# semihkacmaz/CoNFiLD

Hardware: AMD Instinct MI355X
Metric: generated fields/sec (256-step sample + CNF decode), Case4 latent, 1/2/4/8 GPU (higher is better)
Workload: dtype f32

## Files before the change

confild_amd/_lib.py:

```python
from __future__ import annotations

import ctypes as C
import os
import threading

_HERE = os.path.dirname(os.path.abspath(__file__))
LIB_PATH = os.path.join(_HERE, "lib", "libconfild_hip.so")
if os.environ.get("CFD_LIB"):
    LIB_PATH = os.path.join(_HERE, "lib", os.path.basename(os.environ["CFD_LIB"]))

_lock = threading.Lock()
_lib = None

c_f32p = C.POINTER(C.c_float)
c_i64p = C.POINTER(C.c_int64)


class CfdError(RuntimeError):
    pass


class UNetCfg(C.Structure):
    _fields_ = [("image_size", C.c_int), ("in_channels", C.c_int), ("model_channels", C.c_int),
                ("out_channels", C.c_int), ("num_res_blocks", C.c_int), ("n_mult", C.c_int),
                ("channel_mult", C.c_int * 8), ("n_attn", C.c_int), ("attention_ds", C.c_int * 8),
                ("num_heads", C.c_int), ("num_head_channels", C.c_int)]


class SirenCfg(C.Structure):
    _fields_ = [("in_coord_features", C.c_int), ("in_latent_features", C.c_int), ("out_features", C.c_int),
                ("num_hidden_layers", C.c_int), ("hidden_features", C.c_int), ("w0", C.c_float)]


_SIGS = {
    "cfd_last_error": (C.c_char_p, []),
    "cfd_version": (C.c_char_p, []),
    "cfd_unet_create": (C.c_int, [C.POINTER(UNetCfg), C.c_int, C.POINTER(C.c_void_p)]),
    "cfd_unet_destroy": (None, [C.c_void_p]),
    "cfd_unet_num_params": (C.c_int, [C.c_void_p, C.POINTER(C.c_int)]),
    "cfd_unet_param_info": (C.c_int, [C.c_void_p, C.c_int, C.POINTER(C.c_char_p), C.POINTER(C.c_int),
                                      C.c_int64 * 4]),
    "cfd_unet_set_param": (C.c_int, [C.c_void_p, C.c_char_p, C.c_void_p, C.c_size_t]),
    "cfd_unet_set_time_freqs": (C.c_int, [C.c_void_p, C.c_void_p, C.c_int]),
    "cfd_unet_ready": (C.c_int, [C.c_void_p]),
    "cfd_unet_load_flat": (C.c_int, [C.c_void_p, C.c_void_p, C.c_size_t, C.c_void_p]),
    "cfd_unet_set_compute": (C.c_int, [C.c_void_p, C.c_int]),
    "cfd_unet_set_plan_batch": (C.c_int, [C.c_void_p, C.c_int]),
    "cfd_device_cu_count": (C.c_int, [C.c_int, C.POINTER(C.c_int)]),
    "cfd_stream_create_cu_range": (C.c_int, [C.c_int, C.c_int, C.c_int, C.POINTER(C.c_void_p)]),
    "cfd_stream_destroy": (C.c_int, [C.c_void_p]),
    "cfd_unet_check_finite": (C.c_int, [C.c_void_p, C.POINTER(C.c_int), C.c_void_p]),
    "cfd_unet_workspace_bytes": (C.c_int, [C.c_void_p, C.c_int, C.POINTER(C.c_size_t)]),
    "cfd_unet_forward": (C.c_int, [C.c_void_p, C.c_void_p, C.c_void_p, C.c_void_p, C.c_int, C.c_void_p,
                                   C.c_size_t, C.c_void_p]),
    "cfd_unet_tape_bytes": (C.c_int, [C.c_void_p, C.c_int, C.POINTER(C.c_size_t)]),
    "cfd_unet_vjp_workspace_bytes": (C.c_int, [C.c_void_p, C.c_int, C.POINTER(C.c_size_t)]),
    "cfd_unet_forward_tape": (C.c_int, [C.c_void_p, C.c_void_p, C.c_void_p, C.c_void_p, C.c_int, C.c_void_p,
                                        C.c_size_t, C.c_void_p, C.c_size_t, C.c_void_p]),
    "cfd_unet_input_vjp": (C.c_int, [C.c_void_p, C.c_void_p, C.c_void_p, C.c_int, C.c_void_p, C.c_size_t,
                                     C.c_void_p, C.c_size_t, C.c_void_p]),
    "cfd_unet_set_tape_mode": (C.c_int, [C.c_void_p, C.c_int]),
    "cfd_sched_create": (C.c_int, [C.c_void_p, C.c_int, C.c_int, C.POINTER(C.c_void_p)]),
    "cfd_sched_destroy": (None, [C.c_void_p]),
    "cfd_sched_step": (C.c_int, [C.c_void_p, C.c_int, C.c_int, C.c_void_p, C.c_void_p, C.c_void_p, C.c_void_p,
                                 C.c_uint64, C.c_uint64, C.c_uint64, C.c_void_p, C.c_void_p, C.c_int64, C.c_int,
                                 C.c_void_p]),
    "cfd_sched_step_known": (C.c_int, [C.c_void_p, C.c_int, C.c_int, C.c_void_p, C.c_void_p, C.c_void_p, C.c_void_p,
                                       C.c_uint64, C.c_uint64, C.c_uint64, C.c_void_p, C.c_void_p, C.c_int64,
                                       C.c_int, C.c_void_p, C.c_int64, C.c_void_p, C.c_int64, C.c_void_p,
                                       C.c_void_p, C.c_uint64, C.c_void_p]),
    "cfd_sched_step_jump": (C.c_int, [C.c_void_p, C.c_int, C.c_int, C.c_void_p, C.c_void_p, C.c_void_p, C.c_void_p,
                                      C.c_uint64, C.c_uint64, C.c_uint64, C.c_void_p, C.c_void_p, C.c_int64,
                                      C.c_int, C.c_void_p, C.c_int64, C.c_void_p, C.c_int64, C.c_void_p,
                                      C.c_void_p, C.c_uint64, C.c_float, C.c_float, C.c_void_p, C.c_uint64,
                                      C.c_void_p]),
    "cfd_sampler_set_jumps": (C.c_int, [C.c_void_p, C.c_void_p]),
    "cfd_sampler_set_known": (C.c_int, [C.c_void_p, C.c_void_p, C.c_int64, C.c_void_p, C.c_int64, C.c_void_p,
                                        C.c_void_p]),
    "cfd_sampler_captures": (C.c_int, [C.c_void_p, C.POINTER(C.c_uint64)]),
    "cfd_dps_latent_residual_workspace_bytes": (C.c_int, [C.c_int64, C.c_int, C.POINTER(C.c_size_t)]),
    "cfd_dps_latent_residual": (C.c_int, [C.c_void_p, C.c_int, C.c_void_p, C.c_void_p, C.c_void_p, C.c_void_p,
                                          C.c_int64, C.c_void_p, C.c_int64, C.c_void_p, C.c_void_p, C.c_void_p,
                                          C.c_int64, C.c_int, C.c_void_p, C.c_size_t, C.c_void_p]),
    "cfd_sampler_create": (C.c_int, [C.c_void_p, C.c_void_p, C.c_int, C.c_int, C.c_int, C.c_int64, C.c_int,
                                     C.c_void_p, C.c_void_p, C.c_int, C.c_int, C.POINTER(C.c_void_p)]),
    "cfd_sampler_destroy": (None, [C.c_void_p]),
    "cfd_sampler_run": (C.c_int, [C.c_void_p, C.c_void_p, C.c_void_p, C.c_int, C.c_int, C.c_uint64, C.c_uint64,
                                  C.c_void_p]),
    "cfd_randn": (C.c_int, [C.c_void_p, C.c_int64, C.c_uint64, C.c_uint64, C.c_uint64, C.c_void_p]),
    "cfd_sine_probe": (C.c_int, [C.c_void_p, C.c_void_p, C.c_int64, C.c_int, C.c_void_p]),
    "cfd_latent_denorm": (C.c_int, [C.c_void_p, C.c_void_p, C.c_int64, C.c_void_p, C.c_void_p, C.c_int64,
                                    C.c_void_p]),
    "cfd_dps_residual": (C.c_int, [C.c_void_p, C.c_int64, C.c_void_p, C.c_void_p, C.c_void_p, C.c_int64, C.c_int,
                                   C.c_void_p]),
    "cfd_dps_latent_grad": (C.c_int, [C.c_void_p, C.c_int, C.c_void_p, C.c_void_p, C.c_void_p, C.c_void_p,
                                      C.c_void_p, C.c_void_p, C.c_int64, C.c_void_p, C.c_void_p, C.c_int64, C.c_int,
                                      C.c_void_p]),
    "cfd_dps_update": (C.c_int, [C.c_void_p, C.c_void_p, C.c_void_p, C.c_float, C.c_void_p, C.c_int64,
                                 C.c_void_p]),
    "cfd_dps_update_known": (C.c_int, [C.c_void_p, C.c_void_p, C.c_void_p, C.c_float, C.c_void_p, C.c_void_p,
                                       C.c_int64, C.c_int, C.c_void_p, C.c_int64, C.c_void_p, C.c_int64, C.c_void_p,
                                       C.c_void_p, C.c_uint64, C.c_uint64, C.c_uint64, C.c_void_p]),
    "cfd_siren_create": (C.c_int, [C.POINTER(SirenCfg), C.c_int, C.POINTER(C.c_void_p)]),
    "cfd_siren_destroy": (None, [C.c_void_p]),
    "cfd_siren_num_params": (C.c_int, [C.c_void_p, C.POINTER(C.c_int)]),
    "cfd_siren_param_info": (C.c_int, [C.c_void_p, C.c_int, C.POINTER(C.c_char_p), C.POINTER(C.c_int),
                                       C.c_int64 * 4]),
    "cfd_siren_set_param": (C.c_int, [C.c_void_p, C.c_char_p, C.c_void_p, C.c_size_t]),
    "cfd_siren_ready": (C.c_int, [C.c_void_p]),
    "cfd_siren_workspace_bytes": (C.c_int, [C.c_void_p, C.c_int, C.POINTER(C.c_size_t)]),
    "cfd_siren_set_compute": (C.c_int, [C.c_void_p, C.c_int]),
    "cfd_siren_get_compute": (C.c_int, [C.c_void_p, C.POINTER(C.c_int)]),
    "cfd_siren_forward": (C.c_int, [C.c_void_p, C.c_void_p, C.c_int64, C.c_void_p, C.c_int, C.c_void_p,
                                    C.c_void_p, C.c_void_p, C.c_void_p, C.c_int64, C.c_void_p, C.c_void_p,
                                    C.c_size_t, C.c_void_p]),
    "cfd_siren_jacobian_workspace_bytes": (C.c_int, [C.c_void_p, C.c_int, C.POINTER(C.c_size_t)]),
    "cfd_siren_forward_jacobian": (C.c_int, [C.c_void_p, C.c_void_p, C.c_int64, C.c_void_p, C.c_int, C.c_void_p,
                                             C.c_void_p, C.c_void_p, C.c_void_p, C.c_int64, C.c_void_p, C.c_void_p,
                                             C.c_void_p, C.c_size_t, C.c_void_p]),
    "cfd_siren_forward_jacobian_split": (C.c_int, [C.c_void_p, C.c_void_p, C.c_int64, C.c_void_p, C.c_int,
                                                   C.c_void_p, C.c_void_p, C.c_void_p, C.c_void_p, C.c_int64,
                                                   C.c_void_p, C.c_void_p, C.c_void_p, C.c_size_t, C.c_void_p]),
    "cfd_siren_hessian_workspace_bytes": (C.c_int, [C.c_void_p, C.c_int, C.POINTER(C.c_size_t)]),
    "cfd_siren_forward_hessian": (C.c_int, [C.c_void_p, C.c_void_p, C.c_int64, C.c_void_p, C.c_int, C.c_void_p,
                                            C.c_void_p, C.c_void_p, C.c_void_p, C.c_int64, C.c_void_p, C.c_void_p,
                                            C.c_void_p, C.c_int, C.c_void_p, C.c_size_t, C.c_void_p]),
    "cfd_siren_forward_hessian_split": (C.c_int, [C.c_void_p, C.c_void_p, C.c_int64, C.c_void_p, C.c_int,
                                                  C.c_void_p, C.c_void_p, C.c_void_p, C.c_void_p, C.c_int64,
                                                  C.c_void_p, C.c_void_p, C.c_void_p, C.c_int, C.c_void_p,
                                                  C.c_size_t, C.c_void_p]),
    "cfd_siren_vjp_workspace_bytes": (C.c_int, [C.c_void_p, C.c_int64, C.c_int, C.POINTER(C.c_size_t)]),
    "cfd_siren_tape_forward": (C.c_int, [C.c_void_p, C.c_void_p, C.c_int64, C.c_void_p, C.c_int, C.c_void_p,
                                         C.c_void_p, C.c_void_p, C.c_void_p, C.c_int64, C.c_void_p, C.c_void_p,
                                         C.c_size_t, C.c_void_p]),
    "cfd_siren_tape_vjp": (C.c_int, [C.c_void_p, C.c_void_p, C.c_int64, C.c_int, C.c_void_p, C.c_void_p,
                                     C.c_int64, C.c_void_p, C.c_void_p, C.c_size_t, C.c_void_p]),
    "cfd_siren_jtape_workspace_bytes": (C.c_int, [C.c_void_p, C.c_int64, C.c_int, C.POINTER(C.c_size_t)]),
    "cfd_siren_jtape_forward": (C.c_int, [C.c_void_p, C.c_void_p, C.c_int64, C.c_void_p, C.c_int, C.c_void_p,
                                          C.c_void_p, C.c_void_p, C.c_void_p, C.c_int64, C.c_void_p, C.c_void_p,
                                          C.c_void_p, C.c_size_t, C.c_void_p]),
    "cfd_siren_jtape_vjp": (C.c_int, [C.c_void_p, C.c_void_p, C.c_void_p, C.c_int64, C.c_int, C.c_void_p,
                                      C.c_void_p, C.c_int64, C.c_void_p, C.c_void_p, C.c_size_t, C.c_void_p]),
    "cfd_dps_residual_linear": (C.c_int, [C.c_void_p, C.c_int, C.c_void_p, C.c_void_p, C.c_void_p, C.c_int,
                                          C.c_void_p, C.c_int, C.c_void_p, C.c_void_p, C.c_void_p, C.c_void_p,
                                          C.c_int64, C.c_int, C.c_int, C.c_int, C.c_int, C.c_int, C.c_void_p]),
    "cfd_siren_dense_plan": (C.c_int, [C.POINTER(SirenCfg), C.c_int64, C.c_int, C.c_size_t, C.c_int, C.c_int,
                                       C.POINTER(C.c_size_t), C.POINTER(C.c_int64), C.POINTER(C.c_int)]),
    "cfd_siren_dense_workspace_bytes": (C.c_int, [C.c_void_p, C.c_int64, C.c_int, C.c_size_t,
                                                  C.POINTER(C.c_size_t)]),
    "cfd_siren_dense_grad": (C.c_int, [C.c_void_p, C.c_void_p, C.c_int64, C.c_void_p, C.c_int, C.c_int, C.c_void_p,
                                       C.c_void_p, C.c_void_p, C.c_void_p, C.c_int64, C.c_void_p, C.c_int,
                                       C.c_void_p, C.c_int, C.c_void_p, C.c_void_p, C.c_void_p, C.c_size_t,
                                       C.c_size_t, C.c_void_p]),
    "cfd_siren_dense_set_form": (C.c_int, [C.c_void_p, C.c_int, C.c_int]),
    "cfd_siren_train_workspace_bytes": (C.c_int, [C.c_void_p, C.c_int64, C.c_int, C.POINTER(C.c_size_t)]),
    "cfd_siren_train_grad": (C.c_int, [C.c_void_p, C.c_void_p, C.c_int64, C.c_void_p, C.c_void_p, C.c_int,
                                       C.c_void_p, C.c_float, C.c_void_p, C.c_void_p, C.c_void_p, C.c_void_p,
                                       C.c_size_t, C.c_void_p]),
    "cfd_unet_param_grad_workspace_bytes": (C.c_int, [C.c_void_p, C.c_int, C.POINTER(C.c_size_t)]),
    "cfd_unet_param_grad": (C.c_int, [C.c_void_p, C.c_void_p, C.c_void_p, C.c_int, C.c_void_p, C.c_size_t,
                                      C.c_void_p, C.c_void_p, C.c_size_t, C.c_void_p]),
    "cfd_eps_mse": (C.c_int, [C.c_void_p, C.c_void_p, C.c_void_p, C.c_void_p, C.c_int64, C.c_int, C.c_float,
                              C.c_void_p, C.c_void_p]),
    "cfd_ema_update": (C.c_int, [C.c_void_p, C.c_void_p, C.c_int64, C.c_double, C.c_void_p]),
    "cfd_q_sample": (C.c_int, [C.c_void_p, C.c_void_p, C.c_void_p, C.c_void_p, C.c_void_p, C.c_int64, C.c_int,
                               C.c_void_p]),
    "cfd_adam_step": (C.c_int, [C.c_void_p, C.c_void_p, C.c_void_p, C.c_void_p, C.c_int64, C.c_double, C.c_double,
                                C.c_double, C.c_double, C.c_double, C.c_int64, C.c_void_p]),
}

EXPORTS = tuple(_SIGS)


def load(path: str = LIB_PATH):
    global _lib
    with _lock:
        if _lib is not None:
            return _lib
        if not os.path.exists(path):
            raise CfdError(f"{path} is missing: build it with `python -c 'import __graft_entry__ as g; g.build()'` "
                           "(or `make -C confild_amd/csrc`)")
        lib = C.CDLL(path)
        for name, (res, args) in _SIGS.items():
            if os.environ.get("CFD_LIB") and not hasattr(lib, name):
                continue
            fn = getattr(lib, name)
            fn.restype = res
            fn.argtypes = args
        _lib = lib
        return lib


def lib():
    import torch
    if not torch.cuda.is_available():
        raise CfdError("confild_amd needs an AMD GPU (MI355X); no HIP device is visible and there is no CPU path")
    return load()


def check(rc: int, what: str = ""):
    if rc != 0:
        msg = load().cfd_last_error().decode()
        kind = {1: "bad argument", 2: "HIP error", 3: "unknown key", 4: "shape error", 5: "state error"}.get(rc, rc)
        raise CfdError(f"{what}: {kind}: {msg}")
# ... 12 lines not shown
```

confild_amd/csrc/conv_x.hip:

```cpp
#include <algorithm>
#include <type_traits>

#include "unet_kernels.hpp"

namespace cfd {

typedef float f16v __attribute__((ext_vector_type(16)));
typedef float f2 __attribute__((ext_vector_type(2)));
typedef _Float16 h2 __attribute__((ext_vector_type(2)));
typedef unsigned u4 __attribute__((ext_vector_type(4)));

__device__ __forceinline__ int xswz(int row, int chunk) { return row * 64 + ((chunk ^ ((row >> 2) & 3)) << 4); }

__device__ __forceinline__ void split4_mix_x(const f4& x, uint2& hi, uint2& lo) {
    hi.x = __builtin_bit_cast(unsigned, __builtin_convertvector((f2){x[0], x[1]}, h2));
    hi.y = __builtin_bit_cast(unsigned, __builtin_convertvector((f2){x[2], x[3]}, h2));
    asm("v_fma_mixlo_f16 %0, %1, 1.0, -%2 op_sel_hi:[0,0,1]" : "=&v"(lo.x) : "v"(x[0]), "v"(hi.x));
    asm("v_fma_mixhi_f16 %0, %1, 1.0, -%2 op_sel:[0,0,1] op_sel_hi:[0,0,1]" : "+v"(lo.x) : "v"(x[1]), "v"(hi.x));
    asm("v_fma_mixlo_f16 %0, %1, 1.0, -%2 op_sel_hi:[0,0,1]" : "=&v"(lo.y) : "v"(x[2]), "v"(hi.y));
    asm("v_fma_mixhi_f16 %0, %1, 1.0, -%2 op_sel:[0,0,1] op_sel_hi:[0,0,1]" : "+v"(lo.y) : "v"(x[3]), "v"(hi.y));
}

template <int BM, int BN, int WGM, int WGN, int PF = 1>
__global__ __launch_bounds__(64 * WGM * WGN, 1) void conv_x_kernel(ConvArgs a) {
    constexpr int NW = WGM * WGN, NT = 64 * NW;
    constexpr int WTM = BM / WGM, WTN = BN / WGN;
    constexpr int TM = WTM / 32, TN = WTN / 32;
    constexpr int RPP = NT / 8;
    constexpr int AIT = BM / RPP, BIT = BN / RPP;
    static_assert(TM >= 1 && TN >= 1 && AIT >= 1 && BIT >= 1, "tile");
    static_assert(BM % RPP == 0 && BN % RPP == 0, "staging");
    constexpr int ABYTES = BM * 64, BBYTES = BN * 64;
    constexpr int STAGE = 2 * ABYTES + 2 * BBYTES;
    __shared__ __attribute__((aligned(16))) char lds[2 * STAGE];

    CFD_STAMP(a.stamps, 2, a.seq, 0);
    const int tid = threadIdx.x, lane = tid & 63;
    const int wave = __builtin_amdgcn_readfirstlane(tid >> 6);
    const int wm = wave / WGN, wn = wave % WGN;

    int bx, by, bz;
    xcd_tile(a.xcd, bx, by, bz);
    const int m0 = bx * BM, n0 = by * BN;
    const int HWo = a.Hout * a.Wout;
    const int kq = tid & 7, rsub = tid >> 3;
    __shared__ int pixtab[9 * BM];

    const int srows = __builtin_amdgcn_readfirstlane(a.Hin * a.Win * (a.M / HWo));
    const __amdgpu_buffer_rsrc_t rs1 = __builtin_amdgcn_make_buffer_rsrc((void*)a.src1, 0, srows * a.C1 * 4, 0x00020000);
    const __amdgpu_buffer_rsrc_t rs2 = __builtin_amdgcn_make_buffer_rsrc(
        (void*)(a.src2 ? (const void*)a.src2 : (const void*)a.src1), 0, a.src2 ? srows * a.C2 * 4 : 0, 0x00020000);
    const int ntap = a.ks * a.ks, KM = ntap * a.Ctot;
    const __amdgpu_buffer_rsrc_t rwh = __builtin_amdgcn_make_buffer_rsrc((void*)a.wbf, 0, a.Cout * KM * 2, 0x00020000);
    const __amdgpu_buffer_rsrc_t rwl = __builtin_amdgcn_make_buffer_rsrc((void*)a.wlo, 0, a.Cout * KM * 2, 0x00020000);
    {
        const float rhw = 1.0f / (float)HWo, rw = 1.0f / (float)a.Wout;
        for (int e = tid; e < ntap * BM; e += NT) {
            const int tap = e / BM, r = e - tap * BM;
            const int ty = tap_row(tap, a.ks), tx = tap - ty * a.ks;
            const int m = m0 + r;
            int pix = -1;
            if (m < a.M) {
                const int b = fdiv24(m, HWo, rhw), rem = m - b * HWo;
                const int oy = fdiv24(rem, a.Wout, rw), ox = rem - oy * a.Wout;
                int iy, ix;
                bool ok;
                if (a.up) {
                    iy = oy - a.pad + ty;
                    ix = ox - a.pad + tx;
                    ok = iy >= 0 && iy < 2 * a.Hin && ix >= 0 && ix < 2 * a.Win;
                    iy >>= 1;
                    ix >>= 1;
                } else {
                    iy = oy * a.stride - a.pad + ty;
                    ix = ox * a.stride - a.pad + tx;
                    ok = iy >= 0 && iy < a.Hin && ix >= 0 && ix < a.Win;
                }
                if (ok) pix = (b * a.Hin + iy) * a.Win + ix;
            }
            CFD_DASSERT(pix < srows);
            pixtab[e] = pix;
        }
    }

    int a_row[AIT];
#pragma unroll
    for (int it = 0; it < AIT; ++it) a_row[it] = rsub + it * RPP;
    int b_row[BIT];
    unsigned b_voff[BIT];
#pragma unroll
    for (int it = 0; it < BIT; ++it) {
        b_row[it] = rsub + it * RPP;
        const int n = n0 + b_row[it];
        b_voff[it] = n < a.Cout ? (unsigned)((n * KM + 4 * kq) * 2) : 0x80000000u;
    }

    const int nkt = a.K / 32;
    const int per = (nkt + gridDim.z - 1) / gridDim.z;
    const int kt0 = bz * per;
    const int kt1 = min(nkt, kt0 + per);
    int cbg, tpg;
    {
        const int kb = kt0 * 32;
        const int tp = kb / a.Ctot;
        tpg = __builtin_amdgcn_readfirstlane(tp);
        cbg = __builtin_amdgcn_readfirstlane(kb - tp * a.Ctot);
    }
    __syncthreads();

    f4 ra[PF][AIT];
    uint2 rbh[PF][BIT], rbl[PF][BIT];
    auto load_tile = [&](int kt, int set) __attribute__((always_inline)) {
#pragma unroll
        for (int it = 0; it < AIT; ++it) {
            const bool second = cbg >= a.C1;
            const unsigned csrc4 = 4u * (second ? a.C2 : a.C1);
            const unsigned cofs4 = 4u * ((second ? cbg - a.C1 : cbg) + 4 * kq);
            const int pix = kt < kt1 ? pixtab[tpg * BM + a_row[it]] : -1;
            const unsigned off = pix >= 0 ? __umul24((unsigned)pix, csrc4) + cofs4 : 0x80000000u;
            ra[set][it] = __builtin_bit_cast(f4, __builtin_amdgcn_raw_buffer_load_b128(second ? rs2 : rs1, off, 0, 0));
        }
#pragma unroll
        for (int it = 0; it < BIT; ++it) {
            const unsigned voff = kt < kt1 ? b_voff[it] : 0x80000000u;
            const int soff = (tpg * a.Ctot + cbg) * 2;
            rbh[set][it] = __builtin_bit_cast(uint2, __builtin_amdgcn_raw_buffer_load_b64(rwh, voff, soff, 0));
            rbl[set][it] = __builtin_bit_cast(uint2, __builtin_amdgcn_raw_buffer_load_b64(rwl, voff, soff, 0));
        }
        cbg += 32;
        while (cbg >= a.Ctot && tpg < ntap) {
            cbg -= a.Ctot;
            ++tpg;
        }
    };
    auto store_tile = [&](int buf, int set) __attribute__((always_inline)) {
        char* base = lds + buf * STAGE;
#pragma unroll
        for (int it = 0; it < AIT; ++it) {
            const int off = xswz(a_row[it], kq >> 1) + (kq & 1) * 8;
            uint2 hv, lv;
            split4_mix_x(ra[set][it], hv, lv);
            *(uint2*)(base + off) = hv;
            *(uint2*)(base + ABYTES + off) = lv;
        }
#pragma unroll
        for (int it = 0; it < BIT; ++it) {
            const int off = xswz(b_row[it], kq >> 1) + (kq & 1) * 8;
            *(uint2*)(base + 2 * ABYTES + off) = rbh[set][it];
            *(uint2*)(base + 2 * ABYTES + BBYTES + off) = rbl[set][it];
        }
    };

    f16v acc[TM][TN];
#pragma unroll
    for (int i = 0; i < TM; ++i)
#pragma unroll
        for (int j = 0; j < TN; ++j)
#pragma unroll
            for (int e = 0; e < 16; ++e) acc[i][j][e] = 0.f;

    const int l32 = lane & 31, hsel = lane >> 5;
    const int arow0 = wm * WTM + l32, brow0 = wn * WTN + l32;
    auto kstep = [&](int kt, int cur, int lset, int sset) __attribute__((always_inline)) {
            const bool more = kt + 1 < kt1;
            if (kt + PF < kt1) load_tile(kt + PF, lset);
            const char* base = lds + cur * STAGE;
#pragma unroll
            for (int s = 0; s < 2; ++s) {
                const int ch = 2 * s + hsel;
                h8v fah[TM], fal[TM], fbh[TN], fbl[TN];
#pragma unroll
                for (int i = 0; i < TM; ++i) {
                    const int off = xswz(arow0 + 32 * i, ch);
                    fah[i] = *(const h8v*)(base + off);
                    fal[i] = *(const h8v*)(base + ABYTES + off);
                }
#pragma unroll
                for (int j = 0; j < TN; ++j) {
                    const int off = xswz(brow0 + 32 * j, ch);
                    fbh[j] = *(const h8v*)(base + 2 * ABYTES + off);
                    fbl[j] = *(const h8v*)(base + 2 * ABYTES + BBYTES + off);
                }
#pragma unroll
                for (int i = 0; i < TM; ++i)
#pragma unroll
                    for (int j = 0; j < TN; ++j) {
                        acc[i][j] = __builtin_amdgcn_mfma_f32_32x32x16_f16(fal[i], fbh[j], acc[i][j], 0, 0, 0);
                        acc[i][j] = __builtin_amdgcn_mfma_f32_32x32x16_f16(fah[i], fbl[j], acc[i][j], 0, 0, 0);
                        acc[i][j] = __builtin_amdgcn_mfma_f32_32x32x16_f16(fah[i], fbh[j], acc[i][j], 0, 0, 0);
                    }
            }
            if (more) store_tile(cur ^ 1, sset);
            __syncthreads();
    };
    if (kt0 < kt1) {
        load_tile(kt0, 0);
        if constexpr (PF == 2) {
            if (kt0 + 1 < kt1) load_tile(kt0 + 1, 1);
        }
        store_tile(0, 0);
        __syncthreads();
        CFD_STAMP(a.stamps, 2, a.seq, 2);
        if constexpr (PF == 1) {
            int cur = 0;
            for (int kt = kt0; kt < kt1; ++kt) {
                kstep(kt, cur, 0, 0);
                cur ^= 1;
            }
        } else {
            for (int kt = kt0; kt < kt1; kt += 2) {
                kstep(kt, 0, 0, 1);
                if (kt + 1 < kt1) kstep(kt + 1, 1, 1, 0);
            }
        }
    }

    CFD_STAMP(a.stamps, 2, a.seq, 3);
#pragma unroll
    for (int i = 0; i < TM; ++i)
#pragma unroll
        for (int j = 0; j < TN; ++j) acc[i][j] *= a.acc_scale;
    const int n_base = n0 + wn * WTN + l32;
    const int m_base = m0 + wm * WTM + 4 * hsel;
    if (gridDim.z > 1) {
        float* part = a.part + (int64_t)bz * a.M * a.Cout;
#pragma unroll
        for (int i = 0; i < TM; ++i)
#pragma unroll
            for (int e = 0; e < 16; ++e) {
                const int m = m_base + 32 * i + 8 * (e >> 2) + (e & 3);
                if (m >= a.M) continue;
#pragma unroll
                for (int j = 0; j < TN; ++j) {
                    const int n = n_base + 32 * j;
                    if (n < a.Cout) part[(int64_t)m * a.Cout + n] = acc[i][j][e];
                }
            }
#ifdef CFD_STAMPS
        __builtin_amdgcn_s_waitcnt(0);
#endif
        CFD_STAMP(a.stamps, 2, a.seq, 4);
        return;
    }
#pragma unroll
    for (int i = 0; i < TM; ++i)
#pragma unroll
        for (int e = 0; e < 16; ++e) {
            const int m = m_base + 32 * i + 8 * (e >> 2) + (e & 3);
            if (m >= a.M) continue;
            const int bb = m / HWo;
#pragma unroll
            for (int j = 0; j < TN; ++j) {
                const int n = n_base + 32 * j;
                if (n >= a.Cout) continue;
                float v = a.bias ? acc[i][j][e] + a.bias[n] : acc[i][j][e];
                if (a.emb) v = v + a.emb[(int64_t)bb * a.emb_stride + n];
                if (a.res) v = a.res[(int64_t)m * a.Cout + n] + v;
                a.out[(int64_t)m * a.Cout + n] = v;
            }
        }
}

template <int BM, int TW, bool BF = false, bool SB = false, int BN = 128>
__global__ __launch_bounds__(BM * (BN / 64), 1) void conv_h_kernel(ConvArgs a) {
    static_assert(!SB || BF, "a bf16 source needs the bf16 kernel");
    constexpr unsigned SES = SB ? 2u : 4u;
    constexpr int WGN = BN / 64, WGM = BM / 64, NTG = 64 * WGM * WGN;
    static_assert(BN == 64 || BN == 128, "K1h: 64 or 128 output channels per workgroup");
    constexpr int PL = BF ? 1 : 2;
    constexpr int HW2 = TW < 32 ? (TW + 2 + 3) / 4 * 4 : TW + 2;
    constexpr int TR = BM / TW, NPX = (TR + 2) * HW2;
    auto hswz = [](int px, int hr, int chunk) __attribute__((always_inline)) {
        if constexpr (TW == 16) return px * 64 + ((chunk ^ (((px >> 2) + 3 * hr) & 3)) << 4);
        else return xswz(px, chunk);
    };
    constexpr int HPLANE = NPX * 64;
    constexpr int HIT = (NPX * 8 + NTG - 1) / NTG;
    constexpr int TG = BF ? 3 : 1, SPR = 9 / TG;
    constexpr int BPLANE = BN * 64, BSTAGE = PL * BPLANE * TG;
    constexpr int BIT = BN * 4 / NTG;
    constexpr int GBYTES = PL * HPLANE + 2 * BSTAGE;
    static_assert(BM % TW == 0 && BIT >= 1, "tile");
    __shared__ __attribute__((aligned(16))) char lds[GBYTES];

    CFD_STAMP(a.stamps, 3, a.seq, 0);
    const int tid = threadIdx.x, lane = tid & 63;
    const int wave = __builtin_amdgcn_readfirstlane(tid >> 6);
    const int wm = wave / WGN, wn = wave % WGN;
    const int gt = tid;
    char* const halo = lds;
    char* const ring = halo + PL * HPLANE;
    int bx, by, bz;
    xcd_tile(a.xcd, bx, by, bz);
    const int n0 = by * BN;
    const int W = a.Wout, HWo = a.Hout * W;
    const int tps = HWo / BM, tpr = W / TW;
    const int bimg = bx / tps, tl = bx - bimg * tps;
    const int y0 = (tl / tpr) * TR, x0 = (tl - (tl / tpr) * tpr) * TW;
    const int64_t mrow0 = (int64_t)bimg * HWo + (int64_t)y0 * W + x0;
    CFD_DASSERT(mrow0 + (int64_t)(TR - 1) * W + TW <= a.M && HWo % BM == 0 && W % TW == 0);

    const int srows = __builtin_amdgcn_readfirstlane(a.Hin * a.Win * (a.M / HWo));
    const __amdgpu_buffer_rsrc_t rs1 = __builtin_amdgcn_make_buffer_rsrc((void*)a.src1, 0, srows * a.C1 * SES, 0x00020000);
    const __amdgpu_buffer_rsrc_t rs2 = __builtin_amdgcn_make_buffer_rsrc(
        (void*)(a.src2 ? (const void*)a.src2 : (const void*)a.src1), 0, a.src2 ? srows * a.C2 * SES : 0, 0x00020000);
    const __amdgpu_buffer_rsrc_t rwh = __builtin_amdgcn_make_buffer_rsrc((void*)a.wbf, 0, a.Cout * 9 * a.Ctot * 2, 0x00020000);
    const __amdgpu_buffer_rsrc_t rwl = __builtin_amdgcn_make_buffer_rsrc((void*)a.wlo, 0, a.Cout * 9 * a.Ctot * 2, 0x00020000);

    const int kq = gt & 7;
    int hpix[HIT];
#pragma unroll
    for (int it = 0; it < HIT; ++it) {
        const int hp = (gt + it * NTG) >> 3;
        int pix = -1;
        if (hp < NPX) {
            const int hr = hp / HW2, hc = hp - hr * HW2;
            const int iy = y0 - 1 + hr, ix = x0 - 1 + hc;
            if (hc < TW + 2 && iy >= 0 && iy < a.Hout && ix >= 0 && ix < W)
                pix = a.up ? (bimg * a.Hin + (iy >> 1)) * a.Win + (ix >> 1) : (bimg * a.Hin + iy) * a.Win + ix;
        }
        CFD_DASSERT(pix < srows);
        hpix[it] = pix;
    }
    const int bq = gt & 3;
    unsigned bvoff[BIT];
#pragma unroll
    for (int it = 0; it < BIT; ++it) {
        const int n = n0 + (gt >> 2) + it * (NTG / 4);
        bvoff[it] = n < a.Cout ? (unsigned)((n * 9 * a.Ctot + 8 * bq) * 2) : 0x80000000u;
    }

    const int nch = a.Ctot / 32;
    const int per = (nch + gridDim.z - 1) / gridDim.z;
    const int c0 = bz * per, cend = min(nch, c0 + per);
    const int nrounds = max(cend - c0, 0);
    auto chunk_of = [&](int r) __attribute__((always_inline)) { return c0 + r; };

    typedef typename std::conditional<SB, uint2, f4>::type HT;
    HT rh[HIT];
    constexpr int BW = BIT * TG;
    u4 wx_h[BW], wx_l[BW], wy_h[BW], wy_l[BW];
    auto load_halo = [&](int c) __attribute__((always_inline)) {
        const int cb = 32 * c;
        const bool second = cb >= a.C1;
        const unsigned csrc = SES * (unsigned)(second ? a.C2 + 0 : a.C1 + 0);
        const unsigned cofs = SES * ((second ? cb - a.C1 : cb) + 4 * kq);
        if (second) {
#pragma unroll
            for (int it = 0; it < HIT; ++it) {
                const unsigned off = hpix[it] >= 0 ? __umul24((unsigned)hpix[it], csrc) + cofs : 0x80000000u;
                if constexpr (SB)
                    rh[it] = __builtin_bit_cast(uint2, __builtin_amdgcn_raw_buffer_load_b64(rs2, off, 0, 0));
                else
                    rh[it] = __builtin_bit_cast(f4, __builtin_amdgcn_raw_buffer_load_b128(rs2, off, 0, 0));
            }
        } else {
#pragma unroll
            for (int it = 0; it < HIT; ++it) {
                const unsigned off = hpix[it] >= 0 ? __umul24((unsigned)hpix[it], csrc) + cofs : 0x80000000u;
                if constexpr (SB)
                    rh[it] = __builtin_bit_cast(uint2, __builtin_amdgcn_raw_buffer_load_b64(rs1, off, 0, 0));
                else
                    rh[it] = __builtin_bit_cast(f4, __builtin_amdgcn_raw_buffer_load_b128(rs1, off, 0, 0));
            }
        }
    };
    auto store_halo = [&]() __attribute__((always_inline)) {
#pragma unroll
        for (int it = 0; it < HIT; ++it) {
            const int e = gt + it * NTG;
            if (e < NPX * 8) {
                const int off = hswz(e >> 3, (e >> 3) / HW2, kq >> 1) + (kq & 1) * 8;
                if constexpr (SB) {
                    *(uint2*)(halo + off) = rh[it];
                } else if constexpr (BF) {
                    *(bf16x4*)(halo + off) = __builtin_convertvector(rh[it], bf16x4);
                } else {
                    uint2 hv, lv;
                    split4_mix_x(rh[it], hv, lv);
                    *(uint2*)(halo + off) = hv;
                    *(uint2*)(halo + HPLANE + off) = lv;
                }
            }
        }
    };
    auto load_w = [&](int s, u4 (&rbh)[BW], u4 (&rbl)[BW]) __attribute__((always_inline)) {
        const int r = s / SPR, c = chunk_of(r);
        if (c >= cend) return;
#pragma unroll
        for (int u = 0; u < TG; ++u) {
            const int soff = (((s - SPR * r) * TG + u) * a.Ctot + 32 * c) * 2;
#pragma unroll
            for (int it = 0; it < BIT; ++it) {
                rbh[u * BIT + it] = __builtin_bit_cast(u4, __builtin_amdgcn_raw_buffer_load_b128(rwh, bvoff[it], soff, 0));
                if constexpr (!BF)
                    rbl[u * BIT + it] = __builtin_bit_cast(u4, __builtin_amdgcn_raw_buffer_load_b128(rwl, bvoff[it], soff, 0));
            }
        }
    };
    auto store_w = [&](int stage, const u4 (&rbh)[BW], const u4 (&rbl)[BW]) __attribute__((always_inline)) {
#pragma unroll
        for (int u = 0; u < TG; ++u) {
            char* base = ring + stage * BSTAGE + u * PL * BPLANE;
#pragma unroll
            for (int it = 0; it < BIT; ++it) {
                const int off = xswz((gt >> 2) + it * (NTG / 4), bq);
                *(u4*)(base + off) = rbh[u * BIT + it];
                if constexpr (!BF) *(u4*)(base + BPLANE + off) = rbl[u * BIT + it];
            }
        }
    };

    f16v acc[2][2];
#pragma unroll
    for (int i = 0; i < 2; ++i)
#pragma unroll
        for (int j = 0; j < 2; ++j)
#pragma unroll
            for (int e = 0; e < 16; ++e) acc[i][j][e] = 0.f;

    const int l32 = lane & 31, hsel = lane >> 5;
    int hb[2], hrb[2];
#pragma unroll
    for (int i = 0; i < 2; ++i) {
        const int p = wm * 64 + 32 * i + l32;
        hb[i] = (p / TW) * HW2 + (p % TW);
        hrb[i] = p / TW;
    }
    const int brow0 = wn * 64 + l32;
    const int nsteps = nrounds * SPR;

    auto step = [&](int s, u4 (&ldh)[BW], u4 (&ldl)[BW], const u4 (&sth)[BW], const u4 (&stl)[BW])
        __attribute__((always_inline)) {
        const int r = s / SPR, t = s - SPR * r;
        const int c = chunk_of(r);
        if (s + 2 < nsteps) load_w(s + 2, ldh, ldl);
        if (t == 0 && chunk_of(r + 1) < cend) load_halo(chunk_of(r + 1));
        if (c < cend) {
            const char* wb = ring + (s & 1) * BSTAGE;
            if constexpr (BF) {
                const int ty = t;
#pragma unroll
                for (int u = 0; u < TG; ++u) {
                    const int tofs = ty * HW2 + u;
                    const char* wbu = wb + u * BPLANE;
#pragma unroll
                    for (int s2 = 0; s2 < 2; ++s2) {
                        const int ch = 2 * s2 + hsel;
                        bf16x8 fa[2], fb[2];
#pragma unroll
                        for (int i = 0; i < 2; ++i) fa[i] = *(const bf16x8*)(halo + hswz(hb[i] + tofs, hrb[i] + ty, ch));
#pragma unroll
                        for (int jj = 0; jj < 2; ++jj) fb[jj] = *(const bf16x8*)(wbu + xswz(brow0 + 32 * jj, ch));
#pragma unroll
                        for (int i = 0; i < 2; ++i)
#pragma unroll
                            for (int jj = 0; jj < 2; ++jj)
                                acc[i][jj] = __builtin_amdgcn_mfma_f32_32x32x16_bf16(fa[i], fb[jj], acc[i][jj], 0, 0, 0);
                    }
                }
            } else {
            const int ty = t / 3;
            const int tofs = ty * HW2 + (t - 3 * ty);
#pragma unroll
            for (int s2 = 0; s2 < 2; ++s2) {
                const int ch = 2 * s2 + hsel;
                h8v fah[2], fal[2], fbh[2], fbl[2];
#pragma unroll
                for (int i = 0; i < 2; ++i) {
                    CFD_DASSERT(hb[i] + tofs < NPX);
                    const int off = hswz(hb[i] + tofs, hrb[i] + ty, ch);
                    fah[i] = *(const h8v*)(halo + off);
                    fal[i] = *(const h8v*)(halo + HPLANE + off);
                }
#pragma unroll
                for (int jj = 0; jj < 2; ++jj) {
                    const int off = xswz(brow0 + 32 * jj, ch);
                    fbh[jj] = *(const h8v*)(wb + off);
                    fbl[jj] = *(const h8v*)(wb + BPLANE + off);
                }
#pragma unroll
                for (int i = 0; i < 2; ++i)
#pragma unroll
                    for (int jj = 0; jj < 2; ++jj) {
                        acc[i][jj] = __builtin_amdgcn_mfma_f32_32x32x16_f16(fal[i], fbh[jj], acc[i][jj], 0, 0, 0);
                        acc[i][jj] = __builtin_amdgcn_mfma_f32_32x32x16_f16(fah[i], fbl[jj], acc[i][jj], 0, 0, 0);
                        acc[i][jj] = __builtin_amdgcn_mfma_f32_32x32x16_f16(fah[i], fbh[jj], acc[i][jj], 0, 0, 0);
                    }
            }
            }
        }
        if (s + 1 < nsteps && chunk_of((s + 1) / SPR) < cend) store_w((s + 1) & 1, sth, stl);
        __syncthreads();
        if (t == SPR - 1 && s + 1 < nsteps) {
            if (chunk_of(r + 1) < cend) store_halo();
            __syncthreads();
        }
    };

    if (nsteps > 0) {
        load_w(0, wx_h, wx_l);
        if (nsteps > 1) load_w(1, wy_h, wy_l);
        load_halo(chunk_of(0));
        store_w(0, wx_h, wx_l);
        store_halo();
        __syncthreads();
        CFD_STAMP(a.stamps, 3, a.seq, 2);
        for (int s = 0; s < nsteps; s += 2) {
            step(s, wx_h, wx_l, wy_h, wy_l);
            if (s + 1 < nsteps) step(s + 1, wy_h, wy_l, wx_h, wx_l);
        }
    }

    CFD_STAMP(a.stamps, 3, a.seq, 3);
    if constexpr (!BF) {
#pragma unroll
        for (int i = 0; i < 2; ++i)
#pragma unroll
            for (int j = 0; j < 2; ++j) acc[i][j] *= a.acc_scale;
    }
    const int n_base = n0 + wn * 64 + l32;
    const int p_base = wm * 64 + 4 * hsel;
    auto pix_of = [&](int p) __attribute__((always_inline)) { return mrow0 + (int64_t)(p / TW) * W + (p % TW); };
    {
        if (a.ldsepi) {
            static_assert(64 * BN * 4 <= (int)sizeof(lds), "epilogue stage fits the LDS");
            float* stg = (float*)lds;
            const bool split = gridDim.z > 1;
            float* dstb = split ? a.part + (int64_t)bz * a.M * a.Cout : a.out;
            constexpr int Q = BN / 4;
            __syncthreads();
            for (int r = 0; r < WGM; ++r) {
                if (wm == r) {
#pragma unroll
                    for (int i = 0; i < 2; ++i)
#pragma unroll
                        for (int e = 0; e < 16; ++e)
#pragma unroll
                            for (int j = 0; j < 2; ++j)
                                stg[(32 * i + 8 * (e >> 2) + (e & 3) + 4 * hsel) * BN + wn * 64 + 32 * j + l32] =
                                    acc[i][j][e];
                }
                __syncthreads();
                for (int q = tid; q < 64 * Q; q += NTG) {
                    const int p = q / Q, c = (q - p * Q) * 4;
                    const int n = n0 + c;
                    if (n < a.Cout) {
                        const int64_t m = pix_of(r * 64 + p);
                        f4 v = *(const f4*)(stg + p * BN + c);
                        if (!split) {
                            if (a.bias) v = v + *(const f4*)(a.bias + n);
                            if (a.emb) v = v + *(const f4*)(a.emb + (int64_t)bimg * a.emb_stride + n);
                            if (a.res) v = *(const f4*)(a.res + m * a.Cout + n) + v;
                        }
                        *(f4*)(dstb + m * a.Cout + n) = v;
                    }
                }
                __syncthreads();
            }
#ifdef CFD_STAMPS
            __builtin_amdgcn_s_waitcnt(0);
#endif
            CFD_STAMP(a.stamps, 3, a.seq, 4);
            return;
        }
    }
    if (gridDim.z > 1) {
        float* part = a.part + (int64_t)bz * a.M * a.Cout;
#pragma unroll
        for (int i = 0; i < 2; ++i)
#pragma unroll
            for (int e = 0; e < 16; ++e) {
                const int64_t m = pix_of(p_base + 32 * i + 8 * (e >> 2) + (e & 3));
#pragma unroll
                for (int j = 0; j < 2; ++j) {
                    const int n = n_base + 32 * j;
                    if (n < a.Cout) part[(int64_t)m * a.Cout + n] = acc[i][j][e];
                }
            }
#ifdef CFD_STAMPS
        __builtin_amdgcn_s_waitcnt(0);
#endif
        CFD_STAMP(a.stamps, 3, a.seq, 4);
        return;
    }
#pragma unroll
    for (int i = 0; i < 2; ++i)
#pragma unroll
        for (int e = 0; e < 16; ++e) {
            const int64_t m = pix_of(p_base + 32 * i + 8 * (e >> 2) + (e & 3));
#pragma unroll
            for (int j = 0; j < 2; ++j) {
                const int n = n_base + 32 * j;
                if (n >= a.Cout) continue;
                float v = a.bias ? acc[i][j][e] + a.bias[n] : acc[i][j][e];
                if (a.emb) v = v + a.emb[(int64_t)bimg * a.emb_stride + n];
                if (a.res) v = a.res[(int64_t)m * a.Cout + n] + v;
                a.out[(int64_t)m * a.Cout + n] = v;
            }
        }
#ifdef CFD_STAMPS
    __builtin_amdgcn_s_waitcnt(0);
#endif
    CFD_STAMP(a.stamps, 3, a.seq, 4);
}

int conv_h_tw(const ConvArgs& a) {
    const bool geo = !a.tmode && a.ks == 3 && a.stride == 1 && a.pad == 1 && a.C1 % 32 == 0 && a.C2 % 32 == 0 &&
                     (a.up ? a.Hout == 2 * a.Hin && a.Wout == 2 * a.Win : a.Hout == a.Hin && a.Wout == a.Win) &&
                     a.M % (a.Hout * a.Wout) == 0;
    if (!geo) return 0;
    for (int tw = 64; tw >= 16; tw >>= 1)
        if (a.Wout % tw == 0 && a.Hout % (256 / tw) == 0) return tw;
    return 0;
}

int launch_conv_x(const ConvArgs& a, int variant, int splits, hipStream_t st) {
    CFD_REQUIRE(a.wbf && !a.tmode, CFD_ESTATE, "conv_x: split-f16 or bf16 forward only");
    CFD_REQUIRE(a.Ctot % 32 == 0 && a.C1 % 4 == 0 && a.C2 % 4 == 0, CFD_ESHAPE, "conv_x needs channels % 32 == 0");
    CFD_REQUIRE(splits == 1 || a.part, CFD_ESTATE, "split-K needs a partial buffer");
    {
        const int64_t srows = (int64_t)a.Hin * a.Win * (a.M / (a.Hout * a.Wout));
        CFD_REQUIRE(srows < (1 << 24) && srows * std::max(a.C1, a.C2) * 4 < (1ll << 31) &&
                        (int64_t)a.Cout * a.K * 2 < (1ll << 31) && a.ks * a.ks <= 9,
                    CFD_ESHAPE, "conv_x: operands beyond 2 GiB");
    }
    auto grid = [&](int bm, int bn) __attribute__((always_inline)) {
        return dim3((unsigned)ceil_div(a.M, bm), (unsigned)ceil_div(a.Cout, bn), splits);
    };
    if (variant == 22) {
        const int tw = conv_h_tw(a);
        CFD_REQUIRE(tw > 0 && !a.wlo, CFD_ESHAPE, "conv_h bf16: 3x3 stride-1 with a 16/32/64-divisible width");
        const dim3 g = grid(256, 128);
        if (a.src_bf16) {
            if (tw == 64) hipLaunchKernelGGL((conv_h_kernel<256, 64, true, true>), g, dim3(512), 0, st, a);
            else if (tw == 32) hipLaunchKernelGGL((conv_h_kernel<256, 32, true, true>), g, dim3(512), 0, st, a);
            else hipLaunchKernelGGL((conv_h_kernel<256, 16, true, true>), g, dim3(512), 0, st, a);
        } else {
            if (tw == 64) hipLaunchKernelGGL((conv_h_kernel<256, 64, true>), g, dim3(512), 0, st, a);
            else if (tw == 32) hipLaunchKernelGGL((conv_h_kernel<256, 32, true>), g, dim3(512), 0, st, a);
            else hipLaunchKernelGGL((conv_h_kernel<256, 16, true>), g, dim3(512), 0, st, a);
        }
        check_launch("conv_h_kernel");
        return splits;
    }
    CFD_REQUIRE(!a.src_bf16, CFD_ESTATE, "internal: a bf16 convolution source needs the K1hb kernel");
    if (variant == 20) {
        const int tw = conv_h_tw(a);
        CFD_REQUIRE(tw > 0, CFD_ESHAPE, "conv_h: 3x3 stride-1 with a 16/32/64-divisible width");
        static const int smalln = smalln_below();
        const dim3 g = grid(256, 128);
        if ((int64_t)g.x * g.y * g.z < smalln && a.Cout % 64 == 0) {
            const dim3 g64 = grid(256, 64);
            if (tw == 64) hipLaunchKernelGGL((conv_h_kernel<256, 64, false, false, 64>), g64, dim3(256), 0, st, a);
            else if (tw == 32) hipLaunchKernelGGL((conv_h_kernel<256, 32, false, false, 64>), g64, dim3(256), 0, st, a);
            else hipLaunchKernelGGL((conv_h_kernel<256, 16, false, false, 64>), g64, dim3(256), 0, st, a);
            check_launch("conv_h_kernel");
            return splits;
        }
        if (tw == 64) hipLaunchKernelGGL((conv_h_kernel<256, 64>), g, dim3(512), 0, st, a);
        else if (tw == 32) hipLaunchKernelGGL((conv_h_kernel<256, 32>), g, dim3(512), 0, st, a);
        else hipLaunchKernelGGL((conv_h_kernel<256, 16>), g, dim3(512), 0, st, a);
        check_launch("conv_h_kernel");
        return splits;
    }
    CFD_REQUIRE(a.wlo, CFD_ESTATE, "internal: K1x runs split-f16 operands only");
    switch (variant) {
        case 1: hipLaunchKernelGGL((conv_x_kernel<128, 128, 2, 2>), grid(128, 128), dim3(256), 0, st, a); break;
        case 2: hipLaunchKernelGGL((conv_x_kernel<256, 128, 4, 2>), grid(256, 128), dim3(512), 0, st, a); break;
        default: CFD_REQUIRE(false, CFD_EARG, "conv_x variant");
    }
    check_launch("conv_x_kernel");
    return splits;
}

}
```

confild_amd/csrc/siren_split.hip:

```cpp
#include <cstdint>
#include <cstdlib>
#include <algorithm>

#include "siren.hpp"

typedef _Float16 h8 __attribute__((ext_vector_type(8)));
typedef _Float16 h2 __attribute__((ext_vector_type(2)));
typedef float f2 __attribute__((ext_vector_type(2)));
typedef unsigned u2 __attribute__((ext_vector_type(2)));
typedef unsigned u4 __attribute__((ext_vector_type(4)));

namespace cfd {

struct Frag {
    u4 v;
    __device__ __forceinline__ h8 h() const { return __builtin_bit_cast(h8, v); }
};

__device__ __forceinline__ unsigned pk_f16(float a, float b) {
    return __builtin_bit_cast(unsigned, __builtin_convertvector((f2){a, b}, h2));
}

__device__ __forceinline__ void split8(const float (&x0)[4], const float (&x1)[4], Frag& hi, Frag& lo) {
    unsigned hw[4], lw[4];
// ... 42 lines not shown
    u = fmaf(u, s, -0.166666597127914428710938f);
    const float y = fmaf(s, u * r, r);
    return __uint_as_float(__float_as_uint(y) + (__float_as_uint(t) << 31));
}

__device__ __forceinline__ float sin_hw(float x) {
    const float t = fmaf(x, 0.159154943091895335768f, 12582912.0f);
    const float q = t - 12582912.0f;
    float r = fmaf(q, -6.28125f, x);
    r = fmaf(q, -0.001934051513671875f, r);
    r = fmaf(q, -1.2554228305816650391e-06f, r);
    r = fmaf(q, -2.4308402513106841524e-10f, r);
    return __builtin_amdgcn_sinf(r * 0.159154943091895335768f);
}

__device__ __forceinline__ float sin_hw_rev(float x) {
    const float t = fmaf(x, 0.159154943091895335768f, 12582912.0f);
    const float q = t - 12582912.0f;
    float r = fmaf(x, 0.15915493667125701904f, -q);
    r = fmaf(x, 6.4206382432985265041e-09f, r);
    return __builtin_amdgcn_sinf(r);
}

template <int HWSIN>
__device__ __forceinline__ float hidden_sine(float x) {
    if constexpr (HWSIN == 4) return __builtin_amdgcn_sinf(x);
    else if constexpr (HWSIN == 3) return __builtin_amdgcn_sinf(__builtin_amdgcn_fractf(x));
    else if constexpr (HWSIN == 2) return sin_hw_rev(x);
    else if constexpr (HWSIN == 1) return sin_hw(x);
    else return sin1_cw(x);
}

template <bool PK>
__device__ __forceinline__ f2 sin2_sel(f2 x) {
    if constexpr (PK) return sin2_cw(x);
    else return (f2){sin1_cw(x.x), sin1_cw(x.y)};
}

constexpr int vmcnt_imm(int n) { return (n & 15) | (7 << 4) | (15 << 8) | (((n >> 4) & 3) << 14); }
constexpr int vm_lgkm0_imm(int n) { return vmcnt_imm(n) & ~(15 << 8); }

template <int NB, int WAVES, int RING, int CG, int RB = 1, bool NOSYNC = false, bool PKSIN = true>
__global__ __launch_bounds__(64 * WAVES, CG == 1 ? 2 : 1) void siren_fused_split(SirenArgs p) {
    static_assert(NB % 2 == 0, "split-f16 chain needs H % 32 == 0");
    constexpr int NQ = NB / 2;
    constexpr int TILE = 16 * CG * WAVES;
    constexpr int H = NB * 16;
    constexpr int BLK = NB * 256;
    constexpr int SLOT = RB * BLK;
    static_assert(NB % RB == 0, "ring slots hold whole groups of RB blocks");
    extern __shared__ __attribute__((aligned(16))) float smem[];
    const int nh = p.nh;
    float* wbuf = smem;
    float* film = smem + RING * SLOT;
    float* w0s = film + (nh + 1) * H;
    float* wos = w0s + 4 * H;

    const int lane = threadIdx.x & 63;
    const int wave = threadIdx.x >> 6;
    const int g = lane >> 4;
    const int j16 = lane & 15;
    const int64_t b = p.b0 + blockIdx.y;
    const int64_t n0 = (int64_t)blockIdx.x * TILE + wave * 16 * CG + j16;

    {
        const float* fsrc = p.film + b * (int64_t)(nh + 1) * H;
        const int nf = (nh + 1) * H;
        for (int i = threadIdx.x * 4; i < nf; i += 64 * WAVES * 4) {
            const int layer = i / H;
            const float sc = layer == 0 ? 1.0f : p.wscale[layer - 1];
            *(f4*)(film + i) = *(const f4*)(fsrc + i) * sc;
        }
    }
    for (int f = threadIdx.x; f < H; f += 64 * WAVES) {
        f4 w = {0.f, 0.f, 0.f, 0.f};
        for (int k = 0; k < p.d; ++k) w[k] = p.w0[f * p.d + k];
        *(f4*)(w0s + 4 * f) = w;
    }
    for (int i = threadIdx.x; i < 4 * H; i += 64 * WAVES) wos[i] = i < p.c * H ? p.wout[i] : 0.f;
    float cn[CG][4];
#pragma unroll
    for (int c = 0; c < CG; ++c) {
        const int64_t n = n0 + 16 * c;
        const int64_t nc = n < p.N ? n : p.N - 1;
#pragma unroll
        for (int k = 0; k < 4; ++k) {
            float v = 0.f;
            if (k < p.d) {
                v = p.coords[nc * p.d + k];
                if (p.xmax) v = (v - p.xmin[k]) / (p.xmax[k] - p.xmin[k]) * 2.0f - 1.0f;
            }
            cn[c][k] = v;
        }
    }

    __syncthreads();
    const int nslots = nh * NB / RB;
    for (int k = 0; k < RING - 1; ++k)
        if (k < nslots) siren_issue_block<RB * NB, WAVES>(p.wimg, k, wbuf + k * SLOT, wave, lane);
    constexpr int PC_LO = RB * NB / WAVES, PC_HI = (RB * NB + WAVES - 1) / WAVES;
    const bool pc_hi = wave < (RB * NB) % WAVES;

    Frag BH[CG][NQ], BL[CG][NQ], NH[CG][NQ], NL[CG][NQ];
    float o[CG][4];
#pragma unroll
    for (int c = 0; c < CG; ++c)
#pragma unroll
        for (int oc = 0; oc < 4; ++oc) o[c][oc] = 0.f;
    auto out_acc = [&](int c, int j, const float (&x)[4]) __attribute__((always_inline)) {
#pragma unroll
        for (int oc = 0; oc < 4; ++oc) {
            if (oc < p.c) {
                const f4 w = *(const f4*)(wos + oc * H + 16 * j + 4 * g);
                o[c][oc] = fmaf(w.x, x[0], o[c][oc]);
                o[c][oc] = fmaf(w.y, x[1], o[c][oc]);
                o[c][oc] = fmaf(w.z, x[2], o[c][oc]);
                o[c][oc] = fmaf(w.w, x[3], o[c][oc]);
            }
        }
    };

    static_for<NQ>([&](auto qc) {
        constexpr int q = decltype(qc)::value;
#pragma unroll
        for (int c = 0; c < CG; ++c) {
            float x[2][4];
#pragma unroll
            for (int hb = 0; hb < 2; ++hb) {
                const int blk = 2 * q + hb;
                const f4 fv = *(const f4*)(film + 16 * blk + 4 * g);
                float u[4];
#pragma unroll
                for (int r = 0; r < 4; ++r) {
                    const f4 w = *(const f4*)(w0s + 4 * (16 * blk + 4 * g + r));
                    float a = cn[c][0] * w[0];
#pragma unroll
                    for (int k = 1; k < 4; ++k)
                        if (k < p.d) a = fmaf(cn[c][k], w[k], a);
                    u[r] = p.w0f * (a + fv[r]);
                }
#pragma unroll
                for (int r = 0; r < 4; r += 2) {
                    const f2 v = sin2_cw((f2){u[r], u[r + 1]});
                    x[hb][r] = v.x;
                    x[hb][r + 1] = v.y;
                }
            }
            split8(x[0], x[1], BH[c][q], BL[c][q]);
        }
    });

    int J = 0, slot = 0;
    constexpr int QE = NQ > 1 ? 1 : 0;
    for (int layer = 1; layer <= nh; ++layer) {
        const bool last = layer == nh;
        const float m = p.w0f / p.wscale[layer - 1];
        float x[CG][4], xs[CG][4];
        auto sines = [&](const f4 (&a)[CG]) __attribute__((always_inline)) {
#pragma unroll
            for (int c = 0; c < CG; ++c) {
                const f2 v0 = sin2_sel<PKSIN>((f2){a[c][0] * m, a[c][1] * m});
                const f2 v1 = sin2_sel<PKSIN>((f2){a[c][2] * m, a[c][3] * m});
                x[c][0] = v0.x;
                x[c][1] = v0.y;
                x[c][2] = v1.x;
                x[c][3] = v1.y;
                asm volatile("" : "+v"(x[c][0]), "+v"(x[c][1]), "+v"(x[c][2]), "+v"(x[c][3]));
            }
        };
        auto epilogue = [&](auto jc) __attribute__((always_inline)) {
            constexpr int j = decltype(jc)::value;
#pragma unroll
            for (int c = 0; c < CG; ++c) {
                if (last) {
                    out_acc(c, j, x[c]);
                } else if constexpr (j & 1) {
                    split8(xs[c], x[c], NH[c][j / 2], NL[c][j / 2]);
                } else {
#pragma unroll
                    for (int r = 0; r < 4; ++r) xs[c][r] = x[c][r];
                }
            }
        };
        f4 prev[CG];
        static_for<NB>([&](auto jc) {
            constexpr int j = decltype(jc)::value;
            const bool steady = J + RING - 1 < nslots;
            {
                const int fill = slot == 0 ? RING - 1 : slot - 1;
                if (steady && !NOSYNC)
                    siren_issue_block<NB, WAVES>(p.wimg, (J + RING - 1) * RB + j % RB,
                                                 wbuf + fill * SLOT + (j % RB) * BLK, wave, lane);
            }
            const float* wb = wbuf + slot * SLOT + (j % RB) * BLK;
            f4 a[CG];
            {
                const f4 f = *(const f4*)(film + layer * H + 16 * j + 4 * g);
#pragma unroll
                for (int c = 0; c < CG; ++c) a[c] = f;
            }
            h8 FH[NQ], FL[NQ];
            FH[0] = *(const h8*)(wb + lane * 4);
            FL[0] = *(const h8*)(wb + 256 + lane * 4);
            static_for<NQ>([&](auto qc) {
                constexpr int q = decltype(qc)::value;
                if constexpr (q + 1 < NQ) {
                    FH[q + 1] = *(const h8*)(wb + (q + 1) * 512 + lane * 4);
                    FL[q + 1] = *(const h8*)(wb + (q + 1) * 512 + 256 + lane * 4);
                }
#pragma unroll
                for (int c = 0; c < CG; ++c)
                    a[c] = __builtin_amdgcn_mfma_f32_16x16x32_f16(FL[q], BH[c][q].h(), a[c], 0, 0, 0);
#pragma unroll
                for (int c = 0; c < CG; ++c)
                    a[c] = __builtin_amdgcn_mfma_f32_16x16x32_f16(FH[q], BL[c][q].h(), a[c], 0, 0, 0);
#pragma unroll
                for (int c = 0; c < CG; ++c)
                    a[c] = __builtin_amdgcn_mfma_f32_16x16x32_f16(FH[q], BH[c][q].h(), a[c], 0, 0, 0);
                if constexpr (j > 0) {
                    if constexpr (q == 0) sines(prev);
                    if constexpr (q == QE) epilogue(std::integral_constant<int, j - 1>{});
                }
                __builtin_amdgcn_sched_barrier(0);
            });
#pragma unroll
            for (int c = 0; c < CG; ++c) prev[c] = a[c];
            if constexpr (j % RB == RB - 1) {
                if (NOSYNC) {
                } else if (steady) {
                    if (PC_HI == PC_LO || !pc_hi)
                        __builtin_amdgcn_s_waitcnt(vmcnt_imm((RING - 2) * PC_LO));
                    else
                        __builtin_amdgcn_s_waitcnt(vmcnt_imm((RING - 2) * PC_HI));
                } else {
                    __builtin_amdgcn_s_waitcnt(vmcnt_imm(0));
                }
                if (!NOSYNC) asm volatile("s_barrier" ::: "memory");
                ++J;
                slot = slot == RING - 1 ? 0 : slot + 1;
            }
        });
        sines(prev);
        epilogue(std::integral_constant<int, NB - 1>{});
        static_for<NQ>([&](auto qc) {
            constexpr int q = decltype(qc)::value;
#pragma unroll
            for (int c = 0; c < CG; ++c) {
                BH[c][q] = NH[c][q];
                BL[c][q] = NL[c][q];
            }
        });
    }

#pragma unroll
    for (int c = 0; c < CG; ++c) {
        float ov[4];
#pragma unroll
        for (int oc = 0; oc < 4; ++oc) {
            float sum = o[c][oc];
            sum += __shfl_xor(sum, 16);
            sum += __shfl_xor(sum, 32);
            ov[oc] = oc < p.c ? sum + p.bout[oc] : 0.f;
        }
        const int64_t n = n0 + 16 * c;
        if (n < p.N && g < p.c) {
            float v = g == 0 ? ov[0] : g == 1 ? ov[1] : g == 2 ? ov[2] : ov[3];
            if (p.ymax) {
                const int64_t yi = n * p.ystride + g;
                const float hi = p.ymax[yi], lo = p.ymin[yi];
                v = (v + 1.0f) / 2.0f * (hi - lo) + lo;
            }
            p.out[(b * p.N + n) * p.c + g] = v;
        }
    }
}

typedef float f16v __attribute__((ext_vector_type(16)));

__device__ __forceinline__ void split2_mix(float a, float b, unsigned& hi, unsigned& lo) {
    hi = pk_f16(a, b);
    asm("v_fma_mixlo_f16 %0, %1, 1.0, -%2 op_sel_hi:[0,0,1]" : "=&v"(lo) : "v"(a), "v"(hi));
    asm("v_fma_mixhi_f16 %0, %1, 1.0, -%2 op_sel:[0,0,1] op_sel_hi:[0,0,1]" : "+v"(lo) : "v"(b), "v"(hi));
}

__device__ __forceinline__ void split_chunk(const float (&x)[16], int e, Frag& hi, Frag& lo) {
    unsigned hw[4], lw[4];
#pragma unroll
    for (int w = 0; w < 4; ++w) split2_mix(x[8 * e + 2 * w], x[8 * e + 2 * w + 1], hw[w], lw[w]);
    hi.v = (u4){hw[0], hw[1], hw[2], hw[3]};
    lo.v = (u4){lw[0], lw[1], lw[2], lw[3]};
    asm volatile("" : "+v"(hi.v), "+v"(lo.v));
}

__device__ __forceinline__ float fma_scalar(float a, float b, float c) {
    float d;
    asm("v_fma_f32 %0, %1, %2, %3" : "=v"(d) : "v"(a), "v"(b), "v"(c));
    return d;
}

template <int NB2, int EXP, int HWSIN>
__device__ __forceinline__ void split32_body(const SirenArgs& p) {
    constexpr int NK = 2 * NB2;
    constexpr int H = 32 * NB2;
    constexpr int BLK = NK * 512;
    constexpr int WAVES = 4, TILE = 128;
    constexpr int NPC = 2 * NK;
// ... 1039 lines not shown
```

confild_amd/csrc/unet.hip:

```cpp
#include <algorithm>
#include <cstring>
#include <cmath>
#include <functional>
#include <map>
#include <string>
#include <vector>

#include "sampler.hpp"
#include "unet_kernels.hpp"
#include "unet_train.hpp"

namespace cfd {

enum class Pack { Raw, Conv3, Conv1, EmbW, EmbB };

struct UParam {
    std::string key;
    std::vector<int64_t> shape;
    Pack pack = Pack::Raw;
    size_t offset = 0;
    size_t count = 0;
    int emb_row = 0;
    bool set = false;
    int tpack = 0;
    size_t toffset = 0;
    float split_inv = 1.f;
    float tsplit_inv = 1.f;
};

struct ResSpec {
    std::string pre;
    int cin, cout, emb_off;
};
struct AttnSpec {
    std::string pre;
    int C, heads, ch;
};

struct Step {
    enum Kind { In, Res, Attn, Down, Up, Push, Cat, Out } kind;
    int idx = 0;
    std::string conv;
    int cin = 0, cout = 0;
};

}

struct cfd_unet {
    cfd_unet_cfg cfg{};
    int device = 0;
    int tdim = 0;
    std::vector<cfd::UParam> params;
    std::map<std::string, int> index;
    std::vector<cfd::ResSpec> res;
    std::vector<cfd::AttnSpec> attn;
    std::vector<cfd::Step> steps;
    int emb_total = 0;
    float* arena = nullptr;
    size_t arena_floats = 0;
    float* emb_w = nullptr;
    float* emb_b = nullptr;
    float* freqs = nullptr;
    float* arena_t = nullptr;
    size_t arena_t_floats = 0;
    uint16_t* arena_bf = nullptr;
    uint16_t* arena_hi = nullptr;
    uint16_t* arena_lo = nullptr;
    uint16_t* arena_thi = nullptr;
    uint16_t* arena_tlo = nullptr;
    int compute = CFD_COMPUTE_SPLIT_F16;
    int plan_b = 0;
    int tape_mode = CFD_TAPE_INPUT_VJP;
    struct TapeRec { int mode, B, plan; uint64_t seq; };
    std::map<const void*, TapeRec> tapes;
    uint64_t tape_seq = 0;
    int* nonfinite = nullptr;
    mutable std::map<int, size_t> ws_cache;
    uint64_t version = 0;
    void* rp_desc = nullptr;
    int64_t* rp_first = nullptr;
    float* rp_part = nullptr;
    float* rp_amax = nullptr;
    int64_t rp_blocks = 0;
    int64_t* rp_tfirst = nullptr;
    int64_t rp_tiles = 0;
};

namespace {

using cfd::Pack;

void add_param(cfd_unet* h, const std::string& key, std::vector<int64_t> shape, Pack pack, int emb_row = 0) {
    cfd::UParam p;
    p.key = key;
    p.shape = shape;
    p.pack = pack;
    p.emb_row = emb_row;
    p.count = 1;
    for (auto s : shape) p.count *= (size_t)s;
    h->index[key] = (int)h->params.size();
    h->params.push_back(p);
}

void add_conv(cfd_unet* h, const std::string& pre, int cin, int cout, int k, bool conv1d = false, bool up = false,
              bool mirror = false) {
    if (conv1d)
        add_param(h, pre + ".weight", {cout, cin, 1}, Pack::Conv1);
    else
        add_param(h, pre + ".weight", {cout, cin, k, k}, k == 3 ? Pack::Conv3 : Pack::Conv1);
    h->params.back().tpack = up ? 2 : mirror ? 3 : 1;
    add_param(h, pre + ".bias", {cout}, Pack::Raw);
}

void add_norm(cfd_unet* h, const std::string& pre, int c) {
    add_param(h, pre + ".weight", {c}, Pack::Raw);
    add_param(h, pre + ".bias", {c}, Pack::Raw);
}

int add_res(cfd_unet* h, const std::string& pre, int cin, int cout) {
    add_norm(h, pre + ".in_layers.0", cin);
    add_conv(h, pre + ".in_layers.2", cin, cout, 3, false, false, true);
    add_param(h, pre + ".emb_layers.1.weight", {cout, h->tdim}, Pack::EmbW, h->emb_total);
    add_param(h, pre + ".emb_layers.1.bias", {cout}, Pack::EmbB, h->emb_total);
    add_norm(h, pre + ".out_layers.0", cout);
    add_conv(h, pre + ".out_layers.3", cout, cout, 3, false, false, true);
    if (cin != cout) add_conv(h, pre + ".skip_connection", cin, cout, 1);
    h->res.push_back({pre, cin, cout, h->emb_total});
    h->emb_total += cout;
    return (int)h->res.size() - 1;
}

int add_attn(cfd_unet* h, const std::string& pre, int C) {
    const int heads = h->cfg.num_head_channels == -1 ? h->cfg.num_heads : C / h->cfg.num_head_channels;
    CFD_REQUIRE(heads > 0 && C % heads == 0, CFD_EARG, "channels not divisible into heads at " + pre);
    add_norm(h, pre + ".norm", C);
    add_conv(h, pre + ".qkv", C, 3 * C, 1, true);
    add_conv(h, pre + ".proj_out", C, C, 1, true);
    h->attn.push_back({pre, C, heads, C / heads});
    return (int)h->attn.size() - 1;
}

bool has_attn(const cfd_unet* h, int ds) {
    for (int i = 0; i < h->cfg.n_attn; ++i)
        if (h->cfg.attention_ds[i] == ds) return true;
    return false;
}

void build(cfd_unet* h) {
    const auto& c = h->cfg;
    const int mc = c.model_channels;
    h->tdim = 4 * mc;
    add_param(h, "time_embed.0.weight", {h->tdim, mc}, Pack::Raw);
    add_param(h, "time_embed.0.bias", {h->tdim}, Pack::Raw);
    add_param(h, "time_embed.2.weight", {h->tdim, h->tdim}, Pack::Raw);
    add_param(h, "time_embed.2.bias", {h->tdim}, Pack::Raw);
    int ch = c.channel_mult[0] * mc;
    add_conv(h, "input_blocks.0.0", c.in_channels, ch, 3);
    h->steps.push_back({cfd::Step::In, 0, "input_blocks.0.0", c.in_channels, ch});
    h->steps.push_back({cfd::Step::Push});
    std::vector<int> chans{ch};
    int ds = 1, idx = 1;
    for (int level = 0; level < c.n_mult; ++level) {
        for (int r = 0; r < c.num_res_blocks; ++r) {
            const int cout = c.channel_mult[level] * mc;
            const std::string pre = "input_blocks." + std::to_string(idx);
            int ri = add_res(h, pre + ".0", ch, cout);
            h->steps.push_back({cfd::Step::Res, ri});
            ch = cout;
            if (has_attn(h, ds)) h->steps.push_back({cfd::Step::Attn, add_attn(h, pre + ".1", ch)});
            h->steps.push_back({cfd::Step::Push});
            chans.push_back(ch);
            ++idx;
        }
        if (level != c.n_mult - 1) {
            const std::string pre = "input_blocks." + std::to_string(idx) + ".0.op";
            add_conv(h, pre, ch, ch, 3);
            h->steps.push_back({cfd::Step::Down, 0, pre, ch, ch});
            h->steps.push_back({cfd::Step::Push});
            chans.push_back(ch);
            ds *= 2;
            ++idx;
        }
    }
    h->steps.push_back({cfd::Step::Res, add_res(h, "middle_block.0", ch, ch)});
    h->steps.push_back({cfd::Step::Attn, add_attn(h, "middle_block.1", ch)});
    h->steps.push_back({cfd::Step::Res, add_res(h, "middle_block.2", ch, ch)});
    idx = 0;
    for (int level = c.n_mult - 1; level >= 0; --level) {
        for (int i = 0; i < c.num_res_blocks + 1; ++i) {
            const int ich = chans.back();
            chans.pop_back();
            const int cout = mc * c.channel_mult[level];
            const std::string pre = "output_blocks." + std::to_string(idx);
            h->steps.push_back({cfd::Step::Cat});
            h->steps.push_back({cfd::Step::Res, add_res(h, pre + ".0", ch + ich, cout)});
            ch = cout;
            int j = 1;
            if (has_attn(h, ds)) {
                h->steps.push_back({cfd::Step::Attn, add_attn(h, pre + ".1", ch)});
                j = 2;
            }
            if (level && i == c.num_res_blocks) {
                const std::string up = pre + "." + std::to_string(j) + ".conv";
                add_conv(h, up, ch, ch, 3, false, true);
                h->steps.push_back({cfd::Step::Up, 0, up, ch, ch});
                ds /= 2;
            }
            ++idx;
        }
    }
    add_norm(h, "out.0", ch);
    add_conv(h, "out.2", c.channel_mult[0] * mc, c.out_channels, 3);
    h->steps.push_back({cfd::Step::Out, 0, "out", ch, c.out_channels});
    size_t off = 0;
    for (auto& p : h->params) {
        if (p.pack == Pack::EmbW || p.pack == Pack::EmbB) continue;
        p.offset = off;
        off += (p.count + 3) & ~size_t(3);
    }
    h->arena_floats = off;
    size_t toff = 0;
    for (auto& p : h->params) {
        if (!p.tpack) continue;
        p.toffset = toff;
        toff += ((p.tpack == 2 ? p.count / 9 * 16 : p.count) + 3) & ~size_t(3);
    }
    h->arena_t_floats = toff;
}

const void* PB(const cfd_unet* h, const std::string& key) {
    if (h->compute == CFD_COMPUTE_F32) return nullptr;
    auto it = h->index.find(key);
    CFD_REQUIRE(it != h->index.end(), CFD_EKEY, "internal: missing param " + key);
    return (h->compute == CFD_COMPUTE_BF16 ? h->arena_bf : h->arena_hi) + h->params[it->second].offset;
}

const void* PL(const cfd_unet* h, const std::string& key, float* inv) {
    *inv = 1.f;
    if (h->compute != CFD_COMPUTE_SPLIT_F16) return nullptr;
    auto it = h->index.find(key);
    CFD_REQUIRE(it != h->index.end(), CFD_EKEY, "internal: missing param " + key);
    *inv = h->params[it->second].split_inv;
    return h->arena_lo + h->params[it->second].offset;
}

uint16_t to_bf16(float f) {
    uint32_t u;
    std::memcpy(&u, &f, 4);
    if ((u & 0x7fffffffu) > 0x7f800000u) return (uint16_t)((u >> 16) | 0x40u);
    return (uint16_t)((u + 0x7fffu + ((u >> 16) & 1u)) >> 16);
}

void PTS(const cfd_unet* h, const std::string& key, cfd::ConvArgs* a) {
    if (h->compute != CFD_COMPUTE_SPLIT_F16) return;
    auto it = h->index.find(key);
    CFD_REQUIRE(it != h->index.end() && h->params[it->second].tpack, CFD_EKEY, "internal: missing conv " + key);
    const auto& p = h->params[it->second];
    a->wbf = h->arena_thi + p.toffset;
    a->wlo = h->arena_tlo + p.toffset;
    a->acc_scale = p.tsplit_inv;
}

const float* PT(const cfd_unet* h, const std::string& key) {
    auto it = h->index.find(key);
    CFD_REQUIRE(it != h->index.end() && h->params[it->second].tpack, CFD_EKEY, "internal: missing conv " + key);
    return h->arena_t + h->params[it->second].toffset;
}

const float* P(const cfd_unet* h, const std::string& key) {
    auto it = h->index.find(key);
    CFD_REQUIRE(it != h->index.end(), CFD_EKEY, "internal: missing param " + key);
    return h->arena + h->params[it->second].offset;
}

struct Act {
    const float* a = nullptr;
    int Ca = 0;
    const float* b = nullptr;
    int Cb = 0;
    int H = 0, W = 0;
    int C() const { return Ca + Cb; }
    bool bf16 = false;
};

struct Workspace {
    char* base;
    size_t off = 0;
    bool dry;
    float* take(size_t nfloats) {
        off = (off + 255) & ~size_t(255);
        float* p = dry ? nullptr : (float*)(base + off);
        off += nfloats * sizeof(float);
        return p;
    }
};

struct Rec {
    Act in;
    const float* h1 = nullptr;
    float *ss1 = nullptr, *st1 = nullptr;
    float *ss2 = nullptr, *st2 = nullptr;
    float *qkv = nullptr, *o = nullptr, *lse = nullptr;
    const float *act1 = nullptr, *act2 = nullptr;
    unsigned *amx1 = nullptr, *amx2 = nullptr;
    int skip_hs = -1;
    int push_hs = -1;
};

struct Tape {
    Workspace* tws;
    std::vector<Rec>* recs;
    bool keep_gnout = false;
    float* temb = nullptr;
    float* th1 = nullptr;
    float* emb = nullptr;
};

struct Sizes {
    size_t max_act = 0, max_qkv = 0, max_cat = 0, max_att = 0;
    size_t max_kvf = 0;
    size_t max_abw = 0;
    size_t max_apart = 0;
    std::vector<size_t> hs;
};

int plan_batch(const cfd_unet* h);

Sizes sizes(const cfd_unet* h) {
    const auto& c = h->cfg;
    const int mc = c.model_channels, S = c.image_size;
    Sizes z;
    int ch = c.channel_mult[0] * mc, hw = S, cmax = 0;
    z.max_act = (size_t)hw * hw * ch;
    z.hs.push_back((size_t)hw * hw * ch);
    for (int l = 0; l < c.n_mult; ++l) cmax = std::max(cmax, c.channel_mult[l] * mc);
    for (int l = 0; l < c.n_mult; ++l) {
        const int co = c.channel_mult[l] * mc;
        z.max_act = std::max(z.max_act, (size_t)hw * hw * std::max(co, ch));
        z.max_qkv = std::max(z.max_qkv, (size_t)hw * hw * 3 * co);
        z.max_cat = std::max(z.max_cat, (size_t)hw * hw * (co + cmax));
        z.max_att = std::max(z.max_att, (size_t)hw * hw * co);
        z.max_kvf = std::max(z.max_kvf, cfd::attention_split_floats(hw * hw, co));
        if (has_attn(h, 1 << l) || l == c.n_mult - 1) {
            z.max_abw = std::max(z.max_abw, cfd::attention_bwd_split_floats(hw * hw, co));
            const int heads = c.num_head_channels == -1 ? c.num_heads : co / c.num_head_channels;
            z.max_apart = std::max(z.max_apart, cfd::attention_part_floats(hw * hw, co, co / heads, plan_batch(h)));
        }
        for (int r = 0; r < c.num_res_blocks; ++r) z.hs.push_back((size_t)hw * hw * co);
        ch = co;
        if (l != c.n_mult - 1) {
            hw /= 2;
            z.hs.push_back((size_t)hw * hw * ch);
        }
    }
    z.max_cat = std::max(z.max_cat, z.max_act);
    return z;
}

constexpr size_t kSplitPer8 = size_t(16) << 20;
int plan_batch(const cfd_unet* h) { return h->plan_b > 0 ? h->plan_b : 8; }
size_t split_cap(const cfd_unet* h, int B) {
    const int pb = plan_batch(h);
    return kSplitPer8 * (size_t)std::max(1, (B + pb - 1) / pb);
}

cfd::ConvPlan plan_checked(const cfd_unet* h, const cfd::ConvArgs& a0, size_t slab_floats) {
    cfd::ConvArgs a = a0;
    a.plan_b = plan_batch(h);
    const cfd::ConvPlan p = cfd::plan_conv(a, kSplitPer8);
    CFD_REQUIRE(p.splits == 1 || (size_t)p.splits * a.M * a.Cout <= slab_floats, CFD_ESTATE,
                "internal: split-K slab too small");
    return p;
}

void run(const cfd_unet* h, const float* x, const int64_t* t, float* eps, int B, Workspace& ws, hipStream_t st,
         Tape* tape = nullptr, bool launch_req = true) {
    const auto& c = h->cfg;
    const int mc = c.model_channels, S = c.image_size;
    const Sizes z = sizes(h);
    const bool launch = launch_req && !ws.dry && !(tape && tape->tws->dry);
    const size_t kSplitCap = split_cap(h, B);
    float* temb = tape ? tape->tws->take((size_t)B * mc) : ws.take((size_t)B * mc);
    float* h1 = tape ? tape->tws->take((size_t)B * h->tdim) : ws.take((size_t)B * h->tdim);
    float* emb = tape ? tape->tws->take((size_t)B * h->tdim) : ws.take((size_t)B * h->tdim);
    if (tape) {
        tape->temb = temb;
        tape->th1 = h1;
        tape->emb = emb;
    }
    float* embo = ws.take((size_t)B * h->emb_total);
    double* gnpart = (double*)ws.take((size_t)B * cfd::kGnMaxChunks * 32 * 2 * 2);
    float* gnss = ws.take((size_t)B * 1024 * 2);
    float* nbuf = ws.take((size_t)B * z.max_cat);
    float* splitk = ws.take(kSplitCap);
    float* kvws = ws.take((size_t)B * z.max_kvf);
    float* apart = z.max_apart ? ws.take((size_t)B * z.max_apart) : nullptr;
    float* pool[3];
    for (auto& p : pool) p = ws.take((size_t)B * z.max_act);
    float* tmp = ws.take((size_t)B * z.max_act);
    float* skipb = ws.take((size_t)B * z.max_act);
    float* qkv = tape ? nullptr : ws.take((size_t)B * z.max_qkv);
    float* abuf = tape ? nullptr : ws.take((size_t)B * z.max_act);
    std::vector<float*> hsbuf;
    for (size_t n : z.hs) hsbuf.push_back(tape ? tape->tws->take((size_t)B * n) : ws.take((size_t)B * n));
    constexpr int kGnSlots = 256;
    unsigned* gslots = tape ? (unsigned*)tape->tws->take(kGnSlots) : nullptr;
    int ngs = 0;
    if (ws.dry && !tape) return;
    auto keep = [&](size_t nfloats) -> float* { return tape->tws->take(nfloats); };
    if (tape && tape->keep_gnout && launch) CFD_HIP(hipMemsetAsync(gslots, 0, sizeof(unsigned) * kGnSlots, st));
    std::vector<Rec>* recs = tape ? tape->recs : nullptr;
    if (recs) recs->assign(h->steps.size(), Rec{});

    auto pick = [&](const float* busy1, const float* busy2) -> float* {
        if (!launch && (ws.dry || !busy1)) return pool[0];
        for (auto p : pool)
            if (p != busy1 && p != busy2) return p;
        throw cfd::Error{CFD_ESTATE, "internal: buffer pool exhausted"};
    };

    if (launch) {
        cfd::launch_temb(t, h->freqs, temb, mc, B, st);
        cfd::launch_linear(temb, P(h, "time_embed.0.weight"), P(h, "time_embed.0.bias"), h1, B, mc, h->tdim, 0, st);
        cfd::launch_linear(h1, P(h, "time_embed.2.weight"), P(h, "time_embed.2.bias"), emb, B, h->tdim, h->tdim, 1,
                           st);
        cfd::launch_linear(emb, h->emb_w, h->emb_b, embo, B, h->tdim, h->emb_total, 1, st);
    }

    struct Pending {
        cfd::ConvArgs a{};
        int splits = 0;
    } pend;
    auto flush = [&]() {
        if (pend.splits > 1 && launch) cfd::launch_splitk_reduce(pend.a, pend.splits, st);
        pend.splits = 0;
    };

    auto gn = [&](const Act& in, const std::string& pre, int silu, float** ss, float** stats,
                  bool keep_raw = true, bool bf16_out = false, const float** actp = nullptr,
                  unsigned** amxp = nullptr) -> Act {
        cfd::GnArgs g{};
        g.src1 = in.a;
        g.src2 = in.b;
        g.gamma = P(h, pre + ".weight");
        g.beta = P(h, pre + ".bias");
        g.part = gnpart;
        g.ss = gnss;
        if (tape) {
            *ss = g.ss = keep((size_t)B * in.C() * 2);
            *stats = g.stats = keep((size_t)B * 64);
        }
        g.out = nbuf;
        if (tape && actp && tape->keep_gnout) {
            CFD_REQUIRE(!bf16_out && ngs < kGnSlots, CFD_ESTATE, "internal: kept GroupNorm output");
            g.out = keep((size_t)B * in.H * in.W * in.C());
            g.amax_out = gslots + ngs++;
            *actp = g.out;
            *amxp = g.amax_out;
        }
        g.C1 = in.Ca;
        g.C2 = in.Cb;
        g.Ctot = in.C();
        g.HW = in.H * in.W;
        g.eps = 1e-5f;
        g.plan_b = plan_batch(h);
        g.silu = silu;
        if (pend.splits > 1 && pend.a.out == in.a && pend.a.Cout == in.Ca && cfd::gn_takes_splitk(g, B)) {
            g.kpart = pend.a.part;
            g.ksplits = pend.splits;
            g.kbias = pend.a.bias;
            g.kemb = pend.a.emb;
            g.kemb_stride = pend.a.emb_stride;
            g.kres = pend.a.res;
            g.kx = keep_raw || cfd::gn2_applies(g) ? pend.a.out : nullptr;
            pend.splits = 0;
        } else {
            flush();
        }
        static const int gn_log = getenv("CFD_CONV_LOG") ? atoi(getenv("CFD_CONV_LOG")) : 0;
        if (gn_log && launch)
            fprintf(stderr, "GN %s %dx%d C=%d+%d ksplits=%d kres=%d kx=%d silu=%d\n", pre.c_str(), in.H, in.W, g.C1,
                    g.C2, g.kpart ? g.ksplits : 0, g.kres ? 1 : 0, g.kx ? 1 : 0, silu);
        g.out_bf16 = bf16_out ? 1 : 0;
        if (launch) cfd::launch_gn(g, B, st);
        Act r{g.out, in.C(), nullptr, 0, in.H, in.W};
        r.bf16 = bf16_out;
        return r;
    };
    auto conv_args = [&](const Act& in, const std::string& pre, int cout, int ks, int stride, int up,
                         const float* embp, const float* resp, float* out) {
        cfd::ConvArgs a{};
        a.src1 = in.a;
        a.src2 = in.b;
        a.C1 = in.Ca;
        a.C2 = in.Cb;
        a.Ctot = in.C();
        a.w = P(h, pre + ".weight");
        a.wbf = PB(h, pre + ".weight");
        a.wlo = PL(h, pre + ".weight", &a.acc_scale);
        a.bias = P(h, pre + ".bias");
        a.emb = embp;
        a.emb_stride = h->emb_total;
        a.res = resp;
        a.out = out;
        a.part = splitk;
        a.Hin = in.H;
        a.Win = in.W;
        a.Hout = up ? in.H * 2 : (stride == 2 ? (in.H + 1) / 2 : in.H);
        a.Wout = up ? in.W * 2 : (stride == 2 ? (in.W + 1) / 2 : in.W);
        a.stride = stride;
        a.ks = ks;
        a.pad = ks == 3 ? 1 : 0;
        a.up = up;
        a.Cout = cout;
        a.M = B * a.Hout * a.Wout;
        a.K = ks * ks * a.Ctot;
        a.src_bf16 = in.bf16 ? 1 : 0;
        return a;
    };
    static const int gn_bf16out = getenv("CFD_GN_BF16OUT") ? atoi(getenv("CFD_GN_BF16OUT")) : 1;
    auto feeds_k1hb = [&](const Act& in, const std::string& pre, int cout) -> bool {
        if (!gn_bf16out || h->compute != CFD_COMPUTE_BF16) return false;
        Act n{nbuf, in.C(), nullptr, 0, in.H, in.W};
        const cfd::ConvArgs a = conv_args(n, pre, cout, 3, 1, 0, nullptr, nullptr, nullptr);
        return a.wbf && !a.wlo && cfd::conv_runs_k1hb(a, plan_checked(h, a, kSplitCap));
    };
    using Tweak = std::function<void(cfd::ConvArgs&, const cfd::ConvPlan&)>;
    auto conv = [&](const Act& in, const std::string& pre, int cout, int ks, int stride, int up,
                    const float* embp, const float* resp, float* out, const Tweak& tweak = {}) {
        cfd::ConvArgs a = conv_args(in, pre, cout, ks, stride, up, embp, resp, out);
        flush();
        const cfd::ConvPlan plan = plan_checked(h, a, kSplitCap);
        if (tweak) tweak(a, plan);
        CFD_REQUIRE(!a.src_bf16 || cfd::conv_runs_k1hb(a, plan), CFD_ESTATE,
                    "internal: bf16 GroupNorm output feeds a convolution other than K1hb at " + pre);
        static const int conv_log = getenv("CFD_CONV_LOG") ? atoi(getenv("CFD_CONV_LOG")) : 0;
        if (conv_log && launch)
            fprintf(stderr, "CONV %s %dx%d C=%d+%d->%d ks=%d s=%d up=%d M=%d kx=%d bm=%d bn=%d nw=%d splits=%d\n",
                    pre.c_str(), a.Hin, a.Win, a.C1, a.C2, a.Cout, a.ks, a.stride, a.up, a.M, plan.kx, plan.bm,
                    plan.bn, plan.nw, plan.splits);
        if (launch) {
            const int sp = cfd::launch_conv(a, plan, st, true);
            if (sp > 1) {
                pend.a = a;
                pend.splits = sp;
            }
        }
    };

    std::vector<std::pair<Act, int>> stack;
    Act cur;
    size_t hs_i = 0;
    int pending_skip = -1;
    for (size_t si = 0; si < h->steps.size(); ++si) {
        const auto& s = h->steps[si];
        Rec rec;
        rec.in = cur;
        const bool to_skip = si + 1 < h->steps.size() && h->steps[si + 1].kind == cfd::Step::Push;
        auto dest = [&](const float* busy1, const float* busy2, size_t nfl) -> float* {
            if (to_skip) return hsbuf[hs_i];
            return tape ? keep(nfl) : pick(busy1, busy2);
        };
        switch (s.kind) {
            case cfd::Step::In: {
                cfd::ConvArgs a{};
                a.src1 = x;
                a.C1 = c.in_channels;
                a.Ctot = c.in_channels;
                a.w = P(h, s.conv + ".weight");
                a.bias = P(h, s.conv + ".bias");
                a.out = hsbuf[0];
                a.Hin = a.Hout = S;
                a.Win = a.Wout = S;
                a.Cout = s.cout;
                a.M = B * S * S;
                if (launch) cfd::launch_conv_in(a, st);
                cur = Act{hsbuf[0], s.cout, nullptr, 0, S, S};
                break;
            }
            case cfd::Step::Push: {
                float* dst = hsbuf[hs_i];
                if (cur.a != dst) {
                    flush();
                    if (launch)
                        CFD_HIP(hipMemcpyAsync(dst, cur.a, sizeof(float) * (size_t)B * cur.H * cur.W * cur.Ca,
                                               hipMemcpyDeviceToDevice, st));
                    cur.a = dst;
                }
                rec.push_hs = (int)hs_i;
                stack.push_back({cur, (int)hs_i});
                ++hs_i;
                break;
            }
            case cfd::Step::Cat: {
                const auto skip = stack.back();
                stack.pop_back();
                CFD_REQUIRE(cur.b == nullptr && skip.first.H == cur.H, CFD_ESTATE, "internal: concat shape");
                cur.b = skip.first.a;
                cur.Cb = skip.first.Ca;
                pending_skip = skip.second;
                break;
            }
            case cfd::Step::Res: {
                const auto& r = h->res[s.idx];
                CFD_REQUIRE(cur.C() == r.cin, CFD_ESTATE, "internal: ResBlock input channels at " + r.pre);
                rec.skip_hs = pending_skip;
                pending_skip = -1;
                const size_t nout = (size_t)B * cur.H * cur.W * r.cout;
                const Act xin = gn(cur, r.pre + ".in_layers.0", 1, &rec.ss1, &rec.st1, true,
                                   feeds_k1hb(cur, r.pre + ".in_layers.2", r.cout), &rec.act1, &rec.amx1);
                const float* resp = nullptr;
                if (r.cin != r.cout) {
                    resp = skipb;
                } else {
                    CFD_REQUIRE(cur.b == nullptr, CFD_ESTATE, "identity skip on a concatenated input");
                    resp = cur.a;
                }
                float* hb = tape ? keep(nout) : tmp;
                conv(xin, r.pre + ".in_layers.2", r.cout, 3, 1, 0, embo + r.emb_off, nullptr, hb);
                rec.h1 = hb;
                const Act th{hb, r.cout, nullptr, 0, cur.H, cur.W};
                const Act hn = gn(th, r.pre + ".out_layers.0", 1, &rec.ss2, &rec.st2, tape != nullptr,
                                  feeds_k1hb(th, r.pre + ".out_layers.3", r.cout), &rec.act2, &rec.amx2);
                float* out = dest(cur.a, cur.b, nout);
                if (r.cin != r.cout)
                    conv(cur, r.pre + ".skip_connection", r.cout, 1, 1, 0, nullptr, nullptr, skipb);
                conv(hn, r.pre + ".out_layers.3", r.cout, 3, 1, 0, nullptr, resp, out);
                cur = Act{out, r.cout, nullptr, 0, cur.H, cur.W};
                break;
            }
            case cfd::Step::Attn: {
                const auto& at = h->attn[s.idx];
                const int T = cur.H * cur.W;
                const Act xn = gn(cur, at.pre + ".norm", 0, &rec.ss1, &rec.st1, true, false, &rec.act1, &rec.amx1);
                float* qb = tape ? keep((size_t)B * T * 3 * at.C) : qkv;
                float* ob = tape ? keep((size_t)B * T * at.C) : abuf;
                const float attn_scale = (float)(1.0 / std::sqrt(std::sqrt((double)at.ch)));
                const bool split_attn = h->compute != CFD_COMPUTE_F32 && (at.ch == 32 || at.ch == 64 || at.ch == 128);
                bool kv_packed = false;
                conv(xn, at.pre + ".qkv", 3 * at.C, 1, 1, 0, nullptr, nullptr, qb,
                     [&](cfd::ConvArgs& a, const cfd::ConvPlan& plan) {
                         if (!split_attn || h->compute == CFD_COMPUTE_F32 || !cfd::conv_kv_pack_ok(a, plan, T))
                             return;
                         a.kvf = kvws;
                         a.kv_voff = cfd::attention_split_voff(T, at.ch, at.heads, B);
                         a.kv_ch = at.ch;
                         a.kv_heads = at.heads;
                         a.kv_T = T;
                         a.kv_scale = attn_scale;
                         kv_packed = true;
                     });
                cfd::AttnArgs aa{qb, ob, T, at.C, attn_scale, nullptr};
// ... 280 lines not shown
                float* out = gfree(dcur.a);
                if (pg) wgrad(dcur.a, dcur.Ca, in, nullptr, 0, dcur.H, dcur.W, 3, 2, 1, 0, s.conv, dmax);
                dconv(dcur.a, dcur.Ca, dcur.H, dcur.W, s.conv + ".weight", s.cin, in.H, in.W, 3, 2, 1, 1, out);
                dcur = Act{out, s.cin, nullptr, 0, in.H, in.W};
                dmax = nullptr;
                break;
            }
            case cfd::Step::Push:
                dmax = nullptr;
                cfd::launch_add(const_cast<float*>(dcur.a), dhs[r.push_hs], (int64_t)B * dcur.H * dcur.W * dcur.Ca,
                                st);
                break;
            case cfd::Step::Cat:
                break;
            case cfd::Step::Res: {
                const auto& rs = h->res[s.idx];
                const float* dout = dcur.a;
                float* G = gfree(dout);
                const Act h1{r.h1, rs.cout, nullptr, 0, in.H, in.W};
                unsigned* omax = dmax;
                if (pg)
                    omax = r.act2 ? wgrad(dout, rs.cout, Act{r.act2, rs.cout, nullptr, 0, in.H, in.W}, nullptr, 0, in.H,
                                          in.W, 3, 1, 1, 0, rs.pre + ".out_layers.3", omax, r.amx2)
                                  : wgrad(dout, rs.cout, h1, r.ss2, 1, in.H, in.W, 3, 1, 1, 0, rs.pre + ".out_layers.3",
                                          omax);
                dconv(dout, rs.cout, in.H, in.W, rs.pre + ".out_layers.3.weight", rs.cout, in.H, in.W, 3, 1, 1, 0, G);
                float* dh1 = gfree(dout, G);
                unsigned* h1max = slot();
                gnb(h1, r.ss2, r.st2, rs.pre + ".out_layers.0", 1, G, nullptr, dh1, nullptr, true, h1max);
                if (pg) {
                    if (r.act1)
                        wgrad(dh1, rs.cout, Act{r.act1, in.C(), nullptr, 0, in.H, in.W}, nullptr, 0, in.H, in.W, 3, 1, 1,
                              0, rs.pre + ".in_layers.2", h1max, r.amx1);
                    else
                        wgrad(dh1, rs.cout, in, r.ss1, 1, in.H, in.W, 3, 1, 1, 0, rs.pre + ".in_layers.2", h1max);
                    cfd::launch_colsum(dh1, (int64_t)in.H * in.W, rs.cout, B, cpart, crow, st);
                    const std::string ek = rs.pre + ".emb_layers.1";
                    cfd::launch_linear_wgrad(crow, pg->emb, B, h->tdim, rs.cout, 1, GP(ek + ".weight"),
                                             GP(ek + ".bias"), st);
                    const float* W_emb = h->emb_w + (size_t)h->params[h->index.at(ek + ".weight")].emb_row * h->tdim;
                    cfd::launch_linear_dgrad(crow, W_emb, pg->emb, B, h->tdim, rs.cout, 1, 1, demb, st);
                }
                dconv(dh1, rs.cout, in.H, in.W, rs.pre + ".in_layers.2.weight", in.C(), in.H, in.W, 3, 1, 1, 0, G);
                const float* addsrc = dout;
                if (rs.cin != rs.cout) {
                    if (pg) wgrad(dout, rs.cout, in, nullptr, 0, in.H, in.W, 1, 1, 0, 0, rs.pre + ".skip_connection", omax);
                    float* sk = gfree(dout, G, dh1);
                    dconv(dout, rs.cout, in.H, in.W, rs.pre + ".skip_connection.weight", in.C(), in.H, in.W, 1, 1, 0,
                          0, sk);
                    addsrc = sk;
                }
                float* dx = dh1;
                unsigned* xm = slot();
                gnb(in, r.ss1, r.st1, rs.pre + ".in_layers.0", 1, G, addsrc, dx,
                    in.b ? dhs[r.skip_hs] : nullptr, true, xm);
                dcur = Act{dx, in.Ca, nullptr, 0, in.H, in.W};
                dmax = xm;
                break;
            }
            case cfd::Step::Attn: {
                const auto& at = h->attn[s.idx];
                const int T = in.H * in.W;
                const float* dout = dcur.a;
                float* dA = gfree(dout);
                if (pg)
                    wgrad(dout, at.C, Act{r.o, at.C, nullptr, 0, in.H, in.W}, nullptr, 0, in.H, in.W, 1, 1, 0, 0,
                          at.pre + ".proj_out", dmax);
                dconv(dout, at.C, in.H, in.W, at.pre + ".proj_out.weight", at.C, in.H, in.W, 1, 1, 0, 0, dA);
                cfd::AttnBwdArgs ab{r.qkv, r.o, dA, r.lse, dd, dqkv, T, at.C,
                                    (float)(1.0 / std::sqrt(std::sqrt((double)at.ch)))};
                if (h->compute == CFD_COMPUTE_SPLIT_F16 && cfd::attention_bwd_split_ok(T, at.ch)) {
                    CFD_REQUIRE(cfd::attention_bwd_split_floats(T, at.C) <= z.max_abw, CFD_ESTATE,
                                "internal: attention backward workspace");
                    cfd::launch_attention_bwd_split(ab, at.ch, at.heads, B, abws, st);
                } else {
                    cfd::launch_attention_bwd(ab, at.ch, at.heads, B, st);
                }
                if (pg) {
                    if (r.act1)
                        wgrad(dqkv, 3 * at.C, Act{r.act1, at.C, nullptr, 0, in.H, in.W}, nullptr, 0, in.H, in.W, 1, 1, 0,
                              0, at.pre + ".qkv", nullptr, r.amx1);
                    else
                        wgrad(dqkv, 3 * at.C, in, r.ss1, 0, in.H, in.W, 1, 1, 0, 0, at.pre + ".qkv");
                }
                float* dxn = gfree(dout, dA);
                dconv(dqkv, 3 * at.C, in.H, in.W, at.pre + ".qkv.weight", at.C, in.H, in.W, 1, 1, 0, 0, dxn);
                unsigned* am = slot();
                gnb(in, r.ss1, r.st1, at.pre + ".norm", 0, dxn, dout, dA, nullptr, true, am);
                dcur = Act{dA, at.C, nullptr, 0, in.H, in.W};
                dmax = am;
                break;
            }
            case cfd::Step::In: {
                if (pg) {
                    wgrad(dcur.a, dcur.Ca, Act{pg->x, c.in_channels, nullptr, 0, S, S}, nullptr, 0, S, S, 3, 1, 1, 0,
                          s.conv, dmax);
                    cfd::launch_linear_wgrad(demb, pg->th1, B, h->tdim, h->tdim, 1, GP("time_embed.2.weight"),
                                             GP("time_embed.2.bias"), st);
                    cfd::launch_linear_dgrad(demb, P(h, "time_embed.2.weight"), pg->th1, B, h->tdim, h->tdim, 1, 0,
                                             dth1, st);
                    cfd::launch_linear_wgrad(dth1, pg->temb, B, c.model_channels, h->tdim, 0,
                                             GP("time_embed.0.weight"), GP("time_embed.0.bias"), st);
                }
                if (!d_x) break;
                cfd::ConvArgs a{};
                a.src1 = dcur.a;
                a.C1 = dcur.Ca;
                a.Ctot = dcur.Ca;
                a.w = PT(h, s.conv + ".weight");
                a.out = d_x;
                a.Hin = a.Hout = S;
                a.Win = a.Wout = S;
                a.Cout = c.in_channels;
                a.M = B * S * S;
                a.K = 9 * dcur.Ca;
                a.tmode = 1;
                cfd::launch_conv_out(a, st);
                break;
            }
        }
    }
}

}

extern "C" int cfd_unet_create(const cfd_unet_cfg* cfg, int device, cfd_unet** out) {
    return cfd::guard([&] {
        CFD_REQUIRE(cfg && out, CFD_EARG, "null argument");
        CFD_REQUIRE(cfg->n_mult >= 1 && cfg->n_mult <= 8 && cfg->n_attn >= 0 && cfg->n_attn <= 8, CFD_EARG,
                    "bad channel_mult / attention list");
        CFD_REQUIRE(cfg->model_channels > 0 && cfg->model_channels % 32 == 0, CFD_EARG,
                    "model_channels must be a positive multiple of 32");
        CFD_REQUIRE(cfg->in_channels >= 1 && cfg->in_channels <= 4 && cfg->out_channels >= 1 &&
                        cfg->out_channels <= 4,
                    CFD_EARG, "in/out channels must be 1..4");
        const int levels_down = cfg->n_mult - 1;
        CFD_REQUIRE(cfg->image_size > 0 && (cfg->image_size >> levels_down) << levels_down == cfg->image_size,
                    CFD_EARG, "image_size must be divisible by 2^(len(channel_mult)-1)");
        cfd::DeviceGuard dg(device);
        auto* h = new cfd_unet();
        h->cfg = *cfg;
        h->device = device;
        try {
            build(h);
            CFD_HIP(hipMalloc(&h->arena, sizeof(float) * h->arena_floats));
            CFD_HIP(hipMalloc(&h->emb_w, sizeof(float) * (size_t)h->emb_total * h->tdim));
            CFD_HIP(hipMalloc(&h->emb_b, sizeof(float) * (size_t)h->emb_total));
            CFD_HIP(hipMalloc(&h->arena_t, sizeof(float) * std::max<size_t>(h->arena_t_floats, 4)));
            CFD_HIP(hipMalloc(&h->arena_bf, sizeof(uint16_t) * std::max<size_t>(h->arena_floats, 4)));
            CFD_HIP(hipMalloc(&h->arena_hi, sizeof(uint16_t) * std::max<size_t>(h->arena_floats, 4)));
            CFD_HIP(hipMalloc(&h->arena_lo, sizeof(uint16_t) * std::max<size_t>(h->arena_floats, 4)));
            CFD_HIP(hipMalloc(&h->arena_thi, sizeof(uint16_t) * std::max<size_t>(h->arena_t_floats, 4)));
            CFD_HIP(hipMalloc(&h->arena_tlo, sizeof(uint16_t) * std::max<size_t>(h->arena_t_floats, 4)));
            const int half = cfg->model_channels / 2;
            std::vector<float> fr(half);
            const float nl = (float)(-std::log(10000.0));
            for (int i = 0; i < half; ++i) fr[i] = std::exp((nl * (float)i) / (float)half);
            CFD_HIP(hipMalloc(&h->freqs, sizeof(float) * std::max(half, 1)));
            CFD_HIP(hipMalloc(&h->nonfinite, sizeof(int)));
            CFD_HIP(hipMemset(h->nonfinite, 0, sizeof(int)));
            CFD_HIP(hipMemcpy(h->freqs, fr.data(), sizeof(float) * half, hipMemcpyHostToDevice));
        } catch (...) {
            cfd_unet_destroy(h);
            throw;
        }
        *out = h;
    });
}

extern "C" void cfd_unet_destroy(cfd_unet* h) {
    if (!h) return;
    (void)hipFree(h->arena);
    (void)hipFree(h->emb_w);
    (void)hipFree(h->emb_b);
    (void)hipFree(h->freqs);
    (void)hipFree(h->arena_t);
    (void)hipFree(h->arena_bf);
    (void)hipFree(h->arena_hi);
    (void)hipFree(h->arena_lo);
    (void)hipFree(h->arena_thi);
    (void)hipFree(h->arena_tlo);
    (void)hipFree(h->nonfinite);
    (void)hipFree(h->rp_desc);
    (void)hipFree(h->rp_first);
    (void)hipFree(h->rp_part);
    (void)hipFree(h->rp_amax);
    (void)hipFree(h->rp_tfirst);
    delete h;
}

extern "C" int cfd_unet_num_params(const cfd_unet* h, int* n) {
    return cfd::guard([&] {
        CFD_REQUIRE(h && n, CFD_EARG, "null argument");
        *n = (int)h->params.size();
    });
}

extern "C" int cfd_unet_param_info(const cfd_unet* h, int idx, const char** key, int* ndim, int64_t shape[4]) {
    return cfd::guard([&] {
        CFD_REQUIRE(h && idx >= 0 && idx < (int)h->params.size(), CFD_EARG, "bad index");
        const auto& p = h->params[idx];
        if (key) *key = p.key.c_str();
        if (ndim) *ndim = (int)p.shape.size();
        if (shape)
            for (size_t i = 0; i < p.shape.size(); ++i) shape[i] = p.shape[i];
    });
}

extern "C" int cfd_unet_set_param(cfd_unet* h, const char* key, const float* host, size_t n) {
    return cfd::guard([&] {
        CFD_REQUIRE(h && key && host, CFD_EARG, "null argument");
        auto it = h->index.find(key);
        CFD_REQUIRE(it != h->index.end(), CFD_EKEY, std::string("unknown U-Net parameter key: ") + key);
        auto& p = h->params[it->second];
        CFD_REQUIRE(n == p.count, CFD_ESHAPE, std::string("size mismatch for ") + key);
        cfd::DeviceGuard dg(h->device);
        switch (p.pack) {
            case Pack::Raw:
                CFD_HIP(hipMemcpy(h->arena + p.offset, host, n * 4, hipMemcpyHostToDevice));
                break;
            case Pack::Conv1:
            case Pack::Conv3: {
                std::vector<float> pk(host, host + n);
                if (p.pack == Pack::Conv3) {
                    const int64_t co = p.shape[0], ci = p.shape[1];
                    for (int64_t o = 0; o < co; ++o)
                        for (int64_t i = 0; i < ci; ++i)
                            for (int tap = 0; tap < 9; ++tap)
                                pk[(o * 9 + tap) * ci + i] = host[(o * ci + i) * 9 + tap];
                }
                CFD_HIP(hipMemcpy(h->arena + p.offset, pk.data(), n * 4, hipMemcpyHostToDevice));
                std::vector<uint16_t> bf(n);
                for (size_t e = 0; e < n; ++e) bf[e] = to_bf16(pk[e]);
                CFD_HIP(hipMemcpy(h->arena_bf + p.offset, bf.data(), n * 2, hipMemcpyHostToDevice));
                float amax = 0.f;
                for (size_t e = 0; e < n; ++e) amax = std::max(amax, std::fabs(pk[e]));
                int ex = 0;
                if (amax > 0.f) std::frexp(amax, &ex);
                const float s = std::ldexp(1.0f, -ex);
                p.split_inv = std::ldexp(1.0f, ex);
                std::vector<_Float16> hi(n), lo(n);
                for (size_t e = 0; e < n; ++e) {
                    const float v = pk[e] * s;
                    hi[e] = (_Float16)v;
                    lo[e] = (_Float16)(v - (float)hi[e]);
                }
                CFD_HIP(hipMemcpy(h->arena_hi + p.offset, hi.data(), n * 2, hipMemcpyHostToDevice));
                CFD_HIP(hipMemcpy(h->arena_lo + p.offset, lo.data(), n * 2, hipMemcpyHostToDevice));
                break;
            }
            case Pack::EmbW:
                CFD_HIP(hipMemcpy(h->emb_w + (size_t)p.emb_row * h->tdim, host, n * 4, hipMemcpyHostToDevice));
                break;
            case Pack::EmbB:
                CFD_HIP(hipMemcpy(h->emb_b + p.emb_row, host, n * 4, hipMemcpyHostToDevice));
                break;
        }
        if (p.tpack) {
            const int64_t co = p.shape[0], ci = p.shape[1];
            const int taps = (int)(p.count / (size_t)(co * ci));
            std::vector<float> pk(p.tpack == 2 ? (size_t)ci * 16 * co : n);
            if (p.tpack == 1 || p.tpack == 3) {
                for (int64_t o = 0; o < co; ++o)
                    for (int64_t i = 0; i < ci; ++i)
                        for (int tap = 0; tap < taps; ++tap)
                            pk[((size_t)i * taps + (p.tpack == 3 ? taps - 1 - tap : tap)) * co + o] =
                                host[((size_t)o * ci + i) * taps + tap];
            } else {
                static const int dlo[4] = {2, 1, 0, 0}, dhi[4] = {2, 2, 1, 0};
                for (int64_t o = 0; o < co; ++o)
                    for (int64_t i = 0; i < ci; ++i)
                        for (int ey = 0; ey < 4; ++ey)
                            for (int ex = 0; ex < 4; ++ex) {
                                float v = 0.f;
                                for (int dy = dlo[ey]; dy <= dhi[ey]; ++dy)
                                    for (int dx = dlo[ex]; dx <= dhi[ex]; ++dx)
                                        v += host[((size_t)o * ci + i) * 9 + dy * 3 + dx];
                                pk[((size_t)i * 16 + ey * 4 + ex) * co + o] = v;
                            }
            }
            CFD_HIP(hipMemcpy(h->arena_t + p.toffset, pk.data(), pk.size() * 4, hipMemcpyHostToDevice));
            float amax = 0.f;
            for (float v : pk) amax = std::max(amax, std::fabs(v));
            int ex = 0;
            if (amax > 0.f) std::frexp(amax, &ex);
            const float sc = std::ldexp(1.0f, -ex);
            p.tsplit_inv = std::ldexp(1.0f, ex);
            std::vector<_Float16> thi(pk.size()), tlo(pk.size());
            for (size_t e = 0; e < pk.size(); ++e) {
                const float v = pk[e] * sc;
                thi[e] = (_Float16)v;
                tlo[e] = (_Float16)(v - (float)thi[e]);
            }
            CFD_HIP(hipMemcpy(h->arena_thi + p.toffset, thi.data(), pk.size() * 2, hipMemcpyHostToDevice));
            CFD_HIP(hipMemcpy(h->arena_tlo + p.toffset, tlo.data(), pk.size() * 2, hipMemcpyHostToDevice));
        }
        p.set = true;
        ++h->version;
    });
}

namespace cfd {
constexpr int RP_CHUNK = 4096;

struct RepackDesc {
    int64_t src, count, off, toff, tcount;
    int pack, tpack, co, ci, taps, emb_row;
};

__device__ __forceinline__ int rp_param(const int64_t* __restrict__ first, int np, int64_t blk) {
    int lo = 0, hi = np;
    while (hi - lo > 1) {
        const int mid = (lo + hi) >> 1;
        if (first[mid] <= blk) lo = mid; else hi = mid;
    }
    return lo;
}

__device__ __forceinline__ float rp_up_value(const float* __restrict__ w, const RepackDesc& d, int64_t e) {
    const int64_t o = e % d.co, r = e / d.co;
    const int q = (int)(r % 16);
    const int64_t i = r / 16;
    const int ey = q >> 2, ex = q & 3;
    const int dlo_y = ey == 0 ? 2 : ey == 1 ? 1 : 0, dhi_y = ey == 0 ? 2 : ey == 1 ? 2 : ey == 2 ? 1 : 0;
    const int dlo_x = ex == 0 ? 2 : ex == 1 ? 1 : 0, dhi_x = ex == 0 ? 2 : ex == 1 ? 2 : ex == 2 ? 1 : 0;
    const float* base = w + (o * d.ci + i) * 9;
    float v = 0.f;
    for (int dy = dlo_y; dy <= dhi_y; ++dy)
        for (int dx = dlo_x; dx <= dhi_x; ++dx) v += base[dy * 3 + dx];
    return v;
}

__global__ __launch_bounds__(256) void rp_amax_kernel(const float* __restrict__ flat,
                                                      const RepackDesc* __restrict__ desc,
                                                      const int64_t* __restrict__ first, int np,
                                                      float* __restrict__ part) {
    const int64_t blk = blockIdx.x;
    const int p = rp_param(first, np, blk);
    const RepackDesc d = desc[p];
    const float* w = flat + d.src;
    const int64_t e0 = (blk - first[p]) * RP_CHUNK;
    float m0 = 0.f, m1 = 0.f;
    for (int64_t e = e0 + threadIdx.x; e < e0 + RP_CHUNK; e += 256) {
        if (e < d.count) m0 = fmaxf(m0, fabsf(w[e]));
        if (d.tpack == 2 && e < d.tcount) m1 = fmaxf(m1, fabsf(rp_up_value(w, d, e)));
    }
    __shared__ float r0[256], r1[256];
    r0[threadIdx.x] = m0;
    r1[threadIdx.x] = m1;
    __syncthreads();
    for (int s = 128; s > 0; s >>= 1) {
        if (threadIdx.x < s) {
            r0[threadIdx.x] = fmaxf(r0[threadIdx.x], r0[threadIdx.x + s]);
            r1[threadIdx.x] = fmaxf(r1[threadIdx.x], r1[threadIdx.x + s]);
        }
        __syncthreads();
    }
    if (threadIdx.x == 0) {
        part[blk * 2] = r0[0];
        part[blk * 2 + 1] = d.tpack == 2 ? r1[0] : r0[0];
    }
}

__global__ __launch_bounds__(256) void rp_reduce_kernel(const float* __restrict__ part,
                                                        const int64_t* __restrict__ first, float* __restrict__ amax) {
    const int p = blockIdx.x;
    float m0 = 0.f, m1 = 0.f;
    for (int64_t b = first[p] + threadIdx.x; b < first[p + 1]; b += 256) {
        m0 = fmaxf(m0, part[b * 2]);
        m1 = fmaxf(m1, part[b * 2 + 1]);
    }
    __shared__ float r0[256], r1[256];
    r0[threadIdx.x] = m0;
    r1[threadIdx.x] = m1;
    __syncthreads();
    for (int s = 128; s > 0; s >>= 1) {
        if (threadIdx.x < s) {
            r0[threadIdx.x] = fmaxf(r0[threadIdx.x], r0[threadIdx.x + s]);
            r1[threadIdx.x] = fmaxf(r1[threadIdx.x], r1[threadIdx.x + s]);
        }
        __syncthreads();
    }
    if (threadIdx.x == 0) {
        amax[p * 2] = r0[0];
        amax[p * 2 + 1] = r1[0];
    }
}

__device__ __forceinline__ uint16_t rp_bf16(float f) {
    const uint32_t u = __float_as_uint(f);
    if ((u & 0x7fffffffu) > 0x7f800000u) return (uint16_t)((u >> 16) | 0x40u);
    return (uint16_t)((u + 0x7fffu + ((u >> 16) & 1u)) >> 16);
}

__device__ __forceinline__ float rp_scale(float amax) {
    if (!(amax > 0.f)) return 1.f;
    int ex;
    frexpf(amax, &ex);
    return ldexpf(1.f, -ex);
}

__device__ __forceinline__ void rp_split(float v, float s, _Float16* hi, _Float16* lo, int64_t i) {
#pragma clang fp contract(off)
    const float x = v * s;
    const _Float16 h = (_Float16)x;
    hi[i] = h;
    lo[i] = (_Float16)(x - (float)h);
}

__global__ __launch_bounds__(256) void rp_pack_kernel(const float* __restrict__ flat,
                                                      const RepackDesc* __restrict__ desc,
                                                      const int64_t* __restrict__ first, int np,
                                                      const float* __restrict__ amax, float* __restrict__ arena,
                                                      uint16_t* __restrict__ arena_bf, _Float16* __restrict__ arena_hi,
                                                      _Float16* __restrict__ arena_lo, float* __restrict__ arena_t,
                                                      _Float16* __restrict__ arena_thi,
                                                      _Float16* __restrict__ arena_tlo, float* __restrict__ emb_w,
                                                      float* __restrict__ emb_b, int tdim) {
    const int64_t blk = blockIdx.x;
    const int p = rp_param(first, np, blk);
    const RepackDesc d = desc[p];
    const float* w = flat + d.src;
    const int64_t e0 = (blk - first[p]) * RP_CHUNK;
    const float s = rp_scale(amax[p * 2]), ts = rp_scale(amax[p * 2 + 1]);
    const bool conv = d.pack == (int)Pack::Conv1 || d.pack == (int)Pack::Conv3;
    for (int64_t e = e0 + threadIdx.x; e < e0 + RP_CHUNK; e += 256) {
        if (e < d.count) {
            if (d.pack == (int)Pack::Raw) {
                arena[d.off + e] = w[e];
            } else if (d.pack == (int)Pack::EmbW) {
                emb_w[(int64_t)d.emb_row * tdim + e] = w[e];
            } else if (d.pack == (int)Pack::EmbB) {
                emb_b[d.emb_row + e] = w[e];
            } else {
                int64_t src = e;
                if (d.pack == (int)Pack::Conv3) {
                    const int64_t i = e % d.ci, ot = e / d.ci, tap = ot % 9, o = ot / 9;
                    src = (o * d.ci + i) * 9 + tap;
                }
                const float v = w[src];
                arena[d.off + e] = v;
                arena_bf[d.off + e] = rp_bf16(v);
                rp_split(v, s, arena_hi, arena_lo, d.off + e);
            }
        }
        (void)conv;
        (void)ts;
    }
}

constexpr int RP_TI = 8;
__global__ __launch_bounds__(256) void rp_tpack_kernel(const float* __restrict__ flat,
                                                       const RepackDesc* __restrict__ desc,
                                                       const int64_t* __restrict__ tfirst, int np,
                                                       const float* __restrict__ amax, float* __restrict__ arena_t,
                                                       _Float16* __restrict__ arena_thi,
                                                       _Float16* __restrict__ arena_tlo) {
    const int64_t blk = blockIdx.x;
    const int p = rp_param(tfirst, np, blk);
    const RepackDesc d = desc[p];
    const float* w = flat + d.src;
    const int64_t tile = blk - tfirst[p];
    const int nti = (d.ci + RP_TI - 1) / RP_TI;
    const int o0 = (int)(tile / nti) * 64, i0 = (int)(tile % nti) * RP_TI;
    const int taps = d.taps, run = RP_TI * taps, ld = run + 1;
    __shared__ float tl[64 * (RP_TI * 9 + 1)];
    for (int e = threadIdx.x; e < 64 * run; e += 256) {
        const int ol = e / run, c = e - ol * run;
        const int o = o0 + ol, i = i0 + c / taps;
        tl[ol * ld + c] = o < d.co && i < d.ci ? w[((int64_t)o * d.ci + i0) * taps + c] : 0.f;
    }
    __syncthreads();
    const float ts = rp_scale(amax[p * 2 + 1]);
    const int ol = threadIdx.x & 63, o = o0 + ol;
    const int nq = d.tpack == 2 ? 16 : taps;
    if (o < d.co) {
        for (int r = threadIdx.x >> 6; r < RP_TI * nq; r += 4) {
            const int il = r / nq, q = r - il * nq, i = i0 + il;
            if (i >= d.ci) break;
            const float* src = tl + ol * ld + il * taps;
            float v;
            if (d.tpack == 2) {
                const int ey = q >> 2, ex = q & 3;
                const int dlo_y = ey == 0 ? 2 : ey == 1 ? 1 : 0, dhi_y = ey == 0 ? 2 : ey == 1 ? 2 : ey == 2 ? 1 : 0;
                const int dlo_x = ex == 0 ? 2 : ex == 1 ? 1 : 0, dhi_x = ex == 0 ? 2 : ex == 1 ? 2 : ex == 2 ? 1 : 0;
                v = 0.f;
                for (int dy = dlo_y; dy <= dhi_y; ++dy)
                    for (int dx = dlo_x; dx <= dhi_x; ++dx) v += src[dy * 3 + dx];
            } else {
                v = src[d.tpack == 3 ? taps - 1 - q : q];
            }
            const int64_t e = ((int64_t)i * nq + q) * d.co + o;
            arena_t[d.toff + e] = v;
            rp_split(v, ts, arena_thi, arena_tlo, d.toff + e);
        }
    }
}
}

extern "C" int cfd_unet_load_flat(cfd_unet* h, const float* flat, size_t n, void* stream) {
    return cfd::guard([&] {
        CFD_REQUIRE(h && flat, CFD_EARG, "null argument");
        const int np = (int)h->params.size();
        size_t total = 0;
        for (const auto& p : h->params) total += p.count;
        CFD_REQUIRE(n == total, CFD_ESHAPE, "flat buffer size differs from the parameter count");
        cfd::DeviceGuard dg(h->device);
        hipStream_t st = (hipStream_t)stream;
        if (!h->rp_desc) {
            std::vector<cfd::RepackDesc> desc(np);
            std::vector<int64_t> first(np + 1);
            int64_t src = 0, blocks = 0;
            for (int k = 0; k < np; ++k) {
                const auto& p = h->params[k];
                cfd::RepackDesc d{};
                d.src = src;
                d.count = (int64_t)p.count;
                d.off = (int64_t)p.offset;
                d.toff = (int64_t)p.toffset;
                d.pack = (int)p.pack;
                d.tpack = p.tpack;
                d.emb_row = p.emb_row;
                d.co = p.shape.size() > 1 ? (int)p.shape[0] : 1;
                d.ci = p.shape.size() > 1 ? (int)p.shape[1] : 1;
                d.taps = (int)(d.count / std::max<int64_t>(1, (int64_t)d.co * d.ci));
                d.tcount = p.tpack == 2 ? (int64_t)d.ci * 16 * d.co : d.count;
                if (p.tpack == 2) CFD_REQUIRE(d.taps == 9, CFD_ESTATE, "internal: upsample pack needs 3x3");
                desc[k] = d;
                first[k] = blocks;
                blocks += std::max<int64_t>(1, cfd::ceil_div(std::max(d.count, d.tcount), cfd::RP_CHUNK));
                src += d.count;
            }
            first[np] = blocks;
            std::vector<int64_t> tfirst(np + 1);
            int64_t tiles = 0;
            for (int k = 0; k < np; ++k) {
                const auto& d = desc[k];
                const bool conv = d.pack == (int)Pack::Conv1 || d.pack == (int)Pack::Conv3;
                tfirst[k] = tiles;
                if (conv && d.tpack) {
                    CFD_REQUIRE(d.taps <= 9 && (int64_t)d.co * d.ci * d.taps == d.count, CFD_ESTATE,
                                "internal: input-gradient pack shape");
                    tiles += cfd::ceil_div(d.co, 64) * cfd::ceil_div(d.ci, cfd::RP_TI);
                }
            }
            tfirst[np] = tiles;
            CFD_HIP(hipMalloc(&h->rp_tfirst, sizeof(int64_t) * (np + 1)));
            CFD_HIP(hipMemcpy(h->rp_tfirst, tfirst.data(), sizeof(int64_t) * (np + 1), hipMemcpyHostToDevice));
            h->rp_tiles = tiles;
            CFD_HIP(hipMalloc(&h->rp_desc, sizeof(cfd::RepackDesc) * np));
            CFD_HIP(hipMalloc(&h->rp_first, sizeof(int64_t) * (np + 1)));
            CFD_HIP(hipMalloc(&h->rp_part, sizeof(float) * 2 * blocks));
            CFD_HIP(hipMalloc(&h->rp_amax, sizeof(float) * 2 * np));
            CFD_HIP(hipMemcpy(h->rp_desc, desc.data(), sizeof(cfd::RepackDesc) * np, hipMemcpyHostToDevice));
            CFD_HIP(hipMemcpy(h->rp_first, first.data(), sizeof(int64_t) * (np + 1), hipMemcpyHostToDevice));
            h->rp_blocks = blocks;
        }
        const auto* desc = (const cfd::RepackDesc*)h->rp_desc;
        hipLaunchKernelGGL(cfd::rp_amax_kernel, dim3((unsigned)h->rp_blocks), dim3(256), 0, st, flat, desc,
                           h->rp_first, np, h->rp_part);
        cfd::check_launch("rp_amax_kernel");
        hipLaunchKernelGGL(cfd::rp_reduce_kernel, dim3(np), dim3(256), 0, st, h->rp_part, h->rp_first, h->rp_amax);
        cfd::check_launch("rp_reduce_kernel");
        hipLaunchKernelGGL(cfd::rp_pack_kernel, dim3((unsigned)h->rp_blocks), dim3(256), 0, st, flat, desc,
                           h->rp_first, np, h->rp_amax, h->arena, h->arena_bf, (_Float16*)h->arena_hi,
                           (_Float16*)h->arena_lo, h->arena_t, (_Float16*)h->arena_thi, (_Float16*)h->arena_tlo,
                           h->emb_w, h->emb_b, h->tdim);
        cfd::check_launch("rp_pack_kernel");
        if (h->rp_tiles) {
            hipLaunchKernelGGL(cfd::rp_tpack_kernel, dim3((unsigned)h->rp_tiles), dim3(256), 0, st, flat, desc,
                               h->rp_tfirst, np, h->rp_amax, h->arena_t, (_Float16*)h->arena_thi,
                               (_Float16*)h->arena_tlo);
            cfd::check_launch("rp_tpack_kernel");
        }
        std::vector<float> amax(2 * (size_t)np);
        CFD_HIP(hipMemcpyAsync(amax.data(), h->rp_amax, sizeof(float) * 2 * np, hipMemcpyDeviceToHost, st));
        CFD_HIP(hipStreamSynchronize(st));
        for (int k = 0; k < np; ++k) {
            auto& p = h->params[k];
            if (p.pack == Pack::Conv1 || p.pack == Pack::Conv3) {
                int ex = 0;
                if (amax[2 * k] > 0.f) std::frexp(amax[2 * k], &ex);
                p.split_inv = std::ldexp(1.0f, ex);
            }
            if (p.tpack) {
                int ex = 0;
                if (amax[2 * k + 1] > 0.f) std::frexp(amax[2 * k + 1], &ex);
                p.tsplit_inv = std::ldexp(1.0f, ex);
            }
            p.set = true;
        }
        ++h->version;
    });
}

extern "C" int cfd_unet_set_compute(cfd_unet* h, int compute) {
    return cfd::guard([&] {
        CFD_REQUIRE(h, CFD_EARG, "null handle");
        CFD_REQUIRE(compute == CFD_COMPUTE_F32 || compute == CFD_COMPUTE_BF16 || compute == CFD_COMPUTE_SPLIT_F16,
                    CFD_EARG, "unknown compute mode");
        if (h->compute != compute) ++h->version;
        h->compute = compute;
    });
}

extern "C" int cfd_unet_set_plan_batch(cfd_unet* h, int nominal_batch) {
    return cfd::guard([&] {
        CFD_REQUIRE(h, CFD_EARG, "null handle");
        CFD_REQUIRE(nominal_batch >= 0 && nominal_batch <= 64, CFD_EARG, "plan batch must be 0 (default) .. 64");
        if (h->plan_b != nominal_batch) {
            ++h->version;
            h->ws_cache.clear();
        }
        h->plan_b = nominal_batch;
    });
}

extern "C" int cfd_unet_set_time_freqs(cfd_unet* h, const float* host, int n) {
    return cfd::guard([&] {
        CFD_REQUIRE(h && host && n == h->cfg.model_channels / 2, CFD_EARG, "freqs must have model_channels/2 entries");
        cfd::DeviceGuard dg(h->device);
        CFD_HIP(hipMemcpy(h->freqs, host, sizeof(float) * n, hipMemcpyHostToDevice));
    });
}

extern "C" int cfd_unet_ready(const cfd_unet* h) {
    return cfd::guard([&] {
        CFD_REQUIRE(h, CFD_EARG, "null handle");
        for (const auto& p : h->params) CFD_REQUIRE(p.set, CFD_ESTATE, "U-Net parameter not set: " + p.key);
    });
}

namespace cfd {
size_t unet_ws_bytes(const cfd_unet* h, int B) {
    auto it = h->ws_cache.find(B);
    if (it != h->ws_cache.end()) return it->second;
    Workspace ws{nullptr, 0, true};
    run(h, nullptr, nullptr, nullptr, B, ws, nullptr);
    h->ws_cache[B] = ws.off + 256;
    return ws.off + 256;
}
void unet_check_ready(const cfd_unet* h) {
    for (const auto& p : h->params) CFD_REQUIRE(p.set, CFD_ESTATE, "U-Net parameter not set: " + p.key);
}
int unet_compute(const cfd_unet* h) { return h->compute; }
uint64_t unet_version(const cfd_unet* h) { return h->version; }
int unet_device(const cfd_unet* h) { return h->device; }
int* unet_nonfinite(const cfd_unet* h) { return h->nonfinite; }
void unet_forward_raw(const cfd_unet* h, const float* x, const int64_t* t, float* eps, int B, void* workspace,
                      hipStream_t st) {
    Workspace ws{(char*)(((uintptr_t)workspace + 255) & ~uintptr_t(255)), 0, false};
    run(h, x, t, eps, B, ws, st);
}
}

extern "C" int cfd_unet_workspace_bytes(const cfd_unet* h, int B, size_t* bytes) {
    return cfd::guard([&] {
        CFD_REQUIRE(h && bytes && B > 0, CFD_EARG, "bad argument");
        *bytes = cfd::unet_ws_bytes(h, B);
    });
}

extern "C" int cfd_unet_forward(cfd_unet* h, const float* x, const int64_t* t, float* eps, int B, void* workspace,
                                size_t ws_bytes, void* stream) {
    return cfd::guard([&] {
        CFD_REQUIRE(h && x && t && eps && workspace, CFD_EARG, "null argument");
        CFD_REQUIRE(B > 0, CFD_EARG, "B must be positive");
        cfd::unet_check_ready(h);
        CFD_REQUIRE(ws_bytes >= cfd::unet_ws_bytes(h, B), CFD_EARG, "workspace too small");
        cfd::unet_forward_raw(h, x, t, eps, B, workspace, (hipStream_t)stream);
    });
}

namespace {
size_t tape_bytes_mode(const cfd_unet* h, int B, int mode) {
    Workspace ws{nullptr, 0, true}, tws{nullptr, 0, true};
    Tape tape{&tws, nullptr};
    tape.keep_gnout = mode == CFD_TAPE_PARAM_GRAD;
    run(h, nullptr, nullptr, nullptr, B, ws, nullptr, &tape, false);
    return tws.off + 256;
}
}

extern "C" int cfd_unet_tape_bytes(const cfd_unet* h, int B, size_t* bytes) {
    return cfd::guard([&] {
        CFD_REQUIRE(h && bytes && B > 0, CFD_EARG, "bad argument");
        *bytes = tape_bytes_mode(h, B, h->tape_mode);
    });
}

namespace {
constexpr size_t kMaxTapes = 64;

const cfd_unet::TapeRec& tape_rec(const cfd_unet* h, const void* tape, int B, size_t tape_bytes) {
    auto it = h->tapes.find(tape);
    CFD_REQUIRE(it != h->tapes.end(), CFD_ESTATE,
                "tape was not recorded by cfd_unet_forward_tape on this handle (or was forgotten: at most 64 live "
                "tapes per handle)");
    CFD_REQUIRE(it->second.B == B, CFD_EARG, "B differs from the batch the tape was recorded at");
    CFD_REQUIRE(it->second.plan == plan_batch(h), CFD_ESTATE,
                "the planned batch changed since the tape was recorded (cfd_unet_set_plan_batch)");
    CFD_REQUIRE(tape_bytes >= tape_bytes_mode(h, B, it->second.mode), CFD_EARG, "tape too small");
    return it->second;
}
}

extern "C" int cfd_unet_set_tape_mode(cfd_unet* h, int mode) {
    return cfd::guard([&] {
        CFD_REQUIRE(h, CFD_EARG, "null handle");
        CFD_REQUIRE(mode == CFD_TAPE_INPUT_VJP || mode == CFD_TAPE_PARAM_GRAD, CFD_EARG, "unknown tape mode");
        h->tape_mode = mode;
    });
}

extern "C" int cfd_unet_vjp_workspace_bytes(const cfd_unet* h, int B, size_t* bytes) {
    return cfd::guard([&] {
        CFD_REQUIRE(h && bytes && B > 0, CFD_EARG, "bad argument");
        Workspace ws{nullptr, 0, true};
        std::vector<Rec> none;
        run_vjp(h, nullptr, nullptr, B, none, ws, nullptr);
        *bytes = ws.off + 256;
    });
}

namespace {
char* align256(void* p) { return (char*)(((uintptr_t)p + 255) & ~uintptr_t(255)); }

void check_ready(const cfd_unet* h) {
    for (const auto& p : h->params) CFD_REQUIRE(p.set, CFD_ESTATE, "U-Net parameter not set: " + p.key);
}
}

extern "C" int cfd_unet_forward_tape(cfd_unet* h, const float* x, const int64_t* t, float* eps, int B,
                                     void* workspace, size_t ws_bytes, void* tape, size_t tape_bytes, void* stream) {
    return cfd::guard([&] {
        CFD_REQUIRE(h && x && t && eps && workspace && tape, CFD_EARG, "null argument");
        CFD_REQUIRE(h->compute != CFD_COMPUTE_BF16, CFD_ESTATE,
                    "the input-gradient path is fp32-accurate: call cfd_unet_set_compute(h, CFD_COMPUTE_F32) "
                    "or CFD_COMPUTE_SPLIT_F16 first");
        CFD_REQUIRE(B > 0, CFD_EARG, "B must be positive");
        check_ready(h);
        size_t need = 0;
        cfd_unet_workspace_bytes(h, B, &need);
        CFD_REQUIRE(ws_bytes >= need, CFD_EARG, "workspace too small");
        CFD_REQUIRE(tape_bytes >= tape_bytes_mode(h, B, h->tape_mode), CFD_EARG, "tape too small");
// ... 84 lines not shown
```

confild_amd/csrc/unet_kernels.hip:

```cpp
#include <algorithm>
#include <cstdlib>

#include "unet_kernels.hpp"

namespace cfd {

__global__ __launch_bounds__(256) void gn_partial_kernel(GnArgs a) {
    const int chunk = blockIdx.x;
    const int64_t b = blockIdx.y;
    const int Ctot = a.Ctot, cq = Ctot / 4, cpg = Ctot / 32;
    const int HW = a.HW;
    const int p0 = (int)((int64_t)HW * chunk / a.nchunks), p1 = (int)((int64_t)HW * (chunk + 1) / a.nchunks);
    const int rows = 256 / cq;
    const int q = threadIdx.x % cq, r0 = threadIdx.x / cq;
    __shared__ double red[2][1024];
    if (r0 < rows) {
        double s[4] = {0, 0, 0, 0}, s2[4] = {0, 0, 0, 0};
        const int c0 = 4 * q;
        for (int p = p0 + r0; p < p1; p += rows) {
            const int64_t pix = b * HW + p;
            const f4 v = c0 < a.C1 ? *(const f4*)(a.src1 + pix * a.C1 + c0)
                                   : *(const f4*)(a.src2 + pix * a.C2 + (c0 - a.C1));
#pragma unroll
            for (int j = 0; j < 4; ++j) {
// ... 1502 lines not shown
                const int k = 4 * (lane + 64 * i);
                if (k < K) {
                    const f4 v = *(const f4*)(xs + bb * K + k);
                    s = fmaf(w[i][0], v[0], s);
                    s = fmaf(w[i][1], v[1], s);
                    s = fmaf(w[i][2], v[2], s);
                    s = fmaf(w[i][3], v[3], s);
                }
            }
            for (int o = 32; o > 0; o >>= 1) s += __shfl_xor(s, o);
            if (lane == 0) y[(int64_t)(b0 + bb) * N + n] = s + bn;
        }
    }
}

int gn_chunks(int HW) {
    const int64_t small = std::min<int64_t>(64, HW / 16);
    return (int)std::max<int64_t>(1, std::min<int64_t>(kGnMaxChunks, std::max<int64_t>(HW / 64, small)));
}

static unsigned long long* g_stamps = nullptr;
void stamps_set(unsigned long long* buf) { g_stamps = buf; }
unsigned long long* stamps_buf() { return g_stamps; }
static int g_seq = 0;

static int env_int(const char* name, int dflt) {
    const char* e = getenv(name);
    return e ? atoi(e) : dflt;
}

bool gn2_applies(const GnArgs& a) {
    const int pb = a.plan_b > 0 ? a.plan_b : 8;
    return (int64_t)a.HW * 8 >= (int64_t)4096 * pb && a.Ctot % 4 == 0 && a.C1 % 4 == 0 && a.C2 % 4 == 0 &&
           a.Ctot <= 1024;
}

static int gn_reg_ipt(const GnArgs& a) {
    return a.Ctot % 128 == 0 ? (int)ceil_div(a.HW, 512 / (a.Ctot / 128)) : 0;
}

bool gn_takes_splitk(const GnArgs& a, int B) {
    (void)B;
    if (gn2_applies(a)) return a.C1 % 4 == 0;
    if (a.Ctot % 128 != 0 || a.C1 % 4 != 0) return false;
    return gn_reg_ipt(a) <= 16;
}

void launch_gn(const GnArgs& a0, int B, hipStream_t st) {
    CFD_REQUIRE(a0.Ctot % 32 == 0 && a0.C1 % 4 == 0 && a0.C2 % 4 == 0 && a0.Ctot <= 1024, CFD_ESHAPE,
                "GroupNorm32 needs channels % 32 == 0 (<= 1024)");
    GnArgs a = a0;
    a.nchunks = gn_chunks(a.HW);
    a.B = B;
    a.stamps = g_stamps;
    a.seq = g_seq++;
    CFD_REQUIRE(!a.kpart || gn_takes_splitk(a, B), CFD_ESTATE, "internal: split-K source on a GroupNorm path without it");
    if (gn2_applies(a)) {
        CFD_REQUIRE(!a.kpart || a.kx, CFD_ESTATE, "internal: gn2 needs the split-K sum's destination");
        a.nchunks = gn2_chunks(a.HW, a.plan_b);
        if (gn2_threads(a.nchunks) == 1024) {
            hipLaunchKernelGGL(gn2_stats_kernel<1024>, dim3(a.nchunks, B), dim3(1024), 0, st, a);
            check_launch("gn2_stats_kernel");
            hipLaunchKernelGGL(gn2_apply_kernel<1024>, dim3(a.nchunks, B), dim3(1024), 0, st, a);
        } else {
            hipLaunchKernelGGL(gn2_stats_kernel<256>, dim3(a.nchunks, B), dim3(256), 0, st, a);
            check_launch("gn2_stats_kernel");
            hipLaunchKernelGGL(gn2_apply_kernel<256>, dim3(a.nchunks, B), dim3(256), 0, st, a);
        }
        check_launch("gn2_apply_kernel");
        return;
    }
    const int ipt = gn_reg_ipt(a);
    if (ipt > 0 && ipt <= 32) {
        const dim3 grid((unsigned)(32 * B));
        const int nq = a.Ctot / 128, r256 = 256 / nq, i256 = (a.HW + r256 - 1) / r256;
        if (i256 <= 4) {
            if (i256 <= 1)
                hipLaunchKernelGGL((gn_fused_reg_kernel<1, 256>), grid, dim3(256), 0, st, a);
            else if (i256 <= 2)
                hipLaunchKernelGGL((gn_fused_reg_kernel<2, 256>), grid, dim3(256), 0, st, a);
            else
                hipLaunchKernelGGL((gn_fused_reg_kernel<4, 256>), grid, dim3(256), 0, st, a);
            check_launch("gn_fused_reg_kernel");
            return;
        }
        if (ipt <= 4)
            hipLaunchKernelGGL((gn_fused_reg_kernel<2, 1024>), grid, dim3(1024), 0, st, a);
        else if (ipt <= 8)
            hipLaunchKernelGGL((gn_fused_reg_kernel<4, 1024>), grid, dim3(1024), 0, st, a);
        else if (ipt <= 16)
            hipLaunchKernelGGL((gn_fused_reg_kernel<8, 1024>), grid, dim3(1024), 0, st, a);
        else
            hipLaunchKernelGGL(gn_fused_reg_kernel<32>, grid, dim3(512), 0, st, a);
        check_launch("gn_fused_reg_kernel");
        return;
    }
    hipLaunchKernelGGL(gn_partial_kernel, dim3(a.nchunks, B), dim3(256), 0, st, a);
    check_launch("gn_partial_kernel");
    hipLaunchKernelGGL(gn_finalize_kernel, dim3(B), dim3(1024), 0, st, a);
    check_launch("gn_finalize_kernel");
    const int64_t nq = (int64_t)B * a.HW * a.Ctot / 4;
    hipLaunchKernelGGL(gn_apply_kernel, dim3((unsigned)std::min<int64_t>(4096, ceil_div(nq, 256))), dim3(256), 0, st, a);
    check_launch("gn_apply_kernel");
}


static int even_splits(int nch, int splits) {
    if (splits <= 1) return 1;
    const int per = (nch + splits - 1) / splits;
    return (nch + per - 1) / per;
}

constexpr int64_t kK1pMin128 = 144, kK1pMin64 = 192;

ConvPlan plan_conv(const ConvArgs& a, size_t part_cap_floats) {
    const int plan_b = a.plan_b > 0 ? a.plan_b : 8;
    ConvPlan p;
    const int64_t mn = (int64_t)plan_b * a.Hout * a.Wout;
    p.bn = a.Cout >= 128 ? 128 : 64;
    auto tiles = [&](int bm) { return ceil_div(mn, bm) * ceil_div(a.Cout, p.bn); };
    p.bm = 64;
    int wg_per_tile = 1;
    if (p.bn == 128) {
        p.bm = 128;
        p.nw = 8;
        wg_per_tile = 2;
    }
    const int nkt = a.K / 32;
    p.splits = 1;
    while (tiles(p.bm) * wg_per_tile * p.splits < 768 && nkt / (p.splits * 2) >= 4 && p.splits < 16)
        p.splits *= 2;
    if (a.ks == 1 && !a.tmode && tiles(p.bm) >= 128) p.splits = 1;
    while (p.splits > 1 && (size_t)p.splits * mn * a.Cout > part_cap_floats) p.splits /= 2;
    if (conv_p_applies(a) && !(ceil_div(mn, 32) * ceil_div(a.Cout, 64) < 32 && a.K >= 1024)) {
        ConvPlan q;
        const int64_t t128 = ceil_div(mn, 128) * ceil_div(a.Cout, 128), t64 = ceil_div(mn, 64) * ceil_div(a.Cout, 64);
        q.kx = t128 >= kK1pMin128 ? 40 : t64 >= kK1pMin64 ? 41 : 42;
        conv_p_tile(q.kx, q.bm, q.bn, q.nw);
        q.splits = 1;
        return q;
    }
    if (a.wlo && a.ks == 3 && a.stride == 1 && !a.tmode && a.Ctot <= 128 && (int64_t)a.Hout * a.Wout >= 36864)
        return p;
    const int64_t srows = mn / ((int64_t)a.Hout * a.Wout) * a.Hin * a.Win;
    const bool fits32 = srows < (1 << 23) && srows * std::max(a.C1, a.C2) * 4 < (1ll << 30) &&
                        (int64_t)a.Cout * a.K * 2 < (1ll << 31);
    auto halo_splits = [&](int64_t t) {
        const int nch = a.Ctot / 32;
        int sp = 1;
        while (t * sp < 256 && sp * 2 <= nch && sp < 16) sp *= 2;
        while (sp > 1 && (size_t)sp * mn * a.Cout > part_cap_floats) sp /= 2;
        return even_splits(nch, sp);
    };
    if (a.wbf && !a.wlo && !a.tmode && a.ks == 3 && a.stride == 1 && a.Cout >= 128 && fits32 && conv_h_tw(a) > 0) {
        ConvPlan q;
        q.kx = 22;
        q.bm = 256;
        q.bn = 128;
        q.nw = 8;
        q.splits = halo_splits(ceil_div(mn, 256) * ceil_div(a.Cout, 128));
        return q;
    }
    if (a.wbf && a.wlo && !a.tmode && a.ks == 3 && a.stride == 1 && a.Cout >= 128 && fits32) {
        ConvPlan q;
        if (conv_h_tw(a) > 0) {
            q.kx = 20;
            q.bm = 256;
            q.bn = 128;
            q.nw = 8;
            q.splits = halo_splits(ceil_div(mn, 256) * ceil_div(a.Cout, 128));
            return q;
        }
        q.kx = mn >= 2048 ? 2 : 1;
        q.bm = q.kx == 2 ? 256 : 128;
        q.bn = 128;
        q.nw = q.kx == 2 ? 8 : 4;
        const int64_t t = ceil_div(mn, q.bm) * ceil_div(a.Cout, q.bn);
        q.splits = 1;
        while (t * q.splits < 256 && nkt / (q.splits * 2) >= 4 && q.splits < 32) q.splits *= 2;
        while (q.splits > 1 && (size_t)q.splits * mn * a.Cout > part_cap_floats) q.splits /= 2;
        return q;
    }
    return p;
}

int smalln_below() {
    const int v = env_int("CFD_CONV_SMALLN", 1);
    return v == 1 ? 128 : std::max(v, 0);
}

template <bool TMODE, int MODE, bool BUFA>
static void launch_conv_tiles_(const ConvArgs& a, const ConvPlan& p, dim3 grid, hipStream_t st) {
    if constexpr (MODE != 0 && BUFA) {
        static const int smalln = smalln_below();
        if (!TMODE && p.nw == 8 && p.bm == 128 && p.bn == 128 && (int64_t)grid.x * grid.y * grid.z < smalln &&
            a.Cout % 64 == 0) {
            const dim3 g64(grid.x, (unsigned)ceil_div(a.Cout, 64), grid.z);
            hipLaunchKernelGGL((conv_gemm_kernel<128, 64, false, MODE, 8, true>), g64, dim3(512), 0, st, a);
            return;
        }
        if (p.nw == 8 && p.bm == 128 && p.bn == 128 && p.pf == 2) {
            hipLaunchKernelGGL((conv_gemm_kernel<128, 128, TMODE, MODE, 8, true, 2>), grid, dim3(512), 0, st, a);
            return;
        }
        if (p.nw == 8 && p.bm == 128 && p.bn == 128 && p.pf == 3) {
            hipLaunchKernelGGL((conv_gemm_kernel<128, 128, TMODE, MODE, 8, true, 3>), grid, dim3(512), 0, st, a);
            return;
        }
    }
    if (p.nw == 8 && p.bm == 128 && p.bn == 128)
        hipLaunchKernelGGL((conv_gemm_kernel<128, 128, TMODE, MODE, 8, BUFA>), grid, dim3(512), 0, st, a);
    else if (p.bm == 128 && p.bn == 128)
        hipLaunchKernelGGL((conv_gemm_kernel<128, 128, TMODE, MODE, 4, BUFA>), grid, dim3(256), 0, st, a);
    else if (p.bm == 64 && p.bn == 128)
        hipLaunchKernelGGL((conv_gemm_kernel<64, 128, TMODE, MODE, 4, BUFA>), grid, dim3(256), 0, st, a);
    else if (p.bm == 128 && p.bn == 64)
        hipLaunchKernelGGL((conv_gemm_kernel<128, 64, TMODE, MODE, 4, BUFA>), grid, dim3(256), 0, st, a);
    else
        hipLaunchKernelGGL((conv_gemm_kernel<64, 64, TMODE, MODE, 4, BUFA>), grid, dim3(256), 0, st, a);
}

template <bool TMODE, int MODE>
static void launch_conv_tiles(const ConvArgs& a, const ConvPlan& p, dim3 grid, hipStream_t st) {
    if (a.bufaddr) return launch_conv_tiles_<TMODE, MODE, true>(a, p, grid, st);
    launch_conv_tiles_<TMODE, MODE, false>(a, p, grid, st);
}

void launch_splitk_reduce(const ConvArgs& a, int splits, hipStream_t st) {
    const int64_t total4 = (int64_t)a.M * a.Cout / 4;
    hipLaunchKernelGGL(splitk_reduce_kernel, dim3((unsigned)ceil_div(total4, 256)), dim3(256), 0, st, a, splits);
    check_launch("splitk_reduce_kernel");
}

static bool conv_x_falls_back(const ConvArgs& a) {
    static const int force_k1s = env_int("CFD_CONV_FORCE_K1S", 0);
    const int64_t srows = (int64_t)a.Hin * a.Win * (a.M / (a.Hout * a.Wout));
    return force_k1s || !(srows < (1 << 24) && a.M < (1 << 24) && srows * std::max(a.C1, a.C2) * 4 < (1ll << 31));
}

static bool conv_p_falls_back(const ConvArgs& a) {
    return !conv_p_applies(a) || (int64_t)a.Cout * a.K * 2 >= (1ll << 31);
}

bool conv_runs_k1hb(const ConvArgs& a, const ConvPlan& p) { return p.kx == 22 && !conv_x_falls_back(a); }

bool conv_kv_pack_ok(const ConvArgs& a, const ConvPlan& p, int T) {
    static const int ldsepi = env_int("CFD_CONV_LDSEPI", 1);
    return ldsepi && (p.kx < 0 || p.kx >= 40) && p.splits == 1 && a.wbf && !a.tmode && a.ks == 1 && a.bias &&
           !a.emb && !a.res && a.Cout % 8 == 0 && a.emb_stride % 4 == 0 && T % 32 == 0 && a.M % T == 0;
}

int launch_conv(const ConvArgs& a, const ConvPlan& p0, hipStream_t st, bool defer) {
    ConvPlan p = p0;
    if (p.kx >= 0 && (conv_x_falls_back(a) || (p.kx >= 40 && conv_p_falls_back(a)))) {
        p.kx = -1;
        p.bm = p.bn = 128;
        p.nw = 8;
    }
    CFD_REQUIRE(!a.src_bf16 || p.kx == 22, CFD_ESTATE, "internal: a bf16 convolution source needs the K1hb kernel");
    static const int pf = env_int("CFD_CONV_PF", 2);
    if (p.kx < 0) p.pf = pf >= 1 && pf <= 3 ? pf : 1;
    CFD_REQUIRE(a.Ctot % 32 == 0 && a.C1 % 4 == 0 && a.C2 % 4 == 0, CFD_ESHAPE, "conv_gemm needs channels % 32 == 0");
    CFD_REQUIRE(a.K == a.ks * a.ks * a.Ctot, CFD_ESHAPE, "conv K mismatch");
    CFD_REQUIRE(p.splits == 1 || (a.part && a.Cout % 4 == 0), CFD_ESTATE, "split-K needs a partial buffer");
    CFD_REQUIRE(!a.tmode || ((a.stride == 1 || a.stride == 2) && !a.up), CFD_ESHAPE, "transposed conv: stride 1|2");
    const dim3 grid((unsigned)ceil_div(a.M, p.bm), (unsigned)ceil_div(a.Cout, p.bn), p.splits);
    CFD_REQUIRE(!(a.tmode && a.wbf && !a.wlo), CFD_ESTATE, "bf16 input-gradient convolutions are not built");
    static const int xcd = env_int("CFD_CONV_XCD", 4);
    static const int ldsepi = env_int("CFD_CONV_LDSEPI", 1);
    ConvArgs b = a;
    b.stamps = g_stamps;
    b.seq = g_seq++;
    b.ldsepi = ldsepi && a.Cout % 4 == 0 && a.emb_stride % 4 == 0;
    const int xo = xcd == 4 ? (a.wbf && !a.wlo ? 1 : 3) : xcd;
    b.xcd = xo == 3 ? ((int64_t)a.Hout * a.Wout <= 256 ? 2 : 1) : xo < 0 || xo > 2 ? 1 : xo;
    {
        const int64_t srows = (int64_t)a.Hin * a.Win * (a.M / (a.Hout * a.Wout));
        const int64_t wes = (a.wbf || a.wlo) ? 2 : 4;
        b.bufaddr = a.ks * a.ks <= 9 && srows < (1 << 24) && a.M < (1 << 24) &&
                    srows * std::max(a.C1, a.C2) * 4 < (1ll << 31) && (int64_t)a.Cout * a.K * wes < (1ll << 31);
    }
    const ConvArgs& a_ = b;
    if (p.kx >= 40) {
        CFD_REQUIRE(p.splits == 1, CFD_ESTATE, "internal: K1p does not split over K");
        launch_conv_p(a_, p.kx, st);
        return 1;
    }
    if (p.kx >= 0) {
        launch_conv_x(a_, p.kx, p.splits, st);
        if (p.splits > 1 && !defer) launch_splitk_reduce(a, p.splits, st);
        return p.splits;
    }
    if (a.tmode && a.wlo)
        launch_conv_tiles<true, 2>(a_, p, grid, st);
    else if (a.tmode)
        launch_conv_tiles<true, 0>(a_, p, grid, st);
    else if (a.wbf && a.wlo)
        launch_conv_tiles<false, 2>(a_, p, grid, st);
    else if (a.wbf)
        launch_conv_tiles<false, 1>(a_, p, grid, st);
    else
        launch_conv_tiles<false, 0>(a_, p, grid, st);
    check_launch("conv_gemm_kernel");
    if (p.splits > 1 && !defer) launch_splitk_reduce(a, p.splits, st);
    return p.splits;
}
// ... 143 lines not shown
```

confild_amd/csrc/unet_kernels.hpp:

```cpp
#pragma once
#include "common.hpp"

namespace cfd {

struct GnArgs {
    const float* src1;
    const float* src2;
    const float* gamma;
    const float* beta;
    double* part;
    float* ss;
    float* out;
    float* stats;
    int C1, C2, Ctot, HW;
    float eps;
    int silu;
    int nchunks;
    int B;
    const float* kpart;
    const float* kbias;
    const float* kemb;
    const float* kres;
    float* kx;
    int ksplits, kemb_stride;
    unsigned long long* stamps;
    int seq;
    int out_bf16;
    unsigned* amax_out;
    int plan_b;
};

struct ConvArgs {
    const float* src1;
    const float* src2;
    const float* w;
    const void* wbf;
    const void* wlo;
    float acc_scale;
    const float* bias;
    const float* emb;
    const float* res;
    float* out;
    float* part;
    int C1, C2, Ctot;
    int Hin, Win, Hout, Wout;
    int stride, ks, pad, up;
    int tmode;
    int Cout;
    int emb_stride;
    int M, K;
    int xcd;
    int bufaddr;
    int ldsepi;
    int* nonfinite;
    int src_bf16;
    void* kvf;
    int64_t kv_voff;
    int kv_ch, kv_heads, kv_T;
    float kv_scale;
    unsigned long long* stamps;
    int seq;
    int plan_b;
};
void stamps_set(unsigned long long* buf);
unsigned long long* stamps_buf();

struct AttnArgs {
    const float* qkv;
    float* out;
    int T, C;
    float scale;
    float* lse;
    int xcdmap;
    int kc;
    float* part;
};

struct GnbArgs {
    const float* x1;
    const float* x2;
    const float* dz;
    const float* ss;
    const float* stats;
    const float* gamma;
    const float* addsrc;
    float* out1;
    float* out2;
    int acc1, acc2;
    double* part;
    float* fin;
    float* ppart;
    unsigned* amax_out;
    int C1, C2, Ctot, HW, silu, nchunks, B;
    int plan_b;
};

struct AttnBwdArgs {
    const float* qkv;
    const float* o;
    const float* dout;
    const float* lse;
    float* dd;
    float* dqkv;
    int T, C;
    float scale;
    h8v* packs;
    float* amax;
    int heads, xcdmap;
};

struct ConvPlan {
    int bm = 128, bn = 128, splits = 1;
    int nw = 4;
    int kx = -1;
    int pf = 1;
};

constexpr int kGnMaxChunks = 512;
int gn_chunks(int HW);
constexpr int kGn2BigHW = 16384, kGn2BigChunks = 256;
static_assert(kGn2BigChunks <= kGnMaxChunks, "gn2 partials live in the kGnMaxChunks slab");
int gn2_chunks(int HW, int plan_b);
inline int gn2_threads(int nchunks) { return nchunks > 64 ? 1024 : 256; }
void launch_gn(const GnArgs& a, int B, hipStream_t st);
bool gn_takes_splitk(const GnArgs& a, int B);
bool gn2_applies(const GnArgs& a);
ConvPlan plan_conv(const ConvArgs& a, size_t part_cap_floats);
int launch_conv(const ConvArgs& a, const ConvPlan& p, hipStream_t st, bool defer = false);
void launch_splitk_reduce(const ConvArgs& a, int splits, hipStream_t st);
__device__ __forceinline__ void xcd_tile(int order, int& bx, int& by, int& bz) {
    bx = blockIdx.x;
    by = blockIdx.y;
    bz = blockIdx.z;
    if (!order) return;
    const unsigned gx = gridDim.x, gy = gridDim.y, gz = gridDim.z;
    const unsigned T = gx * gy * gz, L = blockIdx.x + gx * (blockIdx.y + gy * blockIdx.z);
    const unsigned q = T >> 3, r = T & 7, x = L & 7, sl = L >> 3;
    const unsigned Lp = x < r ? x * (q + 1) + sl : r * (q + 1) + (x - r) * q + sl;
    if (order == 2) {
        bx = Lp % gx;
        bz = (Lp / gx) % gz;
        by = Lp / (gx * gz);
    } else {
        bz = Lp % gz;
        by = (Lp / gz) % gy;
        bx = Lp / (gz * gy);
    }
}
int launch_conv_x(const ConvArgs& a, int variant, int splits, hipStream_t st);
int conv_h_tw(const ConvArgs& a);
bool conv_p_applies(const ConvArgs& a);
void conv_p_tile(int variant, int& bm, int& bn, int& nw);
void launch_conv_p(const ConvArgs& a, int variant, hipStream_t st);
int smalln_below();
bool conv_runs_k1hb(const ConvArgs& a, const ConvPlan& p);
void launch_conv_in(const ConvArgs& a, hipStream_t st);
void launch_conv_out(const ConvArgs& a, hipStream_t st);
void launch_attention(const AttnArgs& a, int CH, int heads, int B, hipStream_t st);
size_t attention_split_floats(int T, int C);
int attention_kv_chunks(int T, int heads, int plan_b);
size_t attention_part_floats(int T, int C, int CH, int plan_b);
void launch_attention_split(const AttnArgs& a, int CH, int heads, int B, int plan_b, float* kvws, hipStream_t st,
                            bool packed);
int64_t attention_split_voff(int T, int CH, int heads, int B);
bool conv_kv_pack_ok(const ConvArgs& a, const ConvPlan& p, int T);
int launch_gn_bwd(const GnbArgs& a, int B, hipStream_t st);
void launch_attention_bwd(const AttnBwdArgs& a, int CH, int heads, int B, hipStream_t st);
size_t attention_bwd_split_floats(int T, int C);
bool attention_bwd_split_ok(int T, int CH);
void launch_attention_bwd_split(const AttnBwdArgs& a, int CH, int heads, int B, float* ws, hipStream_t st);
void launch_add(float* y, const float* x, int64_t n, hipStream_t st);
void launch_temb(const int64_t* t, const float* freqs, float* out, int dim, int B, hipStream_t st);
void launch_linear(const float* x, const float* W, const float* bias, float* y, int B, int K, int N, int act,
                   hipStream_t st);


__device__ __forceinline__ float kln2(float scale) { return scale * 1.44269504088896340736f; }
__device__ __forceinline__ void split8_f16(const float (&v)[8], h8v& hi, h8v& lo) {
#pragma clang fp contract(off)
#pragma unroll
    for (int t = 0; t < 8; ++t) {
        hi[t] = (_Float16)v[t];
        lo[t] = (_Float16)(v[t] - (float)hi[t]);
    }
}
constexpr int vmcnt_wait(int n) { return (n & 15) | (7 << 4) | (15 << 8) | (((n >> 4) & 3) << 14); }
}
```

include/confild.h:

```cpp
#ifndef CONFILD_H
#define CONFILD_H

#include <stddef.h>
#include <stdint.h>

#ifdef __cplusplus
extern "C" {
#endif

enum { CFD_OK = 0, CFD_EARG = 1, CFD_EHIP = 2, CFD_EKEY = 3, CFD_ESHAPE = 4, CFD_ESTATE = 5 };

const char* cfd_last_error(void);
const char* cfd_version(void);

typedef struct cfd_unet cfd_unet;

typedef struct {
    int image_size;
    int in_channels;
    int model_channels;
    int out_channels;
    int num_res_blocks;
    int n_mult;
    int channel_mult[8];
    int n_attn;
    int attention_ds[8];
    int num_heads;
    int num_head_channels;
} cfd_unet_cfg;

int  cfd_unet_create(const cfd_unet_cfg* cfg, int device, cfd_unet** out);
void cfd_unet_destroy(cfd_unet* h);
int  cfd_unet_num_params(const cfd_unet* h, int* n);
int  cfd_unet_param_info(const cfd_unet* h, int idx, const char** key, int* ndim, int64_t shape[4]);
int  cfd_unet_set_param(cfd_unet* h, const char* key, const float* host_data, size_t n);
int  cfd_unet_set_time_freqs(cfd_unet* h, const float* host_freqs, int n);
int  cfd_unet_ready(const cfd_unet* h);
int  cfd_unet_load_flat(cfd_unet* h, const float* flat, size_t n, void* stream);
int  cfd_unet_workspace_bytes(const cfd_unet* h, int B, size_t* bytes);
#define CFD_COMPUTE_F32       0
#define CFD_COMPUTE_BF16      1
#define CFD_COMPUTE_SPLIT_F16 2
int  cfd_unet_set_compute(cfd_unet* h, int compute);
int  cfd_unet_set_plan_batch(cfd_unet* h, int nominal_batch);
int  cfd_unet_forward(cfd_unet* h, const float* x, const int64_t* t, float* eps, int B,
                      void* workspace, size_t ws_bytes, void* stream);
int  cfd_unet_check_finite(cfd_unet* h, int* nonfinite, void* stream);

int  cfd_unet_tape_bytes(const cfd_unet* h, int B, size_t* bytes);
int  cfd_unet_vjp_workspace_bytes(const cfd_unet* h, int B, size_t* bytes);
int  cfd_unet_forward_tape(cfd_unet* h, const float* x, const int64_t* t, float* eps, int B,
                           void* workspace, size_t ws_bytes, void* tape, size_t tape_bytes, void* stream);
int  cfd_unet_input_vjp(cfd_unet* h, const float* d_eps, float* d_x, int B, const void* tape,
                        size_t tape_bytes, void* workspace, size_t ws_bytes, void* stream);
#define CFD_TAPE_INPUT_VJP  0
#define CFD_TAPE_PARAM_GRAD 1
int  cfd_unet_set_tape_mode(cfd_unet* h, int mode);

typedef struct cfd_sched cfd_sched;
enum { CFD_COEF_SRA = 0, CFD_COEF_SRM1, CFD_COEF_M1, CFD_COEF_M2, CFD_COEF_SIGMA,
       CFD_COEF_SQRT_ABP, CFD_COEF_DIR, CFD_COEF_SIGMA_DDIM, CFD_NCOEF };
enum { CFD_STEP_DDPM = 0, CFD_STEP_DDIM = 1 };

int  cfd_sched_create(const float* host_coefs, int n_t, int device, cfd_sched** out);
void cfd_sched_destroy(cfd_sched* s);
int  cfd_sched_step(const cfd_sched* s, int kind, int clip, const float* x, const float* eps,
                    const int64_t* t, const float* noise, uint64_t seed, uint64_t counter,
                    uint64_t offset, float* x_out, float* xstart_out, int64_t n_per_sample, int B,
                    void* stream);
int  cfd_sched_step_known(const cfd_sched* s, int kind, int clip, const float* x, const float* eps,
                          const int64_t* t, const float* noise, uint64_t seed, uint64_t counter,
                          uint64_t offset, float* x_out, float* xstart_out, int64_t n_per_sample, int B,
                          const float* known, int64_t known_bstride, const float* mask, int64_t mask_bstride,
                          const float* table, const float* noise2, uint64_t counter2, void* stream);
int  cfd_sched_step_jump(const cfd_sched* s, int kind, int clip, const float* x, const float* eps,
                         const int64_t* t, const float* noise, uint64_t seed, uint64_t counter,
                         uint64_t offset, float* x_out, float* xstart_out, int64_t n_per_sample, int B,
                         const float* known, int64_t known_bstride, const float* mask, int64_t mask_bstride,
                         const float* table, const float* noise2, uint64_t counter2, float ja, float jb,
                         const float* noise3, uint64_t counter3, void* stream);
typedef struct cfd_sampler cfd_sampler;
int  cfd_sampler_create(const cfd_unet* unet, const cfd_sched* sched, int kind, int clip, int B,
                        int64_t n_per_sample, int n_steps, const int64_t* host_tidx, const int64_t* host_tmodel,
                        int graph, int unroll, cfd_sampler** out);
void cfd_sampler_destroy(cfd_sampler* sp);
int  cfd_device_cu_count(int device, int* n_cu);
int  cfd_stream_create_cu_range(int device, int first_cu, int n_cu, void** stream);
int  cfd_stream_destroy(void* stream);
int  cfd_sampler_run(cfd_sampler* sp, const float* x_in, float* x_out, int k0, int k1, uint64_t seed,
                     uint64_t offset, void* stream);
int  cfd_sampler_set_known(cfd_sampler* sp, const float* known, int64_t known_bstride, const float* mask,
                           int64_t mask_bstride, const float* table, void* stream);
int  cfd_sampler_captures(const cfd_sampler* sp, uint64_t* n);
int  cfd_sampler_set_jumps(cfd_sampler* sp, const float* host_jtab);
int  cfd_randn(float* out, int64_t n, uint64_t seed, uint64_t counter, uint64_t offset, void* stream);
int  cfd_sine_probe(const float* x, float* y, int64_t n, int which, void* stream);
int  cfd_latent_denorm(const float* x, float* y, int64_t n, const float* vmax, const float* vmin,
                       int64_t period, void* stream);

int  cfd_dps_residual(const float* y, int64_t y_batch_stride, const float* A, float* g_A, float* norm,
                      int64_t n_per_sample, int B, void* stream);
int  cfd_dps_latent_grad(const cfd_sched* s, int clip, const float* x, const float* eps, const int64_t* t,
                         const float* g_z, const float* vmax, const float* vmin, int64_t period,
                         float* d_eps, float* g_direct, int64_t n_per_sample, int B, void* stream);
int  cfd_dps_update(const float* sample, const float* g_direct, const float* g_unet, float scale,
                    float* x_out, int64_t n, void* stream);
int  cfd_dps_update_known(const float* sample, const float* g_direct, const float* g_unet, float scale,
                          float* x_out, const int64_t* t, int64_t n_per_sample, int B, const float* known,
                          int64_t known_bstride, const float* mask, int64_t mask_bstride, const float* table,
                          const float* noise2, uint64_t seed, uint64_t counter2, uint64_t offset, void* stream);
int  cfd_dps_latent_residual_workspace_bytes(int64_t n_per_sample, int B, size_t* bytes);
int  cfd_dps_latent_residual(const cfd_sched* s, int clip, const float* x, const float* eps, const int64_t* t,
                             const float* y, int64_t y_bstride, const float* mask, int64_t mask_bstride,
                             float* norm, float* d_eps, float* g_direct, int64_t n_per_sample, int B,
                             void* workspace, size_t ws_bytes, void* stream);

typedef struct cfd_siren cfd_siren;

typedef struct {
    int in_coord_features;
    int in_latent_features;
    int out_features;
    int num_hidden_layers;
    int hidden_features;
    float w0;
} cfd_siren_cfg;

int  cfd_siren_create(const cfd_siren_cfg* cfg, int device, cfd_siren** out);
void cfd_siren_destroy(cfd_siren* h);
int  cfd_siren_num_params(const cfd_siren* h, int* n);
int  cfd_siren_param_info(const cfd_siren* h, int idx, const char** key, int* ndim, int64_t shape[4]);
int  cfd_siren_set_param(cfd_siren* h, const char* key, const float* host_data, size_t n);
int  cfd_siren_ready(const cfd_siren* h);
int  cfd_siren_workspace_bytes(const cfd_siren* h, int b, size_t* bytes);
#define CFD_SIREN_F32       0
#define CFD_SIREN_SPLIT_F16 1
int  cfd_siren_set_compute(cfd_siren* h, int compute);
int  cfd_siren_get_compute(const cfd_siren* h, int* compute);
int  cfd_siren_forward(cfd_siren* h, const float* coords, int64_t N, const float* latents, int b,
                       const float* xmax, const float* xmin,
                       const float* ymax, const float* ymin, int64_t y_stride,
                       float* out, void* workspace, size_t ws_bytes, void* stream);
int  cfd_siren_jacobian_workspace_bytes(const cfd_siren* h, int b, size_t* bytes);
int  cfd_siren_forward_jacobian(cfd_siren* h, const float* coords, int64_t N, const float* latents, int b,
                                const float* xmax, const float* xmin,
                                const float* ymax, const float* ymin, int64_t y_stride,
                                float* out, float* jac,
                                void* workspace, size_t ws_bytes, void* stream);
int  cfd_siren_forward_jacobian_split(cfd_siren* h, const float* coords, int64_t N, const float* latents, int b,
                                      const float* xmax, const float* xmin,
                                      const float* ymax, const float* ymin, int64_t y_stride,
                                      float* out, float* jac,
                                      void* workspace, size_t ws_bytes, void* stream);
int  cfd_siren_hessian_workspace_bytes(const cfd_siren* h, int b, size_t* bytes);
int  cfd_siren_forward_hessian(cfd_siren* h, const float* coords, int64_t N, const float* latents, int b,
                               const float* xmax, const float* xmin,
                               const float* ymax, const float* ymin, int64_t y_stride,
                               float* out, float* jac, float* hess, int diag_only,
                               void* workspace, size_t ws_bytes, void* stream);
int  cfd_siren_forward_hessian_split(cfd_siren* h, const float* coords, int64_t N, const float* latents, int b,
                                     const float* xmax, const float* xmin,
                                     const float* ymax, const float* ymin, int64_t y_stride,
                                     float* out, float* jac, float* hess, int diag_only,
                                     void* workspace, size_t ws_bytes, void* stream);

int  cfd_siren_vjp_workspace_bytes(const cfd_siren* h, int64_t Ns, int R, size_t* bytes);
int  cfd_siren_tape_forward(cfd_siren* h, const float* coords, int64_t Ns, const float* latents, int R,
                            const float* xmax, const float* xmin,
                            const float* ymax, const float* ymin, int64_t y_stride,
                            float* out, void* workspace, size_t ws_bytes, void* stream);
int  cfd_siren_tape_vjp(cfd_siren* h, const float* g_out, int64_t Ns, int R,
                        const float* ymax, const float* ymin, int64_t y_stride,
                        float* g_latents, void* workspace, size_t ws_bytes, void* stream);

int  cfd_siren_jtape_workspace_bytes(const cfd_siren* h, int64_t Ns, int R, size_t* bytes);
int  cfd_siren_jtape_forward(cfd_siren* h, const float* coords, int64_t Ns, const float* latents, int R,
                             const float* xmax, const float* xmin,
                             const float* ymax, const float* ymin, int64_t y_stride,
                             float* out, float* jac, void* workspace, size_t ws_bytes, void* stream);
int  cfd_siren_jtape_vjp(cfd_siren* h, const float* g_out, const float* g_jac, int64_t Ns, int R,
                         const float* ymax, const float* ymin, int64_t y_stride,
                         float* g_latents, void* workspace, size_t ws_bytes, void* stream);
int  cfd_dps_residual_linear(const float* y, int y_per_sample, const float* out, const float* jac,
                             const float* wv, int wv_per_sensor, const float* wj, int wj_per_sensor,
                             float* g_out, float* g_jac, float* norm, float* A, int64_t Ns, int M, int c,
                             int d, int rows_per_sample, int B, void* stream);

#define CFD_DENSE_SLAB 64
#define CFD_DENSE_DEFAULT_BUDGET ((size_t)1 << 30)
int  cfd_siren_dense_plan(const cfd_siren_cfg* cfg, int64_t N, int R, size_t budget, int bwd_form,
                          int compute_form, size_t* bytes, int64_t* chunk_points, int* block_rows);
int  cfd_siren_dense_workspace_bytes(const cfd_siren* h, int64_t N, int R, size_t budget, size_t* bytes);
int  cfd_siren_dense_grad(cfd_siren* h, const float* coords, int64_t N,
                          const float* latents, int R, int rows_per_sample,
                          const float* xmax, const float* xmin,
                          const float* ymax, const float* ymin, int64_t y_stride,
                          const float* y, int y_rows,
                          const float* mask, int mask_rows,
                          float* g_latents, float* norm,
                          void* workspace, size_t ws_bytes, size_t budget, void* stream);
// ... 28 lines not shown
```

Measured before the change: 4.141.

## Decompose nearest-upsample 3x3 convolutions into four 2x2 phase convolutions

Nearest-2x upsample followed by a 3x3 conv is rewritten as four sub-pixel phase convolutions, each with 2x2 folded weights applied on the low-resolution input. This cuts the MACs for these convs from 9 taps to 4 per output pixel. The phase weights are prepacked in split-f16 with per-phase scales, and conv_x and conv_h kernels gain a phase template path with strided output writes. It also adds a barrier in the SIREN kernel and a standalone upsample-conv entry point for testing, and changes the precision characteristics of the summed weights.

Result: faster. 4.198 (median of 6 runs) (+1.4%).

```diff
diff --git a/confild_amd/_lib.py b/confild_amd/_lib.py
--- a/confild_amd/_lib.py
+++ b/confild_amd/_lib.py
@@ -50,6 +50,8 @@
     "cfd_stream_create_cu_range": (C.c_int, [C.c_int, C.c_int, C.c_int, C.POINTER(C.c_void_p)]),
     "cfd_stream_destroy": (C.c_int, [C.c_void_p]),
     "cfd_unet_check_finite": (C.c_int, [C.c_void_p, C.POINTER(C.c_int), C.c_void_p]),
+    "cfd_upsample_conv": (C.c_int, [C.c_void_p, C.c_void_p, C.c_void_p, C.c_void_p, C.c_int, C.c_int, C.c_int,
+                                    C.c_int, C.c_int, C.c_int, C.c_int, C.POINTER(C.c_int), C.c_void_p]),
     "cfd_unet_workspace_bytes": (C.c_int, [C.c_void_p, C.c_int, C.POINTER(C.c_size_t)]),
     "cfd_unet_forward": (C.c_int, [C.c_void_p, C.c_void_p, C.c_void_p, C.c_void_p, C.c_int, C.c_void_p,
                                    C.c_size_t, C.c_void_p]),
diff --git a/confild_amd/csrc/conv_x.hip b/confild_amd/csrc/conv_x.hip
--- a/confild_amd/csrc/conv_x.hip
+++ b/confild_amd/csrc/conv_x.hip
@@ -21,7 +21,11 @@
     asm("v_fma_mixhi_f16 %0, %1, 1.0, -%2 op_sel:[0,0,1] op_sel_hi:[0,0,1]" : "+v"(lo.y) : "v"(x[3]), "v"(hi.y));
 }
 
-template <int BM, int BN, int WGM, int WGN, int PF = 1>
+__device__ __forceinline__ float phase_scale(const ConvArgs& a, int ph) {
+    return ph == 0 ? a.ph_scale[0] : ph == 1 ? a.ph_scale[1] : ph == 2 ? a.ph_scale[2] : a.ph_scale[3];
+}
+
+template <int BM, int BN, int WGM, int WGN, int PF = 1, bool PH = false>
 __global__ __launch_bounds__(64 * WGM * WGN, 1) void conv_x_kernel(ConvArgs a) {
     constexpr int NW = WGM * WGN, NT = 64 * NW;
     constexpr int WTM = BM / WGM, WTN = BN / WGN;
@@ -41,31 +45,40 @@
 
     int bx, by, bz;
     xcd_tile(a.xcd, bx, by, bz);
+    const int ph = PH ? bx & 3 : 0, py = ph >> 1, px = ph & 1;
+    if constexpr (PH) bx >>= 2;
     const int m0 = bx * BM, n0 = by * BN;
     const int HWo = a.Hout * a.Wout;
+    const int HWm = PH ? a.Hin * a.Win : HWo, Wm = PH ? a.Win : a.Wout, Mm = PH ? a.M >> 2 : a.M;
     const int kq = tid & 7, rsub = tid >> 3;
-    __shared__ int pixtab[9 * BM];
+    __shared__ int pixtab[(PH ? 4 : 9) * BM];
 
     const int srows = __builtin_amdgcn_readfirstlane(a.Hin * a.Win * (a.M / HWo));
     const __amdgpu_buffer_rsrc_t rs1 = __builtin_amdgcn_make_buffer_rsrc((void*)a.src1, 0, srows * a.C1 * 4, 0x00020000);
     const __amdgpu_buffer_rsrc_t rs2 = __builtin_amdgcn_make_buffer_rsrc(
         (void*)(a.src2 ? (const void*)a.src2 : (const void*)a.src1), 0, a.src2 ? srows * a.C2 * 4 : 0, 0x00020000);
-    const int ntap = a.ks * a.ks, KM = ntap * a.Ctot;
-    const __amdgpu_buffer_rsrc_t rwh = __builtin_amdgcn_make_buffer_rsrc((void*)a.wbf, 0, a.Cout * KM * 2, 0x00020000);
-    const __amdgpu_buffer_rsrc_t rwl = __builtin_amdgcn_make_buffer_rsrc((void*)a.wlo, 0, a.Cout * KM * 2, 0x00020000);
+    const int ntap = PH ? 4 : a.ks * a.ks, KM = ntap * a.Ctot;
+    const char* const wh0 = PH ? (const char*)a.wph + (int64_t)ph * a.Cout * KM * 2 : (const char*)a.wbf;
+    const char* const wl0 = PH ? (const char*)a.wpl + (int64_t)ph * a.Cout * KM * 2 : (const char*)a.wlo;
+    const __amdgpu_buffer_rsrc_t rwh = __builtin_amdgcn_make_buffer_rsrc((void*)wh0, 0, a.Cout * KM * 2, 0x00020000);
+    const __amdgpu_buffer_rsrc_t rwl = __builtin_amdgcn_make_buffer_rsrc((void*)wl0, 0, a.Cout * KM * 2, 0x00020000);
     {
-        const float rhw = 1.0f / (float)HWo, rw = 1.0f / (float)a.Wout;
+        const float rhw = 1.0f / (float)HWm, rw = 1.0f / (float)Wm;
         for (int e = tid; e < ntap * BM; e += NT) {
             const int tap = e / BM, r = e - tap * BM;
-            const int ty = tap_row(tap, a.ks), tx = tap - ty * a.ks;
+            const int ty = PH ? tap >> 1 : tap_row(tap, a.ks), tx = PH ? tap & 1 : tap - ty * a.ks;
             const int m = m0 + r;
             int pix = -1;
-            if (m < a.M) {
-                const int b = fdiv24(m, HWo, rhw), rem = m - b * HWo;
-                const int oy = fdiv24(rem, a.Wout, rw), ox = rem - oy * a.Wout;
+            if (m < Mm) {
+                const int b = fdiv24(m, HWm, rhw), rem = m - b * HWm;
+                const int oy = fdiv24(rem, Wm, rw), ox = rem - oy * Wm;
                 int iy, ix;
                 bool ok;
-                if (a.up) {
+                if constexpr (PH) {
+                    iy = oy - 1 + py + ty;
+                    ix = ox - 1 + px + tx;
+                    ok = iy >= 0 && iy < a.Hin && ix >= 0 && ix < a.Win;
+                } else if (a.up) {
                     iy = oy - a.pad + ty;
                     ix = ox - a.pad + tx;
                     ok = iy >= 0 && iy < 2 * a.Hin && ix >= 0 && ix < 2 * a.Win;
@@ -95,7 +108,7 @@
         b_voff[it] = n < a.Cout ? (unsigned)((n * KM + 4 * kq) * 2) : 0x80000000u;
     }
 
-    const int nkt = a.K / 32;
+    const int nkt = KM / 32;
     const int per = (nkt + gridDim.z - 1) / gridDim.z;
     const int kt0 = bz * per;
     const int kt1 = min(nkt, kt0 + per);
@@ -219,17 +232,25 @@
 #pragma unroll
     for (int i = 0; i < TM; ++i)
 #pragma unroll
-        for (int j = 0; j < TN; ++j) acc[i][j] *= a.acc_scale;
+        for (int j = 0; j < TN; ++j) acc[i][j] *= PH ? phase_scale(a, ph) : a.acc_scale;
     const int n_base = n0 + wn * WTN + l32;
     const int m_base = m0 + wm * WTM + 4 * hsel;
+    auto orow = [&](int mm, int& bb) __attribute__((always_inline)) {
+        bb = mm / HWm;
+        if constexpr (!PH) return mm;
+        const int rem = mm - bb * HWm, y = rem / Wm, x = rem - y * Wm;
+        return (bb * a.Hout + 2 * y + py) * a.Wout + 2 * x + px;
+    };
     if (gridDim.z > 1) {
         float* part = a.part + (int64_t)bz * a.M * a.Cout;
 #pragma unroll
         for (int i = 0; i < TM; ++i)
 #pragma unroll
             for (int e = 0; e < 16; ++e) {
-                const int m = m_base + 32 * i + 8 * (e >> 2) + (e & 3);
-                if (m >= a.M) continue;
+                const int mm = m_base + 32 * i + 8 * (e >> 2) + (e & 3);
+                if (mm >= Mm) continue;
+                int bb;
+                const int m = orow(mm, bb);
 #pragma unroll
                 for (int j = 0; j < TN; ++j) {
                     const int n = n_base + 32 * j;
@@ -246,9 +267,10 @@
     for (int i = 0; i < TM; ++i)
 #pragma unroll
         for (int e = 0; e < 16; ++e) {
-            const int m = m_base + 32 * i + 8 * (e >> 2) + (e & 3);
-            if (m >= a.M) continue;
-            const int bb = m / HWo;
+            const int mm = m_base + 32 * i + 8 * (e >> 2) + (e & 3);
+            if (mm >= Mm) continue;
+            int bb;
+            const int m = orow(mm, bb);
 #pragma unroll
             for (int j = 0; j < TN; ++j) {
                 const int n = n_base + 32 * j;
@@ -261,9 +283,10 @@
         }
 }
 
-template <int BM, int TW, bool BF = false, bool SB = false, int BN = 128>
+template <int BM, int TW, bool BF = false, bool SB = false, int BN = 128, bool PH = false>
 __global__ __launch_bounds__(BM * (BN / 64), 1) void conv_h_kernel(ConvArgs a) {
     static_assert(!SB || BF, "a bf16 source needs the bf16 kernel");
+    static_assert(!PH || !BF, "the phase form is split-f16 only");
     constexpr unsigned SES = SB ? 2u : 4u;
     constexpr int WGN = BN / 64, WGM = BM / 64, NTG = 64 * WGM * WGN;
     static_assert(BN == 64 || BN == 128, "K1h: 64 or 128 output channels per workgroup");
@@ -276,7 +299,8 @@
     };
     constexpr int HPLANE = NPX * 64;
     constexpr int HIT = (NPX * 8 + NTG - 1) / NTG;
-    constexpr int TG = BF ? 3 : 1, SPR = 9 / TG;
+    constexpr int NTAP = PH ? 4 : 9;
+    constexpr int TG = BF ? 3 : 1, SPR = NTAP / TG;
     constexpr int BPLANE = BN * 64, BSTAGE = PL * BPLANE * TG;
     constexpr int BIT = BN * 4 / NTG;
     constexpr int GBYTES = PL * HPLANE + 2 * BSTAGE;
@@ -292,20 +316,27 @@
     char* const ring = halo + PL * HPLANE;
     int bx, by, bz;
     xcd_tile(a.xcd, bx, by, bz);
+    const int ph = PH ? bx & 3 : 0, py = ph >> 1, px = ph & 1;
+    if constexpr (PH) bx >>= 2;
     const int n0 = by * BN;
-    const int W = a.Wout, HWo = a.Hout * W;
+    const int W = PH ? a.Win : a.Wout, Hh = PH ? a.Hin : a.Hout, HWo = Hh * W;
     const int tps = HWo / BM, tpr = W / TW;
     const int bimg = bx / tps, tl = bx - bimg * tps;
     const int y0 = (tl / tpr) * TR, x0 = (tl - (tl / tpr) * tpr) * TW;
-    const int64_t mrow0 = (int64_t)bimg * HWo + (int64_t)y0 * W + x0;
-    CFD_DASSERT(mrow0 + (int64_t)(TR - 1) * W + TW <= a.M && HWo % BM == 0 && W % TW == 0);
-
-    const int srows = __builtin_amdgcn_readfirstlane(a.Hin * a.Win * (a.M / HWo));
+    const int64_t mrow0 = PH ? ((int64_t)bimg * a.Hout + 2 * y0 + py) * a.Wout + 2 * x0 + px
+                             : (int64_t)bimg * HWo + (int64_t)y0 * W + x0;
+    CFD_DASSERT(mrow0 + (int64_t)(PH ? 2 : 1) * ((int64_t)(TR - 1) * a.Wout + TW - 1) < a.M && HWo % BM == 0 &&
+                W % TW == 0);
+
+    const int srows = __builtin_amdgcn_readfirstlane(a.Hin * a.Win * (a.M / (a.Hout * a.Wout)));
     const __amdgpu_buffer_rsrc_t rs1 = __builtin_amdgcn_make_buffer_rsrc((void*)a.src1, 0, srows * a.C1 * SES, 0x00020000);
     const __amdgpu_buffer_rsrc_t rs2 = __builtin_amdgcn_make_buffer_rsrc(
         (void*)(a.src2 ? (const void*)a.src2 : (const void*)a.src1), 0, a.src2 ? srows * a.C2 * SES : 0, 0x00020000);
-    const __amdgpu_buffer_rsrc_t rwh = __builtin_amdgcn_make_buffer_rsrc((void*)a.wbf, 0, a.Cout * 9 * a.Ctot * 2, 0x00020000);
-    const __amdgpu_buffer_rsrc_t rwl = __builtin_amdgcn_make_buffer_rsrc((void*)a.wlo, 0, a.Cout * 9 * a.Ctot * 2, 0x00020000);
+    const int wbytes = a.Cout * NTAP * a.Ctot * 2;
+    const char* const wh0 = PH ? (const char*)a.wph + (int64_t)ph * wbytes : (const char*)a.wbf;
+    const char* const wl0 = PH ? (const char*)a.wpl + (int64_t)ph * wbytes : (const char*)a.wlo;
+    const __amdgpu_buffer_rsrc_t rwh = __builtin_amdgcn_make_buffer_rsrc((void*)wh0, 0, wbytes, 0x00020000);
+    const __amdgpu_buffer_rsrc_t rwl = __builtin_amdgcn_make_buffer_rsrc((void*)wl0, 0, wbytes, 0x00020000);
 
     const int kq = gt & 7;
     int hpix[HIT];
@@ -315,9 +346,9 @@
         int pix = -1;
         if (hp < NPX) {
             const int hr = hp / HW2, hc = hp - hr * HW2;
-            const int iy = y0 - 1 + hr, ix = x0 - 1 + hc;
-            if (hc < TW + 2 && iy >= 0 && iy < a.Hout && ix >= 0 && ix < W)
-                pix = a.up ? (bimg * a.Hin + (iy >> 1)) * a.Win + (ix >> 1) : (bimg * a.Hin + iy) * a.Win + ix;
+            const int iy = y0 - 1 + hr + py, ix = x0 - 1 + hc + px;
+            if (hc < TW + (PH ? 1 : 2) && (!PH || hr < TR + 1) && iy >= 0 && iy < Hh && ix >= 0 && ix < W)
+                pix = a.up && !PH ? (bimg * a.Hin + (iy >> 1)) * a.Win + (ix >> 1) : (bimg * a.Hin + iy) * a.Win + ix;
         }
         CFD_DASSERT(pix < srows);
         hpix[it] = pix;
@@ -327,7 +358,7 @@
 #pragma unroll
     for (int it = 0; it < BIT; ++it) {
         const int n = n0 + (gt >> 2) + it * (NTG / 4);
-        bvoff[it] = n < a.Cout ? (unsigned)((n * 9 * a.Ctot + 8 * bq) * 2) : 0x80000000u;
+        bvoff[it] = n < a.Cout ? (unsigned)((n * NTAP * a.Ctot + 8 * bq) * 2) : 0x80000000u;
     }
 
     const int nch = a.Ctot / 32;
@@ -460,8 +491,8 @@
                     }
                 }
             } else {
-            const int ty = t / 3;
-            const int tofs = ty * HW2 + (t - 3 * ty);
+            const int ty = PH ? t >> 1 : t / 3;
+            const int tofs = ty * HW2 + (PH ? t & 1 : t - 3 * ty);
 #pragma unroll
             for (int s2 = 0; s2 < 2; ++s2) {
                 const int ch = 2 * s2 + hsel;
@@ -517,11 +548,14 @@
 #pragma unroll
         for (int i = 0; i < 2; ++i)
 #pragma unroll
-            for (int j = 0; j < 2; ++j) acc[i][j] *= a.acc_scale;
+            for (int j = 0; j < 2; ++j) acc[i][j] *= PH ? phase_scale(a, ph) : a.acc_scale;
     }
     const int n_base = n0 + wn * 64 + l32;
     const int p_base = wm * 64 + 4 * hsel;
-    auto pix_of = [&](int p) __attribute__((always_inline)) { return mrow0 + (int64_t)(p / TW) * W + (p % TW); };
+    auto pix_of = [&](int p) __attribute__((always_inline)) {
+        if constexpr (PH) return mrow0 + (int64_t)(p / TW) * (2 * a.Wout) + 2 * (p % TW);
+        else return mrow0 + (int64_t)(p / TW) * W + (p % TW);
+    };
     {
         if (a.ldsepi) {
             static_assert(64 * BN * 4 <= (int)sizeof(lds), "epilogue stage fits the LDS");
@@ -615,6 +649,15 @@
     return 0;
 }
 
+int conv_hp_tw(const ConvArgs& a) {
+    const bool geo = !a.tmode && a.up && a.ks == 3 && a.stride == 1 && a.pad == 1 && a.C1 % 32 == 0 &&
+                     a.C2 % 32 == 0 && a.Hout == 2 * a.Hin && a.Wout == 2 * a.Win && a.M % (a.Hout * a.Wout) == 0;
+    if (!geo) return 0;
+    for (int tw = 64; tw >= 16; tw >>= 1)
+        if (a.Win % tw == 0 && a.Hin % (256 / tw) == 0) return tw;
+    return 0;
+}
+
 int launch_conv_x(const ConvArgs& a, int variant, int splits, hipStream_t st) {
     CFD_REQUIRE(a.wbf && !a.tmode, CFD_ESTATE, "conv_x: split-f16 or bf16 forward only");
     CFD_REQUIRE(a.Ctot % 32 == 0 && a.C1 % 4 == 0 && a.C2 % 4 == 0, CFD_ESHAPE, "conv_x needs channels % 32 == 0");
@@ -665,6 +708,27 @@
         return splits;
     }
     CFD_REQUIRE(a.wlo, CFD_ESTATE, "internal: K1x runs split-f16 operands only");
+    if (variant >= 24 && variant <= 26) {
+        CFD_REQUIRE(a.wph && a.wpl && a.up && a.ks == 3 && a.stride == 1 && a.pad == 1 && a.Hout == 2 * a.Hin &&
+                        a.Wout == 2 * a.Win,
+                    CFD_ESTATE, "internal: the phase form needs an Upsample convolution and its phase packs");
+        if (variant == 24) {
+            const int tw = conv_hp_tw(a);
+            CFD_REQUIRE(tw > 0, CFD_ESHAPE, "conv_h phase form: a 16/32/64-divisible low-resolution width");
+            const dim3 g = grid(256, 128);
+            if (tw == 64) hipLaunchKernelGGL((conv_h_kernel<256, 64, false, false, 128, true>), g, dim3(512), 0, st, a);
+            else if (tw == 32) hipLaunchKernelGGL((conv_h_kernel<256, 32, false, false, 128, true>), g, dim3(512), 0, st, a);
+            else hipLaunchKernelGGL((conv_h_kernel<256, 16, false, false, 128, true>), g, dim3(512), 0, st, a);
+            check_launch("conv_h_kernel (phase)");
+            return splits;
+        }
+        const int bm = variant == 26 ? 256 : 128;
+        const dim3 g(4u * (unsigned)ceil_div(a.M / 4, bm), (unsigned)ceil_div(a.Cout, 128), splits);
+        if (variant == 26) hipLaunchKernelGGL((conv_x_kernel<256, 128, 4, 2, 1, true>), g, dim3(512), 0, st, a);
+        else hipLaunchKernelGGL((conv_x_kernel<128, 128, 2, 2, 1, true>), g, dim3(256), 0, st, a);
+        check_launch("conv_x_kernel (phase)");
+        return splits;
+    }
     switch (variant) {
         case 1: hipLaunchKernelGGL((conv_x_kernel<128, 128, 2, 2>), grid(128, 128), dim3(256), 0, st, a); break;
         case 2: hipLaunchKernelGGL((conv_x_kernel<256, 128, 4, 2>), grid(256, 128), dim3(512), 0, st, a); break;
diff --git a/confild_amd/csrc/siren_split.hip b/confild_amd/csrc/siren_split.hip
--- a/confild_amd/csrc/siren_split.hip
+++ b/confild_amd/csrc/siren_split.hip
@@ -218,6 +218,10 @@
 
     int J = 0, slot = 0;
     constexpr int QE = NQ > 1 ? 1 : 0;
+    if (!NOSYNC) {
+        __builtin_amdgcn_s_waitcnt(vmcnt_imm(0));
+        asm volatile("s_barrier" ::: "memory");
+    }
     for (int layer = 1; layer <= nh; ++layer) {
         const bool last = layer == nh;
         const float m = p.w0f / p.wscale[layer - 1];
diff --git a/confild_amd/csrc/unet.hip b/confild_amd/csrc/unet.hip
--- a/confild_amd/csrc/unet.hip
+++ b/confild_amd/csrc/unet.hip
@@ -26,6 +26,9 @@
     size_t toffset = 0;
     float split_inv = 1.f;
     float tsplit_inv = 1.f;
+    bool phase = false;
+    size_t poffset = 0;
+    float psplit_inv[4] = {1.f, 1.f, 1.f, 1.f};
 };
 
 struct ResSpec {
@@ -68,6 +71,9 @@
     uint16_t* arena_lo = nullptr;
     uint16_t* arena_thi = nullptr;
     uint16_t* arena_tlo = nullptr;
+    uint16_t* arena_phi = nullptr;
+    uint16_t* arena_plo = nullptr;
+    size_t arena_p_elems = 0;
     int compute = CFD_COMPUTE_SPLIT_F16;
     int plan_b = 0;
     int tape_mode = CFD_TAPE_INPUT_VJP;
@@ -226,6 +232,14 @@
         toff += ((p.tpack == 2 ? p.count / 9 * 16 : p.count) + 3) & ~size_t(3);
     }
     h->arena_t_floats = toff;
+    size_t poff = 0;
+    for (auto& p : h->params) {
+        if (p.tpack != 2 || p.shape[0] < cfd::kPhaseMinCout) continue;
+        p.phase = true;
+        p.poffset = poff;
+        poff += (p.count / 9 * 16 + 7) & ~size_t(7);
+    }
+    h->arena_p_elems = poff;
 }
 
 const void* PB(const cfd_unet* h, const std::string& key) {
@@ -259,6 +273,17 @@
     a->wbf = h->arena_thi + p.toffset;
     a->wlo = h->arena_tlo + p.toffset;
     a->acc_scale = p.tsplit_inv;
+}
+
+void PP(const cfd_unet* h, const std::string& key, cfd::ConvArgs* a) {
+    if (h->compute != CFD_COMPUTE_SPLIT_F16) return;
+    auto it = h->index.find(key);
+    CFD_REQUIRE(it != h->index.end(), CFD_EKEY, "internal: missing param " + key);
+    const auto& p = h->params[it->second];
+    if (!p.phase) return;
+    a->wph = h->arena_phi + p.poffset;
+    a->wpl = h->arena_plo + p.poffset;
+    for (int ph = 0; ph < 4; ++ph) a->ph_scale[ph] = p.psplit_inv[ph];
 }
 
 const float* PT(const cfd_unet* h, const std::string& key) {
@@ -498,6 +523,7 @@
         a.w = P(h, pre + ".weight");
         a.wbf = PB(h, pre + ".weight");
         a.wlo = PL(h, pre + ".weight", &a.acc_scale);
+        if (up) PP(h, pre + ".weight", &a);
         a.bias = P(h, pre + ".bias");
         a.emb = embp;
         a.emb_stride = h->emb_total;
@@ -1084,6 +1110,8 @@
             CFD_HIP(hipMalloc(&h->arena_lo, sizeof(uint16_t) * std::max<size_t>(h->arena_floats, 4)));
             CFD_HIP(hipMalloc(&h->arena_thi, sizeof(uint16_t) * std::max<size_t>(h->arena_t_floats, 4)));
             CFD_HIP(hipMalloc(&h->arena_tlo, sizeof(uint16_t) * std::max<size_t>(h->arena_t_floats, 4)));
+            CFD_HIP(hipMalloc(&h->arena_phi, sizeof(uint16_t) * std::max<size_t>(h->arena_p_elems, 8)));
+            CFD_HIP(hipMalloc(&h->arena_plo, sizeof(uint16_t) * std::max<size_t>(h->arena_p_elems, 8)));
             const int half = cfg->model_channels / 2;
             std::vector<float> fr(half);
             const float nl = (float)(-std::log(10000.0));
@@ -1112,6 +1140,8 @@
     (void)hipFree(h->arena_lo);
     (void)hipFree(h->arena_thi);
     (void)hipFree(h->arena_tlo);
+    (void)hipFree(h->arena_phi);
+    (void)hipFree(h->arena_plo);
     (void)hipFree(h->nonfinite);
     (void)hipFree(h->rp_desc);
     (void)hipFree(h->rp_first);
@@ -1227,6 +1257,12 @@
             CFD_HIP(hipMemcpy(h->arena_thi + p.toffset, thi.data(), pk.size() * 2, hipMemcpyHostToDevice));
             CFD_HIP(hipMemcpy(h->arena_tlo + p.toffset, tlo.data(), pk.size() * 2, hipMemcpyHostToDevice));
         }
+        if (p.phase) {
+            std::vector<_Float16> phi, plo;
+            cfd::phase_pack_host(host, p.shape[0], p.shape[1], phi, plo, p.psplit_inv);
+            CFD_HIP(hipMemcpy(h->arena_phi + p.poffset, phi.data(), phi.size() * 2, hipMemcpyHostToDevice));
+            CFD_HIP(hipMemcpy(h->arena_plo + p.poffset, plo.data(), plo.size() * 2, hipMemcpyHostToDevice));
+        }
         p.set = true;
         ++h->version;
     });
@@ -1428,6 +1464,31 @@
         }
     }
 }
+
+__global__ __launch_bounds__(256) void rp_phase_amax_kernel(const float* __restrict__ w, int64_t ci, int64_t np4,
+                                                            unsigned* __restrict__ amax4) {
+    const int ph = blockIdx.y;
+    float m = 0.f;
+    for (int64_t e = (int64_t)blockIdx.x * 256 + threadIdx.x; e < np4; e += (int64_t)gridDim.x * 256)
+        m = fmaxf(m, fabsf(phase_value(w, ci, ph, e)));
+    __shared__ float r[256];
+    r[threadIdx.x] = m;
+    __syncthreads();
+    for (int s = 128; s > 0; s >>= 1) {
+        if (threadIdx.x < s) r[threadIdx.x] = fmaxf(r[threadIdx.x], r[threadIdx.x + s]);
+        __syncthreads();
+    }
+    if (threadIdx.x == 0) atomicMax(amax4 + ph, __float_as_uint(r[0]));
+}
+
+__global__ __launch_bounds__(256) void rp_phase_pack_kernel(const float* __restrict__ w, int64_t ci, int64_t np4,
+                                                            const unsigned* __restrict__ amax4,
+                                                            _Float16* __restrict__ phi, _Float16* __restrict__ plo) {
+    const int ph = blockIdx.y;
+    const float s = rp_scale(__uint_as_float(amax4[ph]));
+    for (int64_t e = (int64_t)blockIdx.x * 256 + threadIdx.x; e < np4; e += (int64_t)gridDim.x * 256)
+        rp_split(phase_value(w, ci, ph, e), s, phi, plo, ph * np4 + e);
+}
 }
 
 extern "C" int cfd_unet_load_flat(cfd_unet* h, const float* flat, size_t n, void* stream) {
@@ -1483,7 +1544,9 @@
             CFD_HIP(hipMalloc(&h->rp_desc, sizeof(cfd::RepackDesc) * np));
             CFD_HIP(hipMalloc(&h->rp_first, sizeof(int64_t) * (np + 1)));
             CFD_HIP(hipMalloc(&h->rp_part, sizeof(float) * 2 * blocks));
-            CFD_HIP(hipMalloc(&h->rp_amax, sizeof(float) * 2 * np));
+            size_t nup = 0;
+            for (const auto& p : h->params) nup += p.phase ? 1 : 0;
+            CFD_HIP(hipMalloc(&h->rp_amax, sizeof(float) * (2 * np + 4 * nup)));
             CFD_HIP(hipMemcpy(h->rp_desc, desc.data(), sizeof(cfd::RepackDesc) * np, hipMemcpyHostToDevice));
             CFD_HIP(hipMemcpy(h->rp_first, first.data(), sizeof(int64_t) * (np + 1), hipMemcpyHostToDevice));
             h->rp_blocks = blocks;
@@ -1505,9 +1568,41 @@
                                (_Float16*)h->arena_tlo);
             cfd::check_launch("rp_tpack_kernel");
         }
-        std::vector<float> amax(2 * (size_t)np);
-        CFD_HIP(hipMemcpyAsync(amax.data(), h->rp_amax, sizeof(float) * 2 * np, hipMemcpyDeviceToHost, st));
+        std::vector<int> ups;
+        for (int k = 0; k < np; ++k)
+            if (h->params[k].phase) ups.push_back(k);
+        unsigned* pamax = (unsigned*)(h->rp_amax + 2 * (size_t)np);
+        if (!ups.empty()) CFD_HIP(hipMemsetAsync(pamax, 0, sizeof(unsigned) * 4 * ups.size(), st));
+        {
+            int64_t src = 0;
+            size_t u = 0;
+            for (int k = 0; k < np; ++k) {
+                const auto& p = h->params[k];
+                if (p.phase) {
+                    const int64_t ci = p.shape[1], np4 = (int64_t)p.count / 9 * 4;
+                    const dim3 g((unsigned)std::min<int64_t>(1024, cfd::ceil_div(np4, 256)), 4);
+                    hipLaunchKernelGGL(cfd::rp_phase_amax_kernel, g, dim3(256), 0, st, flat + src, ci, np4,
+                                       pamax + 4 * u);
+                    cfd::check_launch("rp_phase_amax_kernel");
+                    hipLaunchKernelGGL(cfd::rp_phase_pack_kernel, g, dim3(256), 0, st, flat + src, ci, np4,
+                                       pamax + 4 * u, (_Float16*)h->arena_phi + p.poffset,
+                                       (_Float16*)h->arena_plo + p.poffset);
+                    cfd::check_launch("rp_phase_pack_kernel");
+                    ++u;
+                }
+                src += (int64_t)p.count;
+            }
+        }
+        std::vector<float> amax(2 * (size_t)np + 4 * ups.size());
+        CFD_HIP(hipMemcpyAsync(amax.data(), h->rp_amax, sizeof(float) * amax.size(), hipMemcpyDeviceToHost, st));
         CFD_HIP(hipStreamSynchronize(st));
+        for (size_t u = 0; u < ups.size(); ++u)
+            for (int ph = 0; ph < 4; ++ph) {
+                const float am = amax[2 * (size_t)np + 4 * u + ph];
+                int ex = 0;
+                if (am > 0.f) std::frexp(am, &ex);
+                h->params[ups[u]].psplit_inv[ph] = std::ldexp(1.0f, ex);
+            }
         for (int k = 0; k < np; ++k) {
             auto& p = h->params[k];
             if (p.pack == Pack::Conv1 || p.pack == Pack::Conv3) {
@@ -1523,6 +1618,76 @@
             p.set = true;
         }
         ++h->version;
+    });
+}
+
+extern "C" int cfd_upsample_conv(const float* x, const float* w_host, const float* bias_host, float* out, int B,
+                                 int H, int W, int Cin, int Cout, int plan_b, int device, int* kx, void* stream) {
+    return cfd::guard([&] {
+        CFD_REQUIRE(x && w_host && bias_host && out, CFD_EARG, "null argument");
+        CFD_REQUIRE(B > 0 && H > 0 && W > 0 && Cin > 0 && Cin % 32 == 0 && Cout > 0 && Cout % 4 == 0 && plan_b >= 0 &&
+                        plan_b <= 64,
+                    CFD_ESHAPE, "upsample conv: Cin % 32 == 0, Cout % 4 == 0, plan batch 0 .. 64");
+        cfd::DeviceGuard dg(device);
+        hipStream_t st = (hipStream_t)stream;
+        const size_t n = (size_t)Cout * Cin * 9;
+        std::vector<float> pk(n);
+        for (int64_t o = 0; o < Cout; ++o)
+            for (int64_t i = 0; i < Cin; ++i)
+                for (int tap = 0; tap < 9; ++tap) pk[(o * 9 + tap) * Cin + i] = w_host[(o * Cin + i) * 9 + tap];
+        float amax = 0.f;
+        for (float v : pk) amax = std::max(amax, std::fabs(v));
+        int ex = 0;
+        if (amax > 0.f) std::frexp(amax, &ex);
+        const float s = std::ldexp(1.0f, -ex);
+        std::vector<_Float16> hi(n), lo(n), phi, plo;
+        for (size_t e = 0; e < n; ++e) {
+            const float v = pk[e] * s;
+            hi[e] = (_Float16)v;
+            lo[e] = (_Float16)(v - (float)hi[e]);
+        }
+        cfd::ConvArgs a{};
+        cfd::phase_pack_host(w_host, Cout, Cin, phi, plo, a.ph_scale);
+        struct Bufs {
+            void* p[7] = {};
+            ~Bufs() { for (void* q : p) (void)hipFree(q); }
+        } d;
+        const size_t bytes[6] = {n * 4, n * 2, n * 2, phi.size() * 2, plo.size() * 2, (size_t)Cout * 4};
+        const void* srcs[6] = {pk.data(), hi.data(), lo.data(), phi.data(), plo.data(), bias_host};
+        for (int k = 0; k < 6; ++k) {
+            CFD_HIP(hipMalloc(&d.p[k], bytes[k]));
+            CFD_HIP(hipMemcpy(d.p[k], srcs[k], bytes[k], hipMemcpyHostToDevice));
+        }
+        a.src1 = x;
+        a.C1 = a.Ctot = Cin;
+        a.w = (const float*)d.p[0];
+        a.wbf = d.p[1];
+        a.wlo = d.p[2];
+        a.wph = d.p[3];
+        a.wpl = d.p[4];
+        a.acc_scale = std::ldexp(1.0f, ex);
+        a.bias = (const float*)d.p[5];
+        a.out = out;
+        a.Hin = H;
+        a.Win = W;
+        a.Hout = 2 * H;
+        a.Wout = 2 * W;
+        a.stride = 1;
+        a.ks = 3;
+        a.pad = 1;
+        a.up = 1;
+        a.Cout = Cout;
+        a.M = B * a.Hout * a.Wout;
+        a.K = 9 * Cin;
+        a.plan_b = plan_b > 0 ? plan_b : 8;
+        const cfd::ConvPlan plan = cfd::plan_conv(a, kSplitPer8);
+        if (plan.splits > 1) {
+            CFD_HIP(hipMalloc(&d.p[6], sizeof(float) * plan.splits * (size_t)a.M * Cout));
+            a.part = (float*)d.p[6];
+        }
+        if (kx) *kx = plan.kx;
+        cfd::launch_conv(a, plan, st);
+        CFD_HIP(hipStreamSynchronize(st));
     });
 }
 
diff --git a/confild_amd/csrc/unet_kernels.hip b/confild_amd/csrc/unet_kernels.hip
--- a/confild_amd/csrc/unet_kernels.hip
+++ b/confild_amd/csrc/unet_kernels.hip
@@ -1678,6 +1678,34 @@
         while (sp > 1 && (size_t)sp * mn * a.Cout > part_cap_floats) sp /= 2;
         return even_splits(nch, sp);
     };
+#ifndef CFD_NO_UPPHASE
+    if (a.up && a.wph && a.wpl && a.wbf && a.wlo && !a.tmode && a.ks == 3 && a.stride == 1 && a.pad == 1 &&
+        a.Hout == 2 * a.Hin && a.Wout == 2 * a.Win && a.Cout >= kPhaseMinCout && fits32) {
+        ConvPlan q;
+        q.bn = 128;
+        if (conv_hp_tw(a) > 0) {
+            q.kx = 24;
+            q.bm = 256;
+            q.nw = 8;
+            const int64_t t = ceil_div(mn, 256) * ceil_div(a.Cout, 128);
+            const int nch = a.Ctot / 32;
+            int sp = 1;
+            while (t * sp * 2 <= 256 && sp * 2 <= nch && sp < 16) sp *= 2;
+            while (sp > 1 && (size_t)sp * mn * a.Cout > part_cap_floats) sp /= 2;
+            q.splits = even_splits(nch, sp);
+            return q;
+        }
+        q.kx = mn / 4 >= 2048 ? 26 : 25;
+        q.bm = q.kx == 26 ? 256 : 128;
+        q.nw = q.kx == 26 ? 8 : 4;
+        const int64_t t = 4 * ceil_div(mn / 4, q.bm) * ceil_div(a.Cout, 128);
+        const int nkp = 4 * a.Ctot / 32;
+        q.splits = 1;
+        while (t * q.splits * 2 <= 256 && nkp / (q.splits * 2) >= 4 && q.splits < 32) q.splits *= 2;
+        while (q.splits > 1 && (size_t)q.splits * mn * a.Cout > part_cap_floats) q.splits /= 2;
+        return q;
+    }
+#endif
     if (a.wbf && !a.wlo && !a.tmode && a.ks == 3 && a.stride == 1 && a.Cout >= 128 && fits32 && conv_h_tw(a) > 0) {
         ConvPlan q;
         q.kx = 22;
diff --git a/confild_amd/csrc/unet_kernels.hpp b/confild_amd/csrc/unet_kernels.hpp
--- a/confild_amd/csrc/unet_kernels.hpp
+++ b/confild_amd/csrc/unet_kernels.hpp
@@ -1,4 +1,8 @@
 #pragma once
+#include <algorithm>
+#include <cmath>
+#include <vector>
+
 #include "common.hpp"
 
 namespace cfd {
@@ -37,6 +41,9 @@
     const void* wbf;
     const void* wlo;
     float acc_scale;
+    const void* wph;
+    const void* wpl;
+    float ph_scale[4];
     const float* bias;
     const float* emb;
     const float* res;
@@ -62,6 +69,49 @@
     int seq;
     int plan_b;
 };
+constexpr int kPhaseMinCout = 128;
+
+__host__ __device__ inline void phase_taps(int p, int t, int& lo, int& hi) {
+    lo = t == 0 ? 0 : 1 + p;
+    hi = t == 0 ? p : 2;
+}
+__host__ __device__ inline float phase_value(const float* w, int64_t ci, int ph, int64_t e) {
+    const int64_t i = e % ci, ot = e / ci, o = ot >> 2;
+    const int tap = (int)(ot & 3);
+    int ylo, yhi, xlo, xhi;
+    phase_taps(ph >> 1, tap >> 1, ylo, yhi);
+    phase_taps(ph & 1, tap & 1, xlo, xhi);
+    const float* base = w + (o * ci + i) * 9;
+    double v = 0.0;
+    for (int dy = ylo; dy <= yhi; ++dy)
+        for (int dx = xlo; dx <= xhi; ++dx) v += (double)base[dy * 3 + dx];
+    return (float)v;
+}
+
+inline void phase_pack_host(const float* w, int64_t co, int64_t ci, std::vector<_Float16>& phi,
+                            std::vector<_Float16>& plo, float inv[4]) {
+    const int64_t np4 = co * ci * 4;
+    phi.resize((size_t)np4 * 4);
+    plo.resize((size_t)np4 * 4);
+    std::vector<float> pv((size_t)np4);
+    for (int ph = 0; ph < 4; ++ph) {
+        float amax = 0.f;
+        for (int64_t e = 0; e < np4; ++e) {
+            pv[e] = phase_value(w, ci, ph, e);
+            amax = std::max(amax, std::fabs(pv[e]));
+        }
+        int ex = 0;
+        if (amax > 0.f) std::frexp(amax, &ex);
+        const float sc = std::ldexp(1.0f, -ex);
+        inv[ph] = std::ldexp(1.0f, ex);
+        for (int64_t e = 0; e < np4; ++e) {
+            const float v = pv[e] * sc;
+            phi[ph * np4 + e] = (_Float16)v;
+            plo[ph * np4 + e] = (_Float16)(v - (float)phi[ph * np4 + e]);
+        }
+    }
+}
+
 void stamps_set(unsigned long long* buf);
 unsigned long long* stamps_buf();
 
@@ -149,6 +199,7 @@
 }
 int launch_conv_x(const ConvArgs& a, int variant, int splits, hipStream_t st);
 int conv_h_tw(const ConvArgs& a);
+int conv_hp_tw(const ConvArgs& a);
 bool conv_p_applies(const ConvArgs& a);
 void conv_p_tile(int variant, int& bm, int& bn, int& nw);
 void launch_conv_p(const ConvArgs& a, int variant, hipStream_t st);
diff --git a/include/confild.h b/include/confild.h
--- a/include/confild.h
+++ b/include/confild.h
@@ -46,6 +46,8 @@
 int  cfd_unet_forward(cfd_unet* h, const float* x, const int64_t* t, float* eps, int B,
                       void* workspace, size_t ws_bytes, void* stream);
 int  cfd_unet_check_finite(cfd_unet* h, int* nonfinite, void* stream);
+int  cfd_upsample_conv(const float* x, const float* w_host, const float* bias_host, float* out, int B, int H,
+                       int W, int Cin, int Cout, int plan_b, int device, int* kx, void* stream);
 
 int  cfd_unet_tape_bytes(const cfd_unet* h, int B, size_t* bytes);
 int  cfd_unet_vjp_workspace_bytes(const cfd_unet* h, int B, size_t* bytes);
```
